# zhongyuanzhao/multihop-offload

Measured on AMD Instinct MI355X. Metric: episodes/sec, higher is better.
Workload: dtype fp32; 1 GPU; model=ChebConv-K2-5L-h32, graph=ba100-m2, global_batch=256, T=1000, parallelism=dp1, congest_jobs=2124

## Files before the change

### multihop_offload_amd/engine.py

```python

from __future__ import annotations

import dataclasses
from typing import Optional, Sequence

import numpy as np
import torch

from .graphs import CaseGraph
from .models.chebconv import ChebConvStack
from .queueing import ConflictCSR, delay_with_fallback, fixed_point_mu
from .ops import dispatch as ops


@dataclasses.dataclass
class JobBatch:
    sources: torch.Tensor
    mask: torch.Tensor
    rates: torch.Tensor
    ul: torch.Tensor
    dl: torch.Tensor

    @property
    def num_real(self):
        return self.mask.sum()


@dataclasses.dataclass
class EpisodeResult:
    tau: torch.Tensor
    congest: torch.Tensor
    num_jobs: torch.Tensor
    delay_emp: torch.Tensor
    loss_fn: Optional[torch.Tensor] = None
    loss_mse: Optional[torch.Tensor] = None
    dst: Optional[torch.Tensor] = None
    route_links: Optional[torch.Tensor] = None
    nhop: Optional[torch.Tensor] = None


def hist_percentile(hist: torch.Tensor, dmax: torch.Tensor,
                    q: float) -> torch.Tensor:
    from .sim.timeslot import delay_bin_upper
    hist = hist.to(torch.int64)
    total = hist.sum(-1)
    need = torch.ceil(q * total.to(torch.float64)).to(torch.int64) \
        .clamp(min=1)
    k = (hist.cumsum(-1) >= need[..., None]).to(torch.int8).argmax(-1)
    edges = torch.tensor([delay_bin_upper(i) for i in range(hist.shape[-1])],
                         dtype=torch.int64, device=hist.device)
    got = torch.minimum(edges[k], dmax.to(torch.int64)).to(torch.float64)
    return torch.where(total > 0, got, torch.full_like(got, float("nan")))


@dataclasses.dataclass
class SimStats:
    delay_max: torch.Tensor
    late: torch.Tensor
    delay_hist: torch.Tensor
    stuck: torch.Tensor
    stuck_age: torch.Tensor
    qlen_sum: torch.Tensor
    qlen_max: torch.Tensor
    busy_slots: torch.Tensor
    nb_sum: torch.Tensor
    delay_sum: torch.Tensor
    count: torch.Tensor
    late_after: torch.Tensor
    num_links: int
    T_sim: int
    warmup: int

    def _scope(self, x: torch.Tensor, per: str, how: str = "sum"):
        if per == "job":
            return x
        if per not in ("graph", "all"):
            raise ValueError("per: 'graph', 'job' or 'all'")
        dims = (1,) if per == "graph" else (0, 1)
        return x.amax(dims) if how == "max" else x.sum(dims)

    @staticmethod
    def _ratio(num, den):
        num, den = num.to(torch.float64), den.to(torch.float64)
        return torch.where(den > 0, num / den.clamp(min=1),
                           torch.full_like(den, float("nan")))

    def percentile(self, q: float, per: str = "graph") -> torch.Tensor:
        return hist_percentile(
            self._scope(self.delay_hist.to(torch.int64), per),
            self._scope(self.delay_max, per, "max"), q)

    def late_ratio(self, per: str = "graph") -> torch.Tensor:
        return self._ratio(self._scope(self.late.to(torch.int64), per),
                           self._scope(self.count.to(torch.int64), per))

    def censored_mean_delay(self, per: str = "graph") -> torch.Tensor:
        return self._ratio(
            self._scope(self.delay_sum + self.stuck_age, per),
            self._scope((self.count + self.stuck).to(torch.int64), per))

    def utilization(self) -> torch.Tensor:
        return self.busy_slots.to(torch.float64) \
            / max(self.T_sim - self.warmup, 1)

    def mean_qlen(self) -> torch.Tensor:
        return self.qlen_sum.to(torch.float64) \
            / max(self.T_sim - self.warmup, 1)

    def mean_contention(self) -> torch.Tensor:
        E = self.num_links
        return self._ratio(self.nb_sum[:, :E], self.busy_slots[:, :E])


@dataclasses.dataclass
class SimResult:
    delay_sum: torch.Tensor
    count: torch.Tensor
    mean_delay: torch.Tensor
    backlog: torch.Tensor
    trace: Optional[torch.Tensor] = None
    stats: Optional[SimStats] = None
    sched_slots: Optional[torch.Tensor] = None

    def sched_share(self) -> torch.Tensor:
        if self.sched_slots is None or self.stats is None:
            raise ValueError("sched_share: needs simulate(stats=True, "
                             "mac='mwis')")
        E = self.sched_slots.shape[1]
        return SimStats._ratio(self.sched_slots,
                               self.stats.busy_slots[:, :E])


class EpisodeEngine:

    def __init__(self, cases: Sequence[CaseGraph], model: ChebConvStack,
                 device: str = "cpu", dtype: torch.dtype = torch.float32,
                 fp_iters: int = 10, walk_cap: Optional[int] = None,
                 delay_clamp: float = 0.0, lam_margin: float = 0.0,
                 native_glue: bool = True):
        assert len(cases) > 0
        N = cases[0].num_nodes
        T = cases[0].T
        assert all(c.num_nodes == N for c in cases), "batch shares N"
        E = max(c.num_links for c in cases)
        self.cases = list(cases)
        self.B, self.N, self.E, self.T = len(cases), N, E, T
        self.E_list = [c.num_links for c in cases]
        self.device = torch.device(device)
        self.dtype = dtype
        self.fp_iters = fp_iters
        self.delay_clamp = float(delay_clamp)
        self.lam_margin = float(lam_margin)
        self.model = model.to(self.device)
        self.walk_cap = walk_cap or N

        Cmax = max(len(c.ext.comp_nodes) for c in cases)
        Ee = E + Cmax
        self.Ee = Ee
        B = self.B

        def t(a, dt=None):
            return torch.as_tensor(np.asarray(a), dtype=dt or dtype,
                                   device=self.device)

        def ti(a):
            return torch.as_tensor(np.asarray(a), dtype=torch.int64,
                                   device=self.device)

        def pad_rows(arrs, width, fill, dt=np.float64):
            out = np.full((B, width), fill, dtype=dt)
            for b, a in enumerate(arrs):
                out[b, :len(a)] = a
            return out

        edges_np = np.zeros((B, E, 2), dtype=np.int64)
        for b, c in enumerate(cases):
            edges_np[b, :c.num_links] = c.edges
        self.edges = ti(edges_np)
        self.link_rates = t(pad_rows([c.link_rates for c in cases], E, 1.0))
        self.cf_degs = t(pad_rows([c.cf_degs for c in cases], E, 0.0))
        self.proc_bws = t([c.proc_bws for c in cases])
        self.roles = ti([c.roles for c in cases])
        self.adj = torch.as_tensor(
            np.stack([c.adj for c in cases]) != 0, device=self.device)
        self.link_matrix = ti([c.link_matrix for c in cases])
        nv = -np.ones((B, N), dtype=np.int64)
        for b, c in enumerate(cases):
            v = c.ext.node_vedge
            nv[b] = np.where(v >= 0, v - c.num_links + E, -1)
        self.node_vedge = ti(nv)
        self.comp_mask = self.roles < 2
        self.sp_hop = t([c.sp_hop for c in cases])
        lm = np.zeros((B, E), dtype=bool)
        for b, c in enumerate(cases):
            lm[b, :c.num_links] = True
        self.link_mask = torch.as_tensor(lm, device=self.device)
        sel_b, sel_e = np.nonzero(lm)
        self._lk_sel = ti(sel_b * E + sel_e)
        e0v = edges_np[sel_b, sel_e, 0]
        e1v = edges_np[sel_b, sel_e, 1]
        self._lk_lin01 = ti(sel_b * (N * N) + e0v * N + e1v)
        self._lk_lin10 = ti(sel_b * (N * N) + e1v * N + e0v)

        S = max(len(c.servers) for c in cases)
        srv = -np.ones((B, S), dtype=np.int64)
        for b, c in enumerate(cases):
            srv[b, :len(c.servers)] = c.servers
        self.S = S
        self.servers = ti(srv)
        self.server_mask = self.servers >= 0
        self.servers_safe = self.servers.clamp(min=0)

        mob_counts = [len(c.mobile_nodes) for c in cases]
        assert min(mob_counts) >= 1, \
            "every case needs at least one mobile node (job sources)"
        self.Jmax = max(mob_counts) - 1 if max(mob_counts) > 1 else 1
        self.mobile_mask = self.roles == 0

        rows, cols = [], []
        for b, c in enumerate(cases):
            r = np.repeat(np.arange(c.num_links),
                          np.diff(c.conf_indptr)) + b * E
            rows.append(r)
            cols.append(c.conf_indices + b * E)
        self.conf = ConflictCSR.__new__(ConflictCSR)
        self.conf.row = ti(np.concatenate(rows))
        self.conf.col = ti(np.concatenate(cols))
        self.conf.n = B * E

        def remap(ids, Eb):
            ids = np.asarray(ids)
            return np.where(ids < Eb, ids, ids - Eb + E)

        rows, cols = [], []
        for b, c in enumerate(cases):
            ext = c.ext
            Eb = c.num_links
            ne = ext.num_edges_ext
            r = remap(np.repeat(np.arange(ne), np.diff(ext.ext_indptr)),
                      Eb) + b * Ee
            rows.append(r)
            cols.append(remap(ext.ext_indices, Eb) + b * Ee)
        self.support = ConflictCSR.__new__(ConflictCSR)
        self.support.row = ti(np.concatenate(rows))
        self.support.col = ti(np.concatenate(cols))
        self.support.n = B * Ee

        def feat(attr, link_fill, tail_fill):
            out = np.full((B, Ee), tail_fill, dtype=np.float64)
            for b, c in enumerate(cases):
                v = getattr(c.ext, attr)
                Eb = c.num_links
                out[b, :Eb] = v[:Eb]
                out[b, Eb:E] = link_fill
                out[b, E:E + len(v) - Eb] = v[Eb:]
            return t(out)

        for c in cases:
            c.ext.refresh_rates()
        self.f_self_loop = feat("edge_self_loop", 0.0, 1.0)
        self.f_as_server = feat("edge_as_server", 0.0, 0.0)
        self.f_rate = feat("edge_rate_ext", 1.0, 1.0)
        self.Cmax = Cmax
        bw = np.ones((B, self.Cmax), dtype=np.float64)
        for b, c in enumerate(cases):
            bw[b, :len(c.ext.comp_nodes)] = c.proc_bws[c.ext.comp_nodes]
        self.bw_comp = t(bw)

        cb, cn, cr = [], [], []
        for b, c in enumerate(cases):
            for rank, n in enumerate(c.ext.comp_nodes):
                cb.append(b)
                cn.append(int(n))
                cr.append(rank)
        self._comp_b = ti(cb)
        self._comp_n = ti(cn)
        self._comp_r = ti(cr)

        self._bidx = torch.arange(B, device=self.device)
        self._eye = torch.eye(N, dtype=torch.bool,
                              device=self.device)[None, :, :]
        self._explore_buf = torch.zeros((), dtype=torch.float32,
                                        device=self.device)
        self._rng_state = torch.tensor([12345, 0], dtype=torch.int64,
                                       device=self.device)
        self.overflow_total = torch.zeros((), dtype=torch.int64,
                                          device=self.device)
        self.T_arr = t([float(c.T) for c in cases])
        self.T_link = self.T_arr.repeat_interleave(E)

        def t32(a):
            return torch.as_tensor(np.asarray(a, dtype=np.int32),
                                   device=self.device)

        self.k_adj_indptr = t32([c.adj_indptr for c in cases])

        def pad_i32(arrs, width):
            out = np.zeros((B, width), dtype=np.int32)
            for b, a in enumerate(arrs):
                out[b, :len(a)] = a
            return t32(out)

        self.k_adj_idx = pad_i32([c.adj_indices for c in cases], 2 * E)
        self.k_adj_link = pad_i32([c.adj_link_ids for c in cases], 2 * E)
        cip = np.zeros((B, E + 1), dtype=np.int32)
        for b, c in enumerate(cases):
            Eb = c.num_links
            cip[b, :Eb + 1] = c.conf_indptr
            cip[b, Eb + 1:] = c.conf_indptr[-1]
        self.k_conf_indptr = t32(cip)
        self.k_E_arr = t32([c.num_links for c in cases])
        self.k_N_arr = t32([getattr(c, "real_n", c.num_nodes)
                            for c in cases])
        self._padded = any(getattr(c, "real_n", c.num_nodes) != N
                           for c in cases)
        cc, base = [], [0]
        for c in cases:
            cc.append(np.asarray(c.conf_indices, dtype=np.int32))
            base.append(base[-1] + len(c.conf_indices))
        self.k_conf_cols = t32(np.concatenate(cc))
        self.k_conf_base = torch.as_tensor(np.asarray(base[:-1]),
                                           dtype=torch.int64,
                                           device=self.device)
        self.k_edges = t32(edges_np)
        self.k_servers = t32(srv)
        ipt = np.zeros((B, Ee + 1), dtype=np.int32)
        cc, base = [], [0]
        for b, c in enumerate(cases):
            ext = c.ext
            Eb = c.num_links
            src_ipt = ext.ext_indptr
            counts = np.zeros(Ee, dtype=np.int64)
            counts[:Eb] = np.diff(src_ipt)[:Eb]
            nv = ext.num_edges_ext - Eb
            counts[E:E + nv] = np.diff(src_ipt)[Eb:]
            ipt[b, 1:] = np.cumsum(counts)
            colsrc = np.asarray(ext.ext_indices)
            link_cols = colsrc[:src_ipt[Eb]]
            virt_cols = colsrc[src_ipt[Eb]:]
            allc = np.concatenate([link_cols, virt_cols])
            allc = np.where(allc < Eb, allc, allc - Eb + E)
            cc.append(allc.astype(np.int32))
            base.append(base[-1] + len(allc))
        self.k_ext_indptr = t32(ipt)
        self.k_ext_max_nnz = int(max(int(c.ext.ext_indptr[-1])
                                     for c in cases))
        self.k_ext_cols = t32(np.concatenate(cc))
        self.k_ext_base = torch.as_tensor(np.asarray(base[:-1]),
                                          dtype=torch.int64,
                                          device=self.device)
        import os
        self.use_hip = (self.device.type == "cuda"
                        and os.environ.get("MHO_FORCE_TORCH") != "1")
        self.hip_walk_ok = self.hip_critic_ok = self.hip_actor_ok = False
        if self.use_hip:
            assert dtype == torch.float32, "HIP kernels are fp32"
            from .ops import dispatch
            plan = dispatch.require_hip().queue_lds_plan(N, E, Ee, fp_iters)
            self.hip_walk_ok = plan["walk_eval"]["fits"]
            self.hip_critic_ok = plan["critic"]["fits"]
            self.hip_actor_ok = (plan["actor_head_fwd"]["fits"]
                                 and plan["actor_head_bwd"]["fits"])
        self.native_glue = bool(native_glue) and self.use_hip

    def set_rng_seed(self, seed: int):
        self._rng_state[0] = int(seed)
        self._rng_state[1] = 0

    def sample_jobs(self, arrival_scale: float,
                    gen: Optional[torch.Generator] = None) -> JobBatch:
        B, N, J = self.B, self.N, self.Jmax
        dev = self.device
        scores_raw = torch.rand(B, N, device=dev, generator=gen)
        r_nj = torch.rand(B, device=dev, generator=gen)
        r_rates = torch.rand(B, J, device=dev, generator=gen)
        return self._jobs_from_draws(scores_raw, r_nj, r_rates,
                                     arrival_scale)

    def _jobs_from_draws(self, scores_raw: torch.Tensor, r_nj: torch.Tensor,
                         r_rates: torch.Tensor,
                         arrival_scale: float) -> JobBatch:
        J = self.Jmax
        dev = self.device
        if self.native_glue:
            sources, mask, rates, ul, dl = ops.require_hip().jobs_from_draws(
                scores_raw, r_nj, r_rates, self.mobile_mask,
                float(arrival_scale))
            return JobBatch(sources=sources, mask=mask, rates=rates, ul=ul,
                            dl=dl)
        scores = torch.where(self.mobile_mask, scores_raw,
                             torch.full_like(scores_raw, 2.0))
        order = torch.argsort(scores, dim=1)
        sources = order[:, :J]
        M = self.mobile_mask.sum(1)
        lo = (0.3 * M).to(torch.int64)
        span = (M - lo).clamp(min=1)
        nj = lo + (r_nj * span.to(self.dtype)).to(torch.int64)
        nj = nj.clamp(min=1)
        mask = torch.arange(J, device=dev)[None, :] < nj[:, None]
        sources = torch.where(mask, sources, sources[:, :1])
        rates = (r_rates * 0.4 + 0.1) * arrival_scale
        z = torch.zeros(self.B, J, device=dev, dtype=self.dtype)
        return JobBatch(
            sources=sources,
            mask=mask,
            rates=torch.where(mask, rates.to(self.dtype), z),
            ul=torch.where(mask, torch.full_like(z, 100.0), z),
            dl=torch.where(mask, torch.full_like(z, 1.0), z),
        )

    def pack_jobs(self, instances) -> JobBatch:
        B, J = self.B, self.Jmax
        assert len(instances) == B
        src = np.zeros((B, J), dtype=np.int64)
        mask = np.zeros((B, J), dtype=bool)
        rates = np.zeros((B, J))
        ul = np.zeros((B, J))
        dl = np.zeros((B, J))
        for b, jobs in enumerate(instances):
            k = jobs.num_jobs
            assert k <= J, (k, J)
            src[b, :k] = jobs.sources
            src[b, k:] = (jobs.sources[0] if k
                          else self.cases[b].ext.comp_nodes[0])
            mask[b, :k] = True
            rates[b, :k] = jobs.rates
            ul[b, :k] = jobs.ul
            dl[b, :k] = jobs.dl
        dev, dt = self.device, self.dtype
        return JobBatch(
            sources=torch.as_tensor(src, device=dev),
            mask=torch.as_tensor(mask, device=dev),
            rates=torch.as_tensor(rates, dtype=dt, device=dev),
            ul=torch.as_tensor(ul, dtype=dt, device=dev),
            dl=torch.as_tensor(dl, dtype=dt, device=dev),
        )

    def _features(self, jobs: JobBatch) -> torch.Tensor:
        if self.native_glue:
            return ops.require_hip().cheb_features(
                jobs.sources, jobs.rates.contiguous(), jobs.ul.contiguous(),
                jobs.mask, self.node_vedge, self.comp_mask, self.f_self_loop,
                self.f_rate, self.f_as_server)
        B, Ee, N = self.B, self.Ee, self.N
        arr = torch.zeros(B, N, dtype=self.dtype, device=self.device)
        arr = arr.scatter_add(1, jobs.sources, jobs.rates * jobs.ul)
        f_job = torch.zeros(B, Ee, dtype=self.dtype, device=self.device)
        vidx = torch.where(self.comp_mask, self.node_vedge,
                           torch.zeros_like(self.node_vedge))
        f_job = f_job.scatter_add(
            1, vidx, torch.where(self.comp_mask, arr, torch.zeros_like(arr)))
        return torch.stack([self.f_self_loop, self.f_rate, f_job,
                            self.f_as_server], dim=-1)

    def _actor_head_tables(self):
        return (self.k_conf_indptr, self.k_conf_base, self.k_conf_cols,
                self.link_rates.contiguous(), self.bw_comp.contiguous(),
                self.k_edges, self.node_vedge, self.T_arr.contiguous(),
                self.k_E_arr)

    def _lam_hip(self, jobs: JobBatch) -> torch.Tensor:
        B, Ee = self.B, self.Ee
        x = self._features(jobs)
        from .ops.functions import ChebStackFn, cheb_compat
        if cheb_compat(self.model):
            params = []
            for layer in self.model.layers:
                params += [layer.weight, layer.bias]
            lam = ChebStackFn.apply(x.contiguous(), self, *params)
        else:
            import os as _os
            if _os.environ.get("MHO_ALLOW_TORCH_GPU") != "1":
                raise RuntimeError(
                    "model shape unsupported by the fused ChebConv "
                    "kernels (feature width > 32 or dropout > 0); "
                    "refusing eager torch on GPU — set "
                    "MHO_ALLOW_TORCH_GPU=1 to override")
            return self.model(x.reshape(B * Ee, 4),
                              self.support).reshape(B, Ee)
        if self.lam_margin:
            lam = lam * (1.0 + self.lam_margin)
        return lam

    def _actor_forward_native(self, jobs: JobBatch):
        lam = self._lam_hip(jobs)
        lam_c = lam.detach().contiguous()
        dm, mu_hist = ops.require_hip().actor_head_fwd(
            lam_c, *self._actor_head_tables(), self.N, self.fp_iters,
            self.delay_clamp)
        return dm, (lam, lam_c, mu_hist)

    def _actor_backward_native(self, saved, grad_edge, dm, unit_mtx,
                               written):
        lam, lam_c, mu_hist = saved
        dlam, loss_mse = ops.require_hip().actor_head_bwd_fused(
            grad_edge.contiguous(), dm, unit_mtx, written, lam_c, mu_hist,
            *self._actor_head_tables(), self.fp_iters, self.delay_clamp)
        lam.backward(dlam)
        return loss_mse

    def actor_forward(self, jobs: JobBatch):
        B, E, Ee, N = self.B, self.E, self.Ee, self.N
        if self.use_hip and self.hip_actor_ok:
            from .ops.functions import ActorHeadFn
            dm = ActorHeadFn.apply(self._lam_hip(jobs), self)
            return dm, None, None

        x = self._features(jobs)
        lam = self.model(x.reshape(B * Ee, 4), self.support).reshape(B, Ee)
        if self.lam_margin:
            lam = lam * (1.0 + self.lam_margin)

        lam_link = lam[:, :E].reshape(-1)
        mu = fixed_point_mu(lam_link, self.link_rates.reshape(-1),
                            self.cf_degs.reshape(-1), self.conf,
                            self.fp_iters)
        link_delay = delay_with_fallback(lam_link, mu, self.T_link, 101.0,
                                         self.delay_clamp).reshape(B, E)
        node_delay = delay_with_fallback(lam[:, E:], self.bw_comp,
                                         self.T_arr[:, None], 100.0,
                                         self.delay_clamp)

        dm = self._delay_matrix(link_delay, node_delay)
        return dm, link_delay, node_delay

    def _delay_matrix(self, link_delay, node_delay):
        B, N, E = self.B, self.N, self.E
        flat = torch.zeros(B * N * N, dtype=self.dtype, device=self.device)
        ld_valid = link_delay.reshape(-1)[self._lk_sel]
        flat = flat.index_put((self._lk_lin01,), ld_valid)
        flat = flat.index_put((self._lk_lin10,), ld_valid)
        diag_idx = (self._bidx[:, None] * (N * N)
                    + torch.arange(N, device=self.device)[None, :] * (N + 1))
        inf = torch.full((B, N), float("inf"), dtype=self.dtype,
                         device=self.device)
        flat = flat.index_put((diag_idx.reshape(-1),), inf.reshape(-1))
        lin = (self._comp_b * (N * N) + self._comp_n * (N + 1))
        flat = flat.index_put((lin,), node_delay[self._comp_b, self._comp_r])
        return flat.reshape(B, N, N)

    def apsp(self, dm: torch.Tensor) -> torch.Tensor:
        B, N = self.B, self.N
        with torch.no_grad():
            if self.native_glue:
                return ops.require_hip().floyd_warshall_dm(
                    dm.detach(), self.adj,
                    self.k_N_arr if self._padded else None)
            w = torch.where(self.adj, dm.detach(),
                            torch.full_like(dm, float("inf")))
            w = torch.where(self._eye, torch.zeros_like(w), w)
            return ops.floyd_warshall(
                w, self.k_N_arr if self._padded else None)

    def offload_decide(self, jobs: JobBatch, sp: torch.Tensor,
                       uds: torch.Tensor, explore: float = 0.0,
                       gen: Optional[torch.Generator] = None,
                       prob: bool = False):
        B, J, S = self.B, self.Jmax, self.S
        if S == 0:
            local = uds.gather(1, jobs.sources) * jobs.ul
            return jobs.sources.clone(), local
        if self.use_hip:
            from .ops import dispatch
            ext = dispatch.require_hip()
            expl_t = None
            if torch.is_tensor(explore):
                expl_t = explore.to(self.device, torch.float32)
            elif explore > 0:
                self._explore_buf.fill_(float(explore))
                expl_t = self._explore_buf
            rng_t = None
            if expl_t is not None or prob:
                self._rng_state[1] += 1
                rng_t = self._rng_state
            dst, islocal = ext.decide(
                sp.contiguous(), self.sp_hop.contiguous(), uds.contiguous(),
                self.k_servers, jobs.sources, jobs.mask,
                jobs.ul.contiguous(), jobs.dl.contiguous(),
                expl_t, rng_t, 1 if prob else 0)
            return dst, None

        bJ = self._bidx[:, None]
        src = jobs.sources
        local = uds.gather(1, src) * jobs.ul

        sp_src = sp[bJ, src]
        hop_src = self.sp_hop[bJ, src]
        srv = self.servers_safe[:, None, :].expand(B, J, S)
        ul_d = torch.maximum(sp_src.gather(2, srv) * jobs.ul[..., None],
                             hop_src.gather(2, srv))
        dl_d = torch.maximum(sp_src.gather(2, srv) * jobs.dl[..., None],
                             hop_src.gather(2, srv))
        uds_srv = uds.gather(1, srv.reshape(B, -1)).reshape(B, J, S)
        pr_d = torch.maximum(uds_srv * jobs.ul[..., None],
                             torch.ones_like(uds_srv))
        server_costs = ul_d + dl_d + pr_d
        server_costs = torch.where(
            self.server_mask[:, None, :], server_costs,
            torch.full_like(server_costs, float("inf")))
        costs = torch.cat([server_costs, local[..., None]], dim=2)

        if prob:
            logits = costs.clamp(max=1e30)
            logits = logits - logits.amax(dim=2, keepdim=True)
            p = torch.exp(logits)
            p = torch.where(torch.isfinite(costs), p, torch.zeros_like(p))
            choice = torch.multinomial(
                p.reshape(B * J, S + 1), 1, generator=gen).reshape(B, J)
        else:
            choice = costs.argmin(dim=2)
        if explore > 0:
            nS = self.server_mask.sum(1, keepdim=True)
            r = torch.rand(B, J, device=self.device, generator=gen)
            rc = (torch.rand(B, J, device=self.device, generator=gen)
                  * (nS + 1).to(self.dtype)).to(torch.int64)
            rc = torch.where(rc >= nS, torch.full_like(rc, S), rc)
            choice = torch.where(r < explore, rc, choice)

        is_local = choice >= torch.minimum(
            self.server_mask.sum(1, keepdim=True),
            torch.full_like(choice, S))
        dst = torch.where(
            is_local, src,
            self.servers_safe.gather(1, choice.clamp(max=S - 1)))
        dst = torch.where(jobs.mask, dst, src)
        est = torch.where(
            is_local, local,
            server_costs.gather(2, choice.clamp(max=S - 1)[..., None])[..., 0])
        return dst, est

    def route_walk(self, jobs: JobBatch, dst: torch.Tensor, sp: torch.Tensor):
        B, J, N = self.B, self.Jmax, self.N
        bJ = self._bidx[:, None]
        node = jobs.sources.clone()
        links, hops = [], torch.zeros(B, J, dtype=torch.int64,
                                      device=self.device)
        sp_to_dst = sp.gather(
            2, dst[:, None, :].expand(B, N, J))
        for _ in range(self.walk_cap):
            active = (node != dst) & jobs.mask
            if not bool(active.any()):
                break
            adj_row = self.adj[bJ, node]
            cand = torch.where(adj_row, sp_to_dst.transpose(1, 2),
                               torch.full_like(sp_to_dst.transpose(1, 2),
                                               float("inf")))
            nxt = cand.argmin(dim=2)
            link = self.link_matrix[bJ, node, nxt]
            links.append(torch.where(active, link,
                                     torch.full_like(link, -1)))
            node = torch.where(active, nxt, node)
            hops += active.to(torch.int64)
        if links:
            route_links = torch.stack(links, dim=2)
        else:
            route_links = torch.full((B, J, 0), -1, dtype=torch.int64,
                                     device=self.device)
        self.overflow_total += ((node != dst) & jobs.mask).sum()
        return route_links, hops

    def _episode_eval(self, jobs: JobBatch, dst: torch.Tensor,
                      sp: torch.Tensor):
        if self.use_hip and self.hip_walk_ok:
            from .ops import dispatch
            ext = dispatch.require_hip()
            H = min(self.walk_cap, 64)
            rl, nhop, delay_emp, unit_mtx, written, overflow = ext.walk_eval(
                sp.contiguous(), jobs.sources, dst.contiguous(), jobs.mask,
                jobs.rates.contiguous(), jobs.ul.contiguous(),
                jobs.dl.contiguous(), self.k_adj_indptr, self.k_adj_idx,
                self.k_adj_link, self.k_conf_indptr, self.k_conf_base,
                self.k_conf_cols, self.link_rates.contiguous(),
                self.proc_bws.contiguous(), self.k_edges,
                self.T_arr.contiguous(), self.k_E_arr, self.k_N_arr, H,
                self.fp_iters)
            self._last_overflow = overflow
            self.overflow_total += overflow.sum().to(torch.int64)
            return rl, nhop, delay_emp, unit_mtx, written
        rl, nhop = self.route_walk(jobs, dst, sp)
        delay_emp, unit_mtx, written, *_ = self.evaluate(jobs, dst, rl, nhop)
        return rl, nhop, delay_emp, unit_mtx, written

    def check_overflow(self, strict: bool = True) -> int:
        n = int(self.overflow_total)
        if n:
            self.overflow_total.zero_()
            if strict:
                raise RuntimeError(
                    f"{n} greedy routing walk(s) failed to reach their "
                    f"destination within walk_cap={self.walk_cap} hops — "
                    "loads/delays for those jobs are truncated "
                    "(pathological delay matrix or walk_cap too small "
                    "for this topology)")
        return n

    def evaluate(self, jobs: JobBatch, dst: torch.Tensor,
                 route_links: torch.Tensor, nhop: torch.Tensor):
        B, E, N, J = self.B, self.E, self.N, self.Jmax
        H = route_links.shape[2]
        valid = route_links >= 0
        safe = route_links.clamp(min=0)

        ulr = jobs.ul * jobs.rates
        dlr = jobs.dl * jobs.rates
        load = (ulr + dlr)[..., None].expand(B, J, H)
        flat_idx = (self._bidx[:, None, None] * E + safe).reshape(-1)
        link_lambda = torch.zeros(B * E, dtype=self.dtype, device=self.device)
        link_lambda = link_lambda.scatter_add(
            0, flat_idx, torch.where(valid, load,
                                     torch.zeros_like(load)).reshape(-1))
        server_load = torch.zeros(B, N, dtype=self.dtype, device=self.device)
        server_load = server_load.scatter_add(
            1, dst, torch.where(jobs.mask, ulr, torch.zeros_like(ulr)))

        with torch.no_grad():
            mu = fixed_point_mu(link_lambda, self.link_rates.reshape(-1),
                                self.cf_degs.reshape(-1), self.conf,
                                self.fp_iters)
        lam_r = link_lambda.reshape(B, E)
        mu_r = mu.reshape(B, E)

        lam_h = lam_r.gather(1, safe.reshape(B, -1)).reshape(B, J, H)
        mu_h = mu_r.gather(1, safe.reshape(B, -1)).reshape(B, J, H)
        tot = (jobs.ul + jobs.dl)[..., None]
        gap = mu_h - lam_h
        unit = torch.where(gap > 0, 1.0 / torch.where(gap > 0, gap,
                                                      torch.ones_like(gap)),
                           self.T_arr[:, None, None] * lam_h / (tot * mu_h))
        nh = nhop.to(self.dtype)[..., None]
        hop_delay = (torch.maximum(jobs.ul[..., None] * unit, nh)
                     + torch.maximum(jobs.dl[..., None] * unit, nh))
        link_part = torch.where(valid, hop_delay,
                                torch.zeros_like(hop_delay)).sum(dim=2)

        bw_dst = self.proc_bws.gather(1, dst)
        sl_dst = server_load.gather(1, dst)
        sgap = bw_dst - sl_dst
        sunit = torch.where(
            sgap > 0, 1.0 / torch.where(sgap > 0, sgap, torch.ones_like(sgap)),
            self.T_arr[:, None] * sl_dst / (jobs.ul * bw_dst))
        server_part = torch.maximum(jobs.ul * sunit, torch.ones_like(sunit))
        delay_emp = torch.where(jobs.mask, link_part + server_part,
                                torch.full_like(link_part, float("nan")))

        unit_mtx = torch.zeros(B * N * N, dtype=self.dtype, device=self.device)
        written = torch.zeros(B * N * N, dtype=torch.bool, device=self.device)
        e0 = self.edges[..., 0].gather(1, safe.reshape(B, -1)).reshape(B, J, H)
        e1 = self.edges[..., 1].gather(1, safe.reshape(B, -1)).reshape(B, J, H)
        base = (self._bidx[:, None, None] * (N * N))
        lin01 = (base + e0 * N + e1).reshape(-1)
        lin10 = (base + e1 * N + e0).reshape(-1)
        vmask = valid.reshape(-1)
        unit_mtx = unit_mtx.index_put((lin01[vmask],),
                                      unit.reshape(-1)[vmask])
        unit_mtx = unit_mtx.index_put((lin10[vmask],),
                                      unit.reshape(-1)[vmask])
        written = written.index_put((lin01[vmask],),
                                    torch.ones_like(lin01[vmask],
                                                    dtype=torch.bool))
        written = written.index_put((lin10[vmask],),
                                    torch.ones_like(lin10[vmask],
                                                    dtype=torch.bool))
        lin_d = (self._bidx[:, None] * (N * N) + dst * (N + 1)).reshape(-1)
        jm = jobs.mask.reshape(-1)
        unit_mtx = unit_mtx.index_put((lin_d[jm],), sunit.reshape(-1)[jm])
        written = written.index_put((lin_d[jm],),
                                    torch.ones_like(lin_d[jm],
                                                    dtype=torch.bool))
        return (delay_emp, unit_mtx.reshape(B, N, N),
                written.reshape(B, N, N), lam_r, mu_r, server_load)

    def critic_backward(self, jobs: JobBatch, dst: torch.Tensor,
                        route_links: torch.Tensor,
                        nhop: Optional[torch.Tensor] = None):
        B, E, Ee, J = self.B, self.E, self.Ee, self.Jmax
        vedge_dst = self.node_vedge.gather(1, dst)
        if self.use_hip and self.hip_critic_ok:
            from .ops import dispatch
            ext = dispatch.require_hip()
            grad_edge, loss = ext.critic(
                route_links.contiguous(), nhop.contiguous(),
                vedge_dst.contiguous(), jobs.mask,
                jobs.rates.contiguous(), jobs.ul.contiguous(),
                jobs.dl.contiguous(), self.k_conf_indptr, self.k_conf_base,
                self.k_conf_cols, self.link_rates.contiguous(),
                self.bw_comp.contiguous(), self.k_E_arr,
                self.T_arr.contiguous(), Ee,
                self.fp_iters, self.delay_clamp)
            return grad_edge, loss.sum()
        H = route_links.shape[2]
        valid = route_links >= 0
        safe = route_links.clamp(min=0)

        routes = torch.zeros(B, Ee, J, dtype=self.dtype, device=self.device)
        jidx = torch.arange(J, device=self.device)[None, :, None] \
            .expand(B, J, H)
        routes = routes.index_put(
            (self._bidx[:, None, None].expand(B, J, H)[valid],
             safe[valid], jidx[valid]), torch.ones(1, dtype=self.dtype,
                                                   device=self.device)[0]
            .expand(int(valid.sum())))
        jm = jobs.mask
        routes = routes.index_put(
            (self._bidx[:, None].expand(B, J)[jm], vedge_dst[jm],
             torch.arange(J, device=self.device)[None, :].expand(B, J)[jm]),
            torch.ones(int(jm.sum()), dtype=self.dtype, device=self.device))
        routes.requires_grad_(True)

        jobs_load = (jobs.rates * jobs.ul)[..., None]
        jobs_data = (jobs.ul + jobs.dl)[:, None, :]
        link_load = torch.bmm(routes, jobs_load)[..., 0]
        lam_link = link_load[:, :E].reshape(-1)
        mu = fixed_point_mu(lam_link, self.link_rates.reshape(-1),
                            self.cf_degs.reshape(-1), self.conf,
                            self.fp_iters)
        link_d = delay_with_fallback(lam_link, mu, self.T_link, 101.0,
                                     self.delay_clamp).reshape(B, E)
        node_d = delay_with_fallback(link_load[:, E:], self.bw_comp,
                                     self.T_arr[:, None], 100.0,
                                     self.delay_clamp)
        unit_edge = torch.cat([link_d, node_d], dim=1)
        delay_job_edge = torch.maximum(
            jobs_data * unit_edge[..., None] * routes, routes)
        loss_fn = delay_job_edge.sum()
        (grad_routes,) = torch.autograd.grad(loss_fn, routes,
                                             retain_graph=False)

        seq = torch.cat([safe, vedge_dst[..., None]], dim=2)
        seq_valid = torch.cat([valid, jm[..., None]], dim=2)
        g_seq = grad_routes.gather(
            1, seq.transpose(1, 2)).transpose(1, 2)
        g_seq = grad_routes.gather(1, seq.permute(0, 2, 1))
        g_seq = g_seq.permute(0, 2, 1)
        g_seq = torch.where(seq_valid, g_seq, torch.zeros_like(g_seq))
        pref = -torch.cumsum(g_seq, dim=2)
        grad_edge = torch.zeros(B * Ee, dtype=self.dtype, device=self.device)
        flat_seq = (self._bidx[:, None, None] * Ee + seq).reshape(-1)
        grad_edge = grad_edge.scatter_add(
            0, flat_seq, torch.where(seq_valid, pref,
                                     torch.zeros_like(pref)).reshape(-1))
        return grad_edge.reshape(B, Ee), loss_fn.detach()

    def grad_dist_matrix(self, grad_edge: torch.Tensor, dm: torch.Tensor,
                         unit_mtx: torch.Tensor, written: torch.Tensor):
        B, N, E = self.B, self.N, self.E
        flat = torch.zeros(B * N * N, dtype=self.dtype, device=self.device)
        ge_valid = grad_edge[:, :E].reshape(-1)[self._lk_sel]
        flat = flat.index_put((self._lk_lin01,), ge_valid)
        flat = flat.index_put((self._lk_lin10,), ge_valid)
        lin = (self._comp_b * (N * N) + self._comp_n * (N + 1))
        flat = flat.index_put(
            (lin,), grad_edge[self._comp_b, E + self._comp_r])
        grad_dist = flat.reshape(B, N, N)

        diff = dm.detach() - unit_mtx
        anchor_mask = written & torch.isfinite(dm.detach())
        anchor = torch.where(anchor_mask, 0.001 * diff,
                             torch.zeros_like(diff))
        n_valid = anchor_mask.sum().clamp(min=1)
        loss_mse = ((torch.where(anchor_mask, diff, torch.zeros_like(diff))
                     ** 2).sum() / n_valid.to(diff.dtype))
        return grad_dist + anchor, loss_mse

    def gnn_episode(self, jobs: JobBatch, explore: float = 0.0,
                    gen: Optional[torch.Generator] = None,
                    train: bool = True, prob: bool = False,
                    per_sample: bool = False,
                    refine: int = 0) -> EpisodeResult:
        ctx = torch.enable_grad() if train else torch.no_grad()
        native_bwd = self.native_glue and self.hip_actor_ok
        with ctx:
            if native_bwd:
                dm, actor_saved = self._actor_forward_native(jobs)
            else:
                dm, link_delay, node_delay = self.actor_forward(jobs)
        sp = self.apsp(dm)
        uds = torch.diagonal(dm.detach(), dim1=1, dim2=2)
        dst, est = self.offload_decide(jobs, sp, uds, explore, gen, prob)
        route_links, nhop, delay_emp, unit_mtx, written = \
            self._episode_eval(jobs, dst, sp)
        for _ in range(int(refine) if not train else 0):
            over = jobs.mask & (delay_emp > self.T_arr[:, None])
            if not bool(over.any()):
                break
            dst = torch.where(over, jobs.sources, dst)
            route_links, nhop, delay_emp, unit_mtx, written = \
                self._episode_eval(jobs, dst, sp)

        loss_fn = loss_mse = None
        self.last_per_sample_grads = None
        if train:
            grad_edge, loss_fn = self.critic_backward(jobs, dst, route_links,
                                                      nhop)
            self.per_sample_request = per_sample
            if native_bwd:
                loss_mse = self._actor_backward_native(
                    actor_saved, grad_edge, dm, unit_mtx, written)
            else:
                grad_dist, loss_mse = self.grad_dist_matrix(
                    grad_edge, dm, unit_mtx, written)
            if per_sample and not self.use_hip:
                params = list(self.model.parameters())
                out = []
                for b in range(self.B):
                    gd = torch.zeros_like(grad_dist)
                    gd[b] = grad_dist[b]
                    gs = torch.autograd.grad(dm, params, grad_outputs=gd,
                                             retain_graph=True,
                                             allow_unused=True)
                    out.append([torch.zeros_like(p) if g is None
                                else g.detach()
                                for p, g in zip(params, gs)])
                self.last_per_sample_grads = out
                dm.backward(grad_dist)
            else:
                if not native_bwd:
                    dm.backward(grad_dist)
                if per_sample:
                    self.last_per_sample_grads = \
                        self._collect_per_sample_grads()
            self.per_sample_request = False

        return self._result(jobs, delay_emp, loss_fn, loss_mse,
                            routes=(dst, route_links, nhop))

    def _result(self, jobs: JobBatch, delay_emp: torch.Tensor,
                loss_fn=None, loss_mse=None, routes=None) -> EpisodeResult:
        if self.native_glue:
            tau, congest, nj = ops.require_hip().episode_summary(
                delay_emp.contiguous(), jobs.mask, self.T_arr)
        else:
            nj = jobs.mask.sum(1)
            de = torch.where(jobs.mask, delay_emp,
                             torch.zeros_like(delay_emp))
            tau = de.sum(1) / nj.to(self.dtype)
            congest = ((delay_emp > self.T_arr[:, None]) & jobs.mask).sum(1)
        dst, route_links, nhop = routes or (None, None, None)
        return EpisodeResult(tau=tau, congest=congest, num_jobs=nj,
                             delay_emp=delay_emp, loss_fn=loss_fn,
                             loss_mse=loss_mse, dst=dst,
                             route_links=route_links, nhop=nhop)

    def draw_arrivals(self, jobs: JobBatch, T_sim: int,
                      gen: Optional[torch.Generator] = None) -> torch.Tensor:
        lam = torch.where(jobs.mask, jobs.rates,
                          torch.zeros_like(jobs.rates))
        lam = lam[:, None, :].expand(self.B, int(T_sim), lam.shape[1])
        arr = torch.poisson(lam.contiguous(), generator=gen)
        if arr.numel() and float(arr.max()) > 255:
            raise ValueError("draw_arrivals: a slot count exceeds 255 "
                             "(uint8) — job rates too high for the "
                             "simulator's arrival format")
        return arr.to(torch.uint8)

    def simulate(self, jobs: JobBatch, result: EpisodeResult,
                 arrivals: torch.Tensor, warmup: int = 0,
                 trace: bool = False, stats: bool = False,
                 late_after=None, mac: str = "share") -> SimResult:
        if mac not in ops.MAC_MODES:
            raise ValueError(f"simulate: mac must be one of {ops.MAC_MODES}, "
                             f"not {mac!r}")
        mwis = mac == "mwis"
        sched = None
        if result.dst is None or result.route_links is None \
                or result.nhop is None:
            raise ValueError("simulate: the EpisodeResult carries no routes")
        B, J = self.B, self.Jmax
        arrivals = torch.as_tensor(arrivals, device=self.device)
        assert arrivals.shape[0] == B and arrivals.shape[2] == J, \
            (tuple(arrivals.shape), (B, J))
        T_sim = arrivals.shape[1]
        warmup = int(warmup)
        st = None
        if stats:
            if late_after is None:
                late_after = torch.floor(self.T_arr)
            if not torch.is_tensor(late_after):
                late_after = torch.full((B,), int(late_after))
            late_after = late_after.to(device=self.device,
                                       dtype=torch.int32).reshape(B)
        if self.use_hip:
            out = ops.timeslot_sim(
                arrivals, result.route_links, result.nhop, result.dst,
                jobs.mask, jobs.ul, jobs.dl, self.link_rates, self.proc_bws,
                self.k_conf_indptr, self.k_conf_base, self.k_conf_cols,
                self.k_E_arr, self.k_N_arr, self.T_arr, warmup=warmup,
                trace=trace, stats=stats, late_after=late_after, mac=mac)
            delay_sum, count, tr = out[:3]
            st = out[3] if stats else None
            sched = out[-1] if mwis else None
        else:
            from .sim.timeslot import num_delay_bins, simulate_routes
            if arrivals.numel() and (int(arrivals.max()) > 255
                                     or int(arrivals.min()) < 0):
                raise ValueError("simulate: arrival counts must lie in "
                                 "[0, 255]")
            delay_sum = torch.zeros(B, J, dtype=torch.int64)
            count = torch.zeros(B, J, dtype=torch.int32)
            tr = torch.zeros(B, T_sim, 3, dtype=torch.int32) if trace \
                else None
            arr_np = arrivals.cpu().numpy()
            if stats:
                st = ops.empty_stats(B, J, self.E + self.N,
                                     num_delay_bins(T_sim))
            if mwis:
                sched = torch.zeros(B, self.E, dtype=torch.int32)
            for b, g in enumerate(self.cases):
                k = int(jobs.mask[b].sum())
                assert bool(jobs.mask[b, :k].all()), "mask is a prefix"
                out = simulate_routes(
                    g, jobs.ul[b, :k].cpu().numpy().astype(np.float64),
                    jobs.dl[b, :k].cpu().numpy().astype(np.float64),
                    result.dst[b, :k].cpu().numpy(),
                    result.route_links[b, :k].cpu().numpy(),
                    result.nhop[b, :k].cpu().numpy(), arr_np[b][:, :k],
                    warmup=warmup, trace=trace, stats=stats,
                    late_after=int(late_after[b]) if stats else None,
                    mac=mac)
                if mwis:
                    sched[b, :g.num_links] = torch.as_tensor(
                        out[-1]["sched_slots"])
                    out = out[:-1]
                if stats:
                    ops.fill_stats(st, b, out[-1], slice(0, k),
                                   g.num_links, self.E)
                delay_sum[b, :k] = torch.as_tensor(out[0])
                count[b, :k] = torch.as_tensor(out[1]).to(torch.int32)
                if trace:
                    for c, name in enumerate(("arrivals", "departures",
                                              "pkts_in_network")):
                        tr[b, :, c] = torch.as_tensor(
                            out[2][name]).to(torch.int32)
            delay_sum = delay_sum.to(self.device)
            count = count.to(self.device)
            tr = tr.to(self.device) if trace else None
            if stats:
                st = {k: v.to(self.device) for k, v in st.items()}
            if mwis:
                sched = sched.to(self.device)
        cnt = count.to(torch.float64)
        mean = torch.where(count > 0,
                           delay_sum.to(torch.float64) / cnt.clamp(min=1),
                           torch.full_like(cnt, float("nan")))
        arrived = torch.where(jobs.mask[:, None, :], arrivals,
                              torch.zeros_like(arrivals))[:, warmup:] \
            .sum(1, dtype=torch.int64)
        if stats:
            st = SimStats(**st, delay_sum=delay_sum, count=count,
                          late_after=late_after, num_links=self.E,
                          T_sim=int(T_sim), warmup=warmup)
        return SimResult(delay_sum=delay_sum, count=count, mean_delay=mean,
                         backlog=arrived - count.to(torch.int64), trace=tr,
                         stats=st, sched_slots=sched)

    def _collect_per_sample_grads(self):
        raw = getattr(self, "_per_sample_raw", None)
        if raw is None:
            raise RuntimeError(
                "per-sample gradients need the fused ChebConv GPU path")
        dW, db = raw
        self._per_sample_raw = None
        params = list(self.model.parameters())
        L = len(params) // 2
        out = []
        for b in range(self.B):
            gset = []
            for l in range(L):
                kw, fi, fo = params[2 * l].shape
                gset.append(dW[b, l, :kw, :fi, :fo])
                gset.append(db[b, l, :params[2 * l + 1].shape[0]])
            out.append(gset)
        return out

    def baseline_episode(self, jobs: JobBatch) -> EpisodeResult:
        B, N = self.B, self.N
        with torch.no_grad():
            dlist = 1.0 / self.link_rates
            dm = self._delay_matrix(
                dlist, torch.zeros_like(self.bw_comp))
            sp = self.apsp(dm)
            dproc = 1.0 / self.proc_bws
            uds = torch.where((self.proc_bws > 0),
                              dproc, torch.full_like(dproc, float("inf")))
            dst, est = self.offload_decide(jobs, sp, uds)
            rl, nhop, delay_emp, _, _ = self._episode_eval(jobs, dst, sp)
            return self._result(jobs, delay_emp, routes=(dst, rl, nhop))

    def local_episode(self, jobs: JobBatch) -> EpisodeResult:
        B, J = self.B, self.Jmax
        with torch.no_grad():
            dst = jobs.sources
            if self.use_hip:
                sp0 = torch.zeros(B, self.N, self.N, dtype=self.dtype,
                                  device=self.device)
                route_links, nhop, delay_emp, _, _ = self._episode_eval(
                    jobs, dst, sp0)
            else:
                route_links = torch.full((B, J, 0), -1, dtype=torch.int64,
                                         device=self.device)
                nhop = torch.zeros(B, J, dtype=torch.int64,
                                   device=self.device)
                delay_emp, *_ = self.evaluate(jobs, dst, route_links, nhop)
            return self._result(jobs, delay_emp,
                                routes=(dst, route_links, nhop))
```

### multihop_offload_amd/ops/dispatch.py

```python

from __future__ import annotations

import os

import torch

from . import torch_ref

_HIP_EXT = None
_HIP_TRIED = False


def _load_hip():
    global _HIP_EXT, _HIP_TRIED
    if _HIP_TRIED:
        return _HIP_EXT
    _HIP_TRIED = True
    try:
        from . import hip_loader
        _HIP_EXT = hip_loader.load()
    except Exception:
        _HIP_EXT = None
    return _HIP_EXT


def hip_available() -> bool:
    return _load_hip() is not None


def require_hip():
    ext = _load_hip()
    if ext is None:
        raise RuntimeError(
            "multihop_offload_amd HIP extension not built — run "
            "`python setup.py build_ext --inplace` (gfx950). GPU execution "
            "without the native kernels is disabled by design.")
    return ext


_require_hip = require_hip


def floyd_warshall(w: torch.Tensor, n_arr=None) -> torch.Tensor:
    if w.is_cuda and os.environ.get("MHO_FORCE_TORCH") != "1":
        ext = _require_hip()
        return ext.floyd_warshall(w.contiguous(), n_arr)
    return torch_ref.floyd_warshall(w)


def fw_force_inplace(on: bool) -> None:
    _require_hip().fw_force_inplace(bool(on))


def queue_csr_force_global(on: bool) -> None:
    _require_hip().queue_csr_force_global(bool(on))


def cheb_force_full_width(on: bool) -> None:
    _require_hip().cheb_force_full_width(bool(on))


def cheb_lds_plan(Ee: int, K: int, max_nnz: int) -> dict:
    plan = _require_hip().cheb_lds_plan(int(Ee), int(K), int(max_nnz))
    return {k: dict(v) for k, v in plan.items()}


STAT_KEYS = ("delay_max", "late", "delay_hist", "stuck", "stuck_age",
             "qlen_sum", "qlen_max", "busy_slots", "nb_sum")
_STAT_I64 = ("stuck_age", "qlen_sum", "nb_sum")
_STAT_PER_JOB = STAT_KEYS[:5]


def empty_stats(B: int, J: int, R: int, NB: int) -> dict:
    out = {}
    for k in STAT_KEYS:
        shape = (B, J, NB) if k == "delay_hist" else \
            (B, J) if k in _STAT_PER_JOB else (B, R)
        out[k] = torch.zeros(shape, dtype=torch.int64 if k in _STAT_I64
                             else torch.int32)
    return out


def fill_stats(st: dict, b: int, one: dict, idx, Eb: int, E: int) -> None:
    for k in STAT_KEYS:
        v = torch.as_tensor(one[k])
        if k in _STAT_PER_JOB:
            st[k][b, idx] = v
        else:
            st[k][b, :Eb] = v[:Eb]
            st[k][b, E:E + len(v) - Eb] = v[Eb:]


def timeslot_lds_plan(N: int, E: int, J: int) -> dict:
    return dict(_require_hip().timeslot_lds_plan(int(N), int(E), int(J)))


def timeslot_stats_lds_plan(N: int, E: int, J: int) -> dict:
    return dict(_require_hip().timeslot_stats_lds_plan(int(N), int(E),
                                                       int(J)))


def timeslot_mwis_lds_plan(N: int, E: int, J: int,
                           stats: bool = False) -> dict:
    return dict(_require_hip().timeslot_mwis_lds_plan(int(N), int(E), int(J),
                                                      bool(stats)))


MAC_MODES = ("share", "mwis")


def timeslot_sim(arrivals, route_links, nhop, dst, mask, ul, dl, link_rates,
                 proc_bws, conf_indptr, conf_base, conf_cols, E_arr, n_arr,
                 T_arr=None, warmup: int = 0, trace: bool = False,
                 stats: bool = False, late_after=None, mac: str = "share"):
    if mac not in MAC_MODES:
        raise ValueError(f"timeslot_sim: mac must be one of {MAC_MODES}, "
                         f"not {mac!r}")
    mwis = mac == "mwis"
    B, T, J = arrivals.shape
    if arrivals.numel() and (int(arrivals.max()) > 255
                             or int(arrivals.min()) < 0):
        raise ValueError("timeslot_sim: arrival counts must lie in [0, 255]")
    mask = mask.to(torch.bool)
    arr = torch.where(mask[:, None, :], arrivals,
                      torch.zeros_like(arrivals)).to(torch.uint8).contiguous()
    if route_links.shape[2] == 0:
        route_links = route_links.new_full((B, J, 1), -1)
    warmup = int(warmup)
    if warmup < 0:
        raise ValueError("timeslot_sim: warmup must be non-negative")

    if stats:
        if late_after is None:
            late_after = T
        if not torch.is_tensor(late_after):
            late_after = torch.full((B,), int(late_after), dtype=torch.int32)
        late_after = late_after.to(device=arr.device, dtype=torch.int32) \
            .reshape(B).contiguous()

    if arr.is_cuda:
        ext = _require_hip()
        slot_off = torch.zeros(B, T + 1, dtype=torch.int32, device=arr.device)
        slot_off[:, 1:] = arr.sum(2, dtype=torch.int64).cumsum(1)
        pool = int(slot_off[:, -1].max()) if B else 0
        if T_arr is None:
            T_arr = torch.zeros(B, dtype=torch.float32, device=arr.device)
        args = (
            arr, slot_off, route_links.to(torch.int32).contiguous(),
            nhop.to(torch.int32).contiguous(),
            dst.to(torch.int64).contiguous(), mask.contiguous(),
            ul.to(torch.float32).contiguous(),
            dl.to(torch.float32).contiguous(), conf_indptr, conf_base,
            conf_cols, link_rates.to(torch.float32).contiguous(),
            proc_bws.to(torch.float32).contiguous(),
            T_arr.to(torch.float32).contiguous(), E_arr, n_arr, warmup,
            pool, bool(trace))
        if stats:
            from ..sim.timeslot import num_delay_bins
            fn = ext.timeslot_sim_mwis_stats if mwis \
                else ext.timeslot_sim_stats
            out = fn(*args, late_after, num_delay_bins(T))
        else:
            out = (ext.timeslot_sim_mwis if mwis else ext.timeslot_sim)(*args)
        delay_sum, count, error, tr = out[:4]
        if bool(error.any()):
            bad = torch.nonzero(error).flatten().tolist()
            raise RuntimeError(
                "timeslot_sim: guard rail tripped (input out of range, pool "
                f"or loop bound) in graphs {bad[:8]}, bits "
                f"{error[bad[:8]].tolist()}")
        ret = (delay_sum, count, (tr if trace else None))
        if stats:
            ret += (dict(zip(STAT_KEYS, out[4:4 + len(STAT_KEYS)])),)
        if mwis:
            ret += (out[-1],)
        return ret

    from types import SimpleNamespace

    import numpy as np

    from ..sim.timeslot import num_delay_bins, simulate_routes
    delay_sum = torch.zeros(B, J, dtype=torch.int64)
    count = torch.zeros(B, J, dtype=torch.int32)
    tr = torch.zeros(B, T, 3, dtype=torch.int32) if trace else None
    cip = conf_indptr.numpy()
    cols = conf_cols.numpy()
    N = proc_bws.shape[1]
    E = link_rates.shape[1]
    st = empty_stats(B, J, E + N, num_delay_bins(T)) if stats else None
    sched = torch.zeros(B, E, dtype=torch.int32) if mwis else None
    for b in range(B):
        Eb = int(E_arr[b])
        lo = int(conf_base[b])
        g = SimpleNamespace(
            num_links=Eb, num_nodes=N, conf_indptr=cip[b, :Eb + 1],
            conf_indices=cols[lo:lo + int(cip[b, Eb])],
            link_rates=link_rates[b, :Eb].numpy().astype(np.float64),
            proc_bws=proc_bws[b].numpy().astype(np.float64))
        idx = torch.nonzero(mask[b]).flatten()
        out = simulate_routes(
            g, ul[b, idx].numpy().astype(np.float64),
            dl[b, idx].numpy().astype(np.float64), dst[b, idx].numpy(),
            route_links[b, idx].numpy(), nhop[b, idx].numpy(),
            arr[b][:, idx].numpy(), warmup=warmup, trace=trace,
            stats=stats, late_after=int(late_after[b]) if stats else None,
            mac=mac)
        if mwis:
            sched[b, :Eb] = torch.as_tensor(out[-1]["sched_slots"])
            out = out[:-1]
        if stats:
            fill_stats(st, b, out[-1], idx, Eb, E)
        delay_sum[b, idx] = torch.as_tensor(out[0])
        count[b, idx] = torch.as_tensor(out[1]).to(torch.int32)
        if trace:
            for k, name in enumerate(("arrivals", "departures",
                                      "pkts_in_network")):
                tr[b, :, k] = torch.as_tensor(out[2][name]).to(torch.int32)
    ret = (delay_sum, count, tr)
    if stats:
        ret += (st,)
    if mwis:
        ret += (sched,)
    return ret
```

### multihop_offload_amd/ops/functions.py

```python

from __future__ import annotations

import torch

from . import dispatch


def cheb_compat(model) -> bool:
    if getattr(model, "dropout", 0.0) > 0:
        return False
    for layer in model.layers:
        K, fi, fo = layer.weight.shape
        if fi > 32 or fo > 32:
            return False
    return True


def cheb_lds_fits(Ee: int, K: int = 2) -> bool:
    return dispatch.require_hip().cheb_fits_lds(Ee, K)


def pack_cheb_params(params):
    L = len(params) // 2
    K = params[0].shape[0]
    Wp = params[0].new_zeros(L, K, 32, 32)
    bp = params[0].new_zeros(L, 32)
    for l in range(L):
        w, b = params[2 * l], params[2 * l + 1]
        Wp[l, :w.shape[0], :w.shape[1], :w.shape[2]] = w
        bp[l, :b.shape[0]] = b
    return Wp, bp


class ChebStackFn(torch.autograd.Function):

    @staticmethod
    def forward(ctx, x: torch.Tensor, eng, *params):
        ext = dispatch.require_hip()
        K = params[0].shape[0]
        ctx.native = bool(getattr(eng, "native_glue", False))
        if ctx.native:
            Wp, bp = ext.cheb_pack_params(list(params))
        else:
            Wp, bp = pack_cheb_params(params)
        ctx.K = K
        ctx.large = not cheb_lds_fits(eng.Ee, K)
        extra = ()
        if K > 2:
            if ctx.large:
                raise RuntimeError(
                    f"fused ChebConv with K={K} does not fit LDS at "
                    f"Ee={eng.Ee}; no GPU path for this configuration "
                    "(set MHO_ALLOW_TORCH_GPU=1 to accept eager torch)")
            lam, acts, t1s = ext.cheb_kn_fwd(x, Wp, bp, eng.k_ext_indptr,
                                             eng.k_ext_base, eng.k_ext_cols,
                                             eng.k_ext_max_nnz)
            ctx.t1s = t1s
        elif ctx.large:
            lam, acts = ext.cheb_large_fwd(x, Wp, bp, eng.k_ext_indptr,
                                           eng.k_ext_base, eng.k_ext_cols)
        else:
            lam, acts, t1s, ctx.edge = ext.cheb_fwd_edge(
                x, Wp, bp, eng.k_ext_indptr, eng.k_ext_base, eng.k_ext_cols,
                eng.k_ext_max_nnz, params[-2].shape[2])
            ctx.t1s = t1s
            extra = (x, lam)
        ctx.save_for_backward(acts, Wp, *extra)
        ctx.eng = eng
        ctx.shapes = [tuple(p.shape) for p in params]
        ctx.params = params
        return lam

    @staticmethod
    def backward(ctx, dlam: torch.Tensor):
        acts, Wp, *x_lam = ctx.saved_tensors
        eng = ctx.eng
        ext = dispatch.require_hip()
        if ctx.K > 2:
            dW, db = ext.cheb_kn_bwd(dlam.contiguous(), acts, ctx.t1s, Wp,
                                     eng.k_ext_indptr, eng.k_ext_base,
                                     eng.k_ext_cols, eng.k_ext_max_nnz)
        elif ctx.large:
            dW, db = ext.cheb_large_bwd(dlam.contiguous(), acts, Wp,
                                        eng.k_ext_indptr, eng.k_ext_base,
                                        eng.k_ext_cols)
        else:
            dW, db = ext.cheb_bwd_edge(dlam.contiguous(), *x_lam, acts,
                                       ctx.t1s, Wp, eng.k_ext_indptr,
                                       eng.k_ext_base, eng.k_ext_cols,
                                       eng.k_ext_max_nnz, ctx.edge)
        if getattr(eng, "per_sample_request", False):
            eng._per_sample_raw = (dW, db)
        if ctx.native:
            return (None, None, *_reduce_grads_native(ext, ctx, dW, db))
        dW = dW.sum(dim=0)
        db = db.sum(dim=0)
        grads = []
        for l in range(len(ctx.shapes) // 2):
            kw, fi, fo = ctx.shapes[2 * l]
            grads.append(dW[l, :kw, :fi, :fo].contiguous())
            grads.append(db[l, :ctx.shapes[2 * l + 1][0]].contiguous())
        return (None, None, *grads)


def _reduce_grads_native(ext, ctx, dW, db):
    shapes = [list(s) for s in ctx.shapes]
    numels = [p.numel() for p in ctx.params]
    owner = getattr(ctx.eng.model, "_fused_grad_owner", None)
    if owner is not None:
        flat_g, offsets = owner
        if len(offsets) == len(ctx.params) and all(
                p.grad is not None and p.grad.is_contiguous()
                and p.grad.shape == p.shape
                and p.grad.data_ptr() == flat_g.data_ptr() + 4 * off
                for p, off in zip(ctx.params, offsets)):
            ext.cheb_reduce_grads(dW, db, shapes, flat_g, list(offsets),
                                  True)
            return [None] * len(ctx.params)
    offsets = [sum(numels[:i]) for i in range(len(numels))]
    flat = dW.new_empty(sum(numels))
    ext.cheb_reduce_grads(dW, db, shapes, flat, offsets, False)
    return [flat[o:o + k].view(s)
            for o, k, s in zip(offsets, numels, ctx.shapes)]


class ActorHeadFn(torch.autograd.Function):

    @staticmethod
    def forward(ctx, lam_ext: torch.Tensor, eng):
        ext = dispatch.require_hip()
        dm, mu_hist = ext.actor_head_fwd(
            lam_ext.contiguous(), *eng._actor_head_tables(), eng.N,
            eng.fp_iters, eng.delay_clamp)
        ctx.save_for_backward(lam_ext, mu_hist)
        ctx.eng = eng
        return dm

    @staticmethod
    def backward(ctx, grad_dist: torch.Tensor):
        lam_ext, mu_hist = ctx.saved_tensors
        eng = ctx.eng
        ext = dispatch.require_hip()
        dlam = ext.actor_head_bwd(
            grad_dist.contiguous(), lam_ext.contiguous(), mu_hist,
            *eng._actor_head_tables(), eng.fp_iters, eng.delay_clamp)
        return dlam, None


class FusedAdam:

    def __init__(self, model, lr=1e-4, betas=(0.9, 0.999), eps=1e-7,
                 constraints=True):
        import torch as _t
        params = list(model.parameters())
        n = sum(p.numel() for p in params)
        dev = params[0].device
        assert params[0].dtype == _t.float32, "FusedAdam is fp32"
        self.flat_p = _t.zeros(n, dtype=_t.float32, device=dev)
        self.flat_g = _t.zeros(n, dtype=_t.float32, device=dev)
        self.m = _t.zeros_like(self.flat_p)
        self.v = _t.zeros_like(self.flat_p)
        self.step_dev = _t.zeros(1, dtype=_t.int32, device=dev)
        segs = []
        off = 0
        with _t.no_grad():
            for p in params:
                k = p.numel()
                self.flat_p[off:off + k] = p.detach().reshape(-1)
                p.data = self.flat_p[off:off + k].view(p.shape)
                p.grad = self.flat_g[off:off + k].view(p.shape)
                if p.dim() == 3:
                    K, fi, fo = p.shape
                    segs.append([off, k, K, fi, fo])
                else:
                    segs.append([off, k, 0, 0, 0])
                off += k
        self.seg = _t.tensor(segs, dtype=_t.int32, device=dev)
        model._fused_grad_owner = (self.flat_g, [s[0] for s in segs])
        self.lr, self.betas, self.eps = lr, betas, eps
        self.constraints = constraints

    def zero_grad(self):
        self.flat_g.zero_()

    def step(self, scale: float = 1.0):
        ext = dispatch.require_hip()
        ext.fused_adam(self.flat_p, self.flat_g, self.m, self.v, self.seg,
                       self.step_dev, scale, self.lr, self.betas[0],
                       self.betas[1], self.eps, self.constraints)

    def state_dict(self):
        return {"m": self.m.detach().clone(),
                "v": self.v.detach().clone(),
                "step_dev": self.step_dev.detach().clone(),
                "lr": self.lr}

    def load_state_dict(self, state):
        with torch.no_grad():
            self.m.copy_(state["m"])
            self.v.copy_(state["v"])
            self.step_dev.copy_(state["step_dev"])
        self.lr = state["lr"]

    @property
    def param_groups(self):
        return [_FusedAdamGroup(self)]


class _FusedAdamGroup(dict):
    def __init__(self, opt):
        super().__init__(lr=opt.lr)
        self._opt = opt

    def __setitem__(self, key, value):
        super().__setitem__(key, value)
        if key == "lr":
            self._opt.lr = value


def timeslot_sim(*args, **kwargs):
    return dispatch.timeslot_sim(*args, **kwargs)


def timeslot_lds_fits(N: int, E: int, J: int) -> bool:
    return bool(dispatch.timeslot_lds_plan(N, E, J)["fits"])
```

### multihop_offload_amd/ops/hip/bindings.cpp

```cpp
#include <torch/extension.h>

torch::Tensor floyd_warshall_hip(torch::Tensor w,
                                 c10::optional<torch::Tensor> n_arr);
std::vector<torch::Tensor> decide_hip(
    torch::Tensor sp, torch::Tensor hop, torch::Tensor uds,
    torch::Tensor servers, torch::Tensor src, torch::Tensor mask,
    torch::Tensor ul, torch::Tensor dl,
    c10::optional<torch::Tensor> explore, c10::optional<torch::Tensor> rng,
    long prob);
std::vector<torch::Tensor> walk_eval_hip(
    torch::Tensor sp, torch::Tensor src, torch::Tensor dst,
    torch::Tensor mask, torch::Tensor rate, torch::Tensor ul,
    torch::Tensor dl, torch::Tensor adj_indptr, torch::Tensor adj_idx,
    torch::Tensor adj_link, torch::Tensor conf_indptr,
    torch::Tensor conf_base, torch::Tensor conf_cols, torch::Tensor rates,
    torch::Tensor bw, torch::Tensor edges, torch::Tensor T_arr,
    torch::Tensor E_arr, torch::Tensor n_arr, long H,
    long fp_iters);
std::vector<torch::Tensor> critic_hip(
    torch::Tensor route_links, torch::Tensor nhop, torch::Tensor vedge_dst,
    torch::Tensor mask, torch::Tensor rate, torch::Tensor ul,
    torch::Tensor dl, torch::Tensor conf_indptr, torch::Tensor conf_base,
    torch::Tensor conf_cols, torch::Tensor rates, torch::Tensor bw_comp,
    torch::Tensor E_arr, torch::Tensor T_arr, long Ee, long iters,
    double cap);
std::vector<torch::Tensor> actor_head_fwd_hip(
    torch::Tensor lam_ext, torch::Tensor conf_indptr,
    torch::Tensor conf_base, torch::Tensor conf_cols, torch::Tensor rates,
    torch::Tensor bw_comp, torch::Tensor edges, torch::Tensor node_vedge,
    torch::Tensor T_arr, torch::Tensor E_arr, long N, long iters,
    double cap);
torch::Tensor actor_head_bwd_hip(
    torch::Tensor grad_dist, torch::Tensor lam_ext, torch::Tensor mu_hist,
    torch::Tensor conf_indptr, torch::Tensor conf_base,
    torch::Tensor conf_cols, torch::Tensor rates, torch::Tensor bw_comp,
    torch::Tensor edges, torch::Tensor node_vedge, torch::Tensor T_arr,
    torch::Tensor E_arr, long iters, double cap);
std::vector<torch::Tensor> actor_head_bwd_fused_hip(
    torch::Tensor grad_edge, torch::Tensor dm, torch::Tensor unit_mtx,
    torch::Tensor written, torch::Tensor lam_ext, torch::Tensor mu_hist,
    torch::Tensor conf_indptr, torch::Tensor conf_base,
    torch::Tensor conf_cols, torch::Tensor rates, torch::Tensor bw_comp,
    torch::Tensor edges, torch::Tensor node_vedge, torch::Tensor T_arr,
    torch::Tensor E_arr, long iters, double cap);
torch::Tensor floyd_warshall_dm_hip(torch::Tensor dm, torch::Tensor adj,
                                    c10::optional<torch::Tensor> n_arr);
void fw_force_inplace(bool on);
long fw_register_rows(long N);
py::dict queue_lds_plan(long N, long E, long Ee, long iters);
py::dict queue_csr_stage(long N, long E, long Ee, long iters);
long queue_csr_bytes(long Eb, long nnz);
void queue_csr_force_global(bool on);
long queue_csr_set_budget(long bytes);

std::vector<torch::Tensor> timeslot_sim_hip(
    torch::Tensor arrivals, torch::Tensor slot_off, torch::Tensor route_links,
    torch::Tensor nhop, torch::Tensor dst, torch::Tensor mask,
    torch::Tensor ul, torch::Tensor dl, torch::Tensor conf_indptr,
    torch::Tensor conf_base, torch::Tensor conf_cols, torch::Tensor rates,
    torch::Tensor bw, torch::Tensor T_arr, torch::Tensor E_arr,
    torch::Tensor n_arr, long warmup, long pool, bool want_trace);
py::dict timeslot_lds_plan(long N, long E, long J);
std::vector<torch::Tensor> timeslot_sim_stats_hip(
    torch::Tensor arrivals, torch::Tensor slot_off, torch::Tensor route_links,
    torch::Tensor nhop, torch::Tensor dst, torch::Tensor mask,
    torch::Tensor ul, torch::Tensor dl, torch::Tensor conf_indptr,
    torch::Tensor conf_base, torch::Tensor conf_cols, torch::Tensor rates,
    torch::Tensor bw, torch::Tensor T_arr, torch::Tensor E_arr,
    torch::Tensor n_arr, long warmup, long pool, bool want_trace,
    torch::Tensor late_after, long nbins);
py::dict timeslot_stats_lds_plan(long N, long E, long J);
std::vector<torch::Tensor> timeslot_sim_mwis_hip(
    torch::Tensor arrivals, torch::Tensor slot_off, torch::Tensor route_links,
    torch::Tensor nhop, torch::Tensor dst, torch::Tensor mask,
    torch::Tensor ul, torch::Tensor dl, torch::Tensor conf_indptr,
    torch::Tensor conf_base, torch::Tensor conf_cols, torch::Tensor rates,
    torch::Tensor bw, torch::Tensor T_arr, torch::Tensor E_arr,
    torch::Tensor n_arr, long warmup, long pool, bool want_trace);
std::vector<torch::Tensor> timeslot_sim_mwis_stats_hip(
    torch::Tensor arrivals, torch::Tensor slot_off, torch::Tensor route_links,
    torch::Tensor nhop, torch::Tensor dst, torch::Tensor mask,
    torch::Tensor ul, torch::Tensor dl, torch::Tensor conf_indptr,
    torch::Tensor conf_base, torch::Tensor conf_cols, torch::Tensor rates,
    torch::Tensor bw, torch::Tensor T_arr, torch::Tensor E_arr,
    torch::Tensor n_arr, long warmup, long pool, bool want_trace,
    torch::Tensor late_after, long nbins);
py::dict timeslot_mwis_lds_plan(long N, long E, long J, bool stats);

std::vector<torch::Tensor> cheb_pack_params_hip(
    std::vector<torch::Tensor> params);
void cheb_reduce_grads_hip(torch::Tensor dW, torch::Tensor db,
                           std::vector<std::vector<int64_t>> shapes,
                           torch::Tensor flat_out,
                           std::vector<int64_t> offsets, bool accumulate);
torch::Tensor cheb_features_hip(
    torch::Tensor sources, torch::Tensor rates, torch::Tensor ul,
    torch::Tensor mask, torch::Tensor node_vedge, torch::Tensor comp_mask,
    torch::Tensor f_self_loop, torch::Tensor f_rate,
    torch::Tensor f_as_server);
std::vector<torch::Tensor> episode_summary_hip(torch::Tensor delay_emp,
                                               torch::Tensor mask,
                                               torch::Tensor T_arr);
std::vector<torch::Tensor> jobs_from_draws_hip(
    torch::Tensor scores_raw, torch::Tensor r_nj, torch::Tensor r_rates,
    torch::Tensor mobile_mask, double arrival_scale);

std::vector<torch::Tensor> cheb_fwd_hip(
    torch::Tensor x, torch::Tensor W, torch::Tensor bias,
    torch::Tensor ext_indptr, torch::Tensor ext_base, torch::Tensor ext_cols,
    long max_nnz);
std::vector<torch::Tensor> cheb_bwd_hip(
    torch::Tensor dlam, torch::Tensor acts, torch::Tensor t1s,
    torch::Tensor W, torch::Tensor ext_indptr, torch::Tensor ext_base,
    torch::Tensor ext_cols, long max_nnz);

std::vector<torch::Tensor> cheb_bwd_hip_mask(
    torch::Tensor dlam, torch::Tensor acts, torch::Tensor t1s,
    torch::Tensor W, torch::Tensor ext_indptr, torch::Tensor ext_base,
    torch::Tensor ext_cols, long max_nnz, long stage_mask);
std::vector<torch::Tensor> cheb_kn_fwd_hip(
    torch::Tensor x, torch::Tensor W, torch::Tensor bias,
    torch::Tensor ext_indptr, torch::Tensor ext_base, torch::Tensor ext_cols,
    long max_nnz);
std::vector<torch::Tensor> cheb_kn_bwd_hip(
    torch::Tensor dlam, torch::Tensor acts, torch::Tensor tks,
    torch::Tensor W, torch::Tensor ext_indptr, torch::Tensor ext_base,
    torch::Tensor ext_cols, long max_nnz);
bool cheb_fits_lds(long Ee, long K);
py::dict cheb_lds_plan_py(long Ee, long K, long max_nnz);
void cheb_force_full_width(bool on);
std::tuple<torch::Tensor, torch::Tensor, torch::Tensor, bool>
cheb_fwd_edge_hip(torch::Tensor x, torch::Tensor W, torch::Tensor bias,
                  torch::Tensor ext_indptr, torch::Tensor ext_base,
                  torch::Tensor ext_cols, long max_nnz, long out_width);
std::vector<torch::Tensor> cheb_bwd_edge_hip(
    torch::Tensor dlam, torch::Tensor x, torch::Tensor lam,
    torch::Tensor acts, torch::Tensor t1s, torch::Tensor W,
    torch::Tensor ext_indptr, torch::Tensor ext_base,
    torch::Tensor ext_cols, long max_nnz, bool edge);
std::vector<torch::Tensor> cheb_bwd_edge_hip_mask(
    torch::Tensor dlam, torch::Tensor x, torch::Tensor lam,
    torch::Tensor acts, torch::Tensor t1s, torch::Tensor W,
    torch::Tensor ext_indptr, torch::Tensor ext_base,
    torch::Tensor ext_cols, long max_nnz, bool edge, long stage_mask);

std::vector<torch::Tensor> cheb_large_fwd_hip(
    torch::Tensor x, torch::Tensor W, torch::Tensor bias,
    torch::Tensor ext_indptr, torch::Tensor ext_base,
    torch::Tensor ext_cols);
std::vector<torch::Tensor> cheb_large_bwd_hip(
    torch::Tensor dlam, torch::Tensor acts, torch::Tensor W,
    torch::Tensor ext_indptr, torch::Tensor ext_base,
    torch::Tensor ext_cols);
void fused_adam_hip(torch::Tensor p, torch::Tensor g, torch::Tensor m,
                    torch::Tensor v, torch::Tensor seg, torch::Tensor step,
                    double scale, double lr, double beta1, double beta2,
                    double eps, bool constraints);

PYBIND11_MODULE(TORCH_EXTENSION_NAME, m) {
    m.def("floyd_warshall", &floyd_warshall_hip);
    m.def("decide", &decide_hip);
    m.def("walk_eval", &walk_eval_hip);
    m.def("critic", &critic_hip);
    m.def("actor_head_fwd", &actor_head_fwd_hip);
    m.def("actor_head_bwd", &actor_head_bwd_hip);
    m.def("actor_head_bwd_fused", &actor_head_bwd_fused_hip);
    m.def("floyd_warshall_dm", &floyd_warshall_dm_hip);
    m.def("fw_force_inplace", &fw_force_inplace);
    m.def("fw_register_rows", &fw_register_rows);
    m.def("cheb_pack_params", &cheb_pack_params_hip);
    m.def("cheb_reduce_grads", &cheb_reduce_grads_hip);
    m.def("cheb_features", &cheb_features_hip);
    m.def("episode_summary", &episode_summary_hip);
    m.def("jobs_from_draws", &jobs_from_draws_hip);
    m.def("queue_lds_plan", &queue_lds_plan);
    m.def("queue_csr_stage", &queue_csr_stage);
    m.def("queue_csr_bytes", &queue_csr_bytes);
    m.def("queue_csr_force_global", &queue_csr_force_global);
    m.def("queue_csr_set_budget", &queue_csr_set_budget);
    m.def("timeslot_sim", &timeslot_sim_hip);
    m.def("timeslot_lds_plan", &timeslot_lds_plan);
    m.def("timeslot_sim_stats", &timeslot_sim_stats_hip);
    m.def("timeslot_stats_lds_plan", &timeslot_stats_lds_plan);
    m.def("timeslot_sim_mwis", &timeslot_sim_mwis_hip);
    m.def("timeslot_sim_mwis_stats", &timeslot_sim_mwis_stats_hip);
    m.def("timeslot_mwis_lds_plan", &timeslot_mwis_lds_plan);
    m.def("cheb_fwd", &cheb_fwd_hip);
    m.def("cheb_bwd", &cheb_bwd_hip);
    m.def("cheb_bwd_ablate", &cheb_bwd_hip_mask);
    m.def("cheb_force_full_width", &cheb_force_full_width);
    m.def("cheb_fwd_edge", &cheb_fwd_edge_hip);
    m.def("cheb_bwd_edge", &cheb_bwd_edge_hip);
    m.def("cheb_bwd_edge_ablate", &cheb_bwd_edge_hip_mask);
    m.def("cheb_kn_fwd", &cheb_kn_fwd_hip);
    m.def("cheb_kn_bwd", &cheb_kn_bwd_hip);
    m.def("cheb_fits_lds", &cheb_fits_lds);
    m.def("cheb_lds_plan", &cheb_lds_plan_py);
    m.def("fused_adam", &fused_adam_hip);
    m.def("cheb_large_fwd", &cheb_large_fwd_hip);
    m.def("cheb_large_bwd", &cheb_large_bwd_hip);
}
```

### multihop_offload_amd/ops/hip/chebconv.hip

```cpp

#include <hip/hip_runtime.h>
#include <torch/extension.h>
#include <ATen/cuda/CUDAContext.h>

#include "cheb_tiles.h"

namespace {

using namespace cheb;

constexpr int FWD_NBUF = 2;
constexpr int BWD_NBUF = 3;
constexpr int KN_NBUF = 3;

constexpr int WGRAD_SPLIT = 2;

DEV_INLINE void gemm_layer_fused(float* __restrict__ Xb,
                                 const float* __restrict__ Tb,
                                 const float* __restrict__ Wl,
                                 const float* __restrict__ bl,
                                 int K, bool last, int rows_pad, int tid) {
    const int lane = tid & 63;
    const int wid = tid >> 6;
    const int nw = blockDim.x >> 6;
    const int r_in = lane & 15;
    const int k_in = lane >> 4;
    for (int mt = wid; mt < rows_pad / 16; mt += nw) {
        f32x4 acc[2] = {{0.f, 0.f, 0.f, 0.f}, {0.f, 0.f, 0.f, 0.f}};
#pragma unroll
        for (int kk = 0; kk < F / 4; ++kk) {
            const int k = kk * 4 + k_in;
            const float a = Xb[(mt * 16 + r_in) * STRIDE + k];
#pragma unroll
            for (int h = 0; h < 2; ++h)
                acc[h] = __builtin_amdgcn_mfma_f32_16x16x4f32(
                    a, Wl[k * F + h * 16 + r_in], acc[h], 0, 0, 0);
        }
        if (K > 1) {
#pragma unroll
            for (int kk = 0; kk < F / 4; ++kk) {
                const int k = kk * 4 + k_in;
                const float a = Tb[(mt * 16 + r_in) * STRIDE + k];
#pragma unroll
                for (int h = 0; h < 2; ++h)
                    acc[h] = __builtin_amdgcn_mfma_f32_16x16x4f32(
                        a, Wl[F * F + k * F + h * 16 + r_in], acc[h], 0, 0,
                        0);
            }
        }
#pragma unroll
        for (int h = 0; h < 2; ++h) {
            const int col = h * 16 + (lane & 15);
            const float bv = bl[col];
#pragma unroll
            for (int r = 0; r < 4; ++r) {
                const int row = mt * 16 + (lane >> 4) * 4 + r;
                Xb[row * STRIDE + col] = act(acc[h][r] + bv, last);
            }
        }
    }
}

DEV_INLINE void gemm_dx_fused(const float* __restrict__ Db,
                              float* __restrict__ Ab,
                              float* __restrict__ Tb,
                              const float* __restrict__ Wl, int K,
                              int rows_pad, int tid) {
    const int lane = tid & 63;
    const int wid = tid >> 6;
    const int nw = blockDim.x >> 6;
    const int mtiles = rows_pad / 16;
    const int r_in = lane & 15;
    const int k_in = lane >> 4;
    for (int t = wid; t < mtiles * 2; t += nw) {
        const int mt = t >> 1;
        const int c0 = (t & 1) * 16;
        f32x4 acc0 = {0.f, 0.f, 0.f, 0.f};
        f32x4 acc1 = {0.f, 0.f, 0.f, 0.f};
#pragma unroll
        for (int kk = 0; kk < F / 4; ++kk) {
            const int k = kk * 4 + k_in;
            const float d = Db[(mt * 16 + r_in) * STRIDE + k];
            acc0 = __builtin_amdgcn_mfma_f32_16x16x4f32(
                d, Wl[(c0 + r_in) * F + k], acc0, 0, 0, 0);
            if (K > 1)
                acc1 = __builtin_amdgcn_mfma_f32_16x16x4f32(
                    d, Wl[F * F + (c0 + r_in) * F + k], acc1, 0, 0, 0);
        }
        const int col = c0 + (lane & 15);
#pragma unroll
        for (int r = 0; r < 4; ++r) {
            const int row = mt * 16 + (lane >> 4) * 4 + r;
            Ab[row * STRIDE + col] = acc0[r];
            if (K > 1) Tb[row * STRIDE + col] = acc1[r];
        }
    }
}

DEV_INLINE void spmv(const float* __restrict__ src, float* __restrict__ dst,
                     const int* __restrict__ indptr,
                     const int* __restrict__ cols, int Ee, int rows_pad,
                     int tid, int nt, int mode) {
    for (int task = tid; task < rows_pad * (F / 8); task += nt) {
        const int r = task / (F / 8);
        const int c0 = (task % (F / 8)) * 8;
        float acc[8] = {0, 0, 0, 0, 0, 0, 0, 0};
        if (r < Ee) {
            int a = indptr[r];
            const int end = indptr[r + 1];
            float acc1[8] = {0, 0, 0, 0, 0, 0, 0, 0};
            for (; a + 3 < end; a += 4) {
                const float* s0 = src + cols[a] * STRIDE + c0;
                const float* s1 = src + cols[a + 1] * STRIDE + c0;
                const float* s2 = src + cols[a + 2] * STRIDE + c0;
                const float* s3 = src + cols[a + 3] * STRIDE + c0;
#pragma unroll
                for (int c = 0; c < 8; ++c) {
                    acc[c] += s0[c] + s1[c];
                    acc1[c] += s2[c] + s3[c];
                }
            }
            for (; a < end; ++a) {
                const float* s = src + cols[a] * STRIDE + c0;
#pragma unroll
                for (int c = 0; c < 8; ++c) acc[c] += s[c];
            }
#pragma unroll
            for (int c = 0; c < 8; ++c) acc[c] += acc1[c];
        }
        float* d = dst + r * STRIDE + c0;
        if (mode == 0) {
#pragma unroll
            for (int c = 0; c < 8; ++c) d[c] = acc[c];
        } else if (mode == 1) {
#pragma unroll
            for (int c = 0; c < 8; ++c) d[c] += acc[c];
        } else if (mode == 2) {
#pragma unroll
            for (int c = 0; c < 8; ++c) d[c] = 2.f * acc[c] - d[c];
        } else {
#pragma unroll
            for (int c = 0; c < 8; ++c) d[c] += 2.f * acc[c];
        }
    }
}

DEV_INLINE void zero_rows(float* __restrict__ buf, int rows_pad, int tid,
                          int nt) {
    for (int t = tid; t < rows_pad * F; t += nt)
        buf[(t / F) * STRIDE + (t % F)] = 0.f;
}

DEV_INLINE void negate_rows(float* __restrict__ buf, int rows_pad, int tid,
                            int nt) {
    for (int t = tid; t < rows_pad * F; t += nt) {
        float* p = buf + (t / F) * STRIDE + (t % F);
        *p = -*p;
    }
}

DEV_INLINE void add_rows(float* __restrict__ dst,
                         const float* __restrict__ src, int rows_pad,
                         int tid, int nt) {
    for (int t = tid; t < rows_pad * F; t += nt)
        dst[(t / F) * STRIDE + (t % F)] += src[(t / F) * STRIDE + (t % F)];
}

DEV_INLINE void bias_act_rows(const float* __restrict__ src,
                              float* __restrict__ dst,
                              const float* __restrict__ bl, bool last,
                              int rows_pad, int tid, int nt) {
    for (int t = tid; t < rows_pad * F; t += nt) {
        const int r = t / F, c = t % F;
        dst[r * STRIDE + c] = act(src[r * STRIDE + c] + bl[c], last);
    }
}

DEV_INLINE void graph_csr(const int* __restrict__ ext_indptr,
                          const long* __restrict__ ext_base,
                          const int* __restrict__ ext_cols, int b, int Ee,
                          int stage_csr, int* __restrict__ lds, int tid,
                          int nt, const int*& ipt, const int*& cls) {
    ipt = ext_indptr + (size_t)b * (Ee + 1);
    cls = ext_cols + ext_base[b];
    if (stage_csr) {
        int* l_ipt = lds;
        int* l_cols = l_ipt + (Ee + 1);
        for (int i = tid; i < Ee + 1; i += nt) l_ipt[i] = ipt[i];
        const int nnz = ipt[Ee];
        for (int i = tid; i < nnz; i += nt) l_cols[i] = cls[i];
        ipt = l_ipt;
        cls = l_cols;
    }
}

DEV_INLINE void load_features(float* __restrict__ Xb,
                              const float* __restrict__ xb, int Ee,
                              int rows_pad, int tid, int nt) {
    for (int r = tid; r < rows_pad; r += nt) {
        float* row = Xb + r * STRIDE;
        for (int c = 0; c < F; ++c) row[c] = 0.f;
        if (r < Ee) {
            const float4 v =
                *reinterpret_cast<const float4*>(xb + (size_t)r * 4);
            row[0] = v.x; row[1] = v.y; row[2] = v.z; row[3] = v.w;
        }
    }
}

DEV_INLINE void load_top_delta(float* __restrict__ Db,
                               const float* __restrict__ dlamb, int Ee,
                               int rows_pad, int tid, int nt) {
    for (int r = tid; r < rows_pad; r += nt) {
        float* row = Db + r * STRIDE;
        for (int c = 0; c < F; ++c) row[c] = 0.f;
        if (r < Ee) row[0] = dlamb[r];
    }
}

constexpr int FIN = 4;

DEV_INLINE void load_rows4(float* __restrict__ buf,
                           const float* __restrict__ g4, int cols, int Ee,
                           int rows_pad, int tid, int nt) {
    for (int r = tid; r < rows_pad; r += nt) {
        float* row = buf + r * STRIDE;
        float4 v = {0.f, 0.f, 0.f, 0.f};
        if (r < Ee) v = *reinterpret_cast<const float4*>(g4 + (size_t)r * 4);
        row[0] = v.x; row[1] = v.y; row[2] = v.z; row[3] = v.w;
        for (int c = FIN; c < cols; ++c) row[c] = 0.f;
    }
}

DEV_INLINE void spmv4(const float* __restrict__ src, float* __restrict__ dst,
                      const int* __restrict__ indptr,
                      const int* __restrict__ cols, int Ee, int rows_pad,
                      int tid, int nt) {
    for (int r = tid; r < rows_pad; r += nt) {
        float acc[FIN] = {0, 0, 0, 0};
        if (r < Ee) {
            int a = indptr[r];
            const int end = indptr[r + 1];
            float acc1[FIN] = {0, 0, 0, 0};
            for (; a + 3 < end; a += 4) {
                const float* s0 = src + cols[a] * STRIDE;
                const float* s1 = src + cols[a + 1] * STRIDE;
                const float* s2 = src + cols[a + 2] * STRIDE;
                const float* s3 = src + cols[a + 3] * STRIDE;
#pragma unroll
                for (int c = 0; c < FIN; ++c) {
                    acc[c] += s0[c] + s1[c];
                    acc1[c] += s2[c] + s3[c];
                }
            }
            for (; a < end; ++a) {
                const float* s = src + cols[a] * STRIDE;
#pragma unroll
                for (int c = 0; c < FIN; ++c) acc[c] += s[c];
            }
#pragma unroll
            for (int c = 0; c < FIN; ++c) acc[c] += acc1[c];
        }
#pragma unroll
        for (int c = 0; c < FIN; ++c) dst[r * STRIDE + c] = acc[c];
    }
}

DEV_INLINE void gemm_layer_first(float* __restrict__ Xb,
                                 const float* __restrict__ Tb,
                                 const float* __restrict__ Wl,
                                 const float* __restrict__ bl, int K,
                                 int rows_pad, int tid) {
    const int lane = tid & 63;
    const int wid = tid >> 6;
    const int nw = blockDim.x >> 6;
    const int r_in = lane & 15;
    const int k_in = lane >> 4;
    for (int mt = wid; mt < rows_pad / 16; mt += nw) {
        const float ax = Xb[(mt * 16 + r_in) * STRIDE + k_in];
        const float at = K > 1 ? Tb[(mt * 16 + r_in) * STRIDE + k_in] : 0.f;
        f32x4 acc[2];
#pragma unroll
        for (int h = 0; h < 2; ++h) {
            const f32x4 zero = {0.f, 0.f, 0.f, 0.f};
            acc[h] = __builtin_amdgcn_mfma_f32_16x16x4f32(
                ax, Wl[k_in * F + h * 16 + r_in], zero, 0, 0, 0);
            if (K > 1)
                acc[h] = __builtin_amdgcn_mfma_f32_16x16x4f32(
                    at, Wl[F * F + k_in * F + h * 16 + r_in], acc[h], 0, 0,
                    0);
        }
#pragma unroll
        for (int h = 0; h < 2; ++h) {
            const int col = h * 16 + (lane & 15);
            const float bv = bl[col];
#pragma unroll
            for (int r = 0; r < 4; ++r) {
                const int row = mt * 16 + (lane >> 4) * 4 + r;
                Xb[row * STRIDE + col] = act(acc[h][r] + bv, false);
            }
        }
    }
}

DEV_INLINE void gemm_layer_last(const float* __restrict__ Xb,
                                const float* __restrict__ Tb,
                                const float* __restrict__ Wl,
                                const float* __restrict__ bl,
                                float* __restrict__ lam, int K, int Ee,
                                int rows_pad, int tid) {
    const int lane = tid & 63;
    const int wid = tid >> 6;
    const int nw = blockDim.x >> 6;
    const int r_in = lane & 15;
    const int k_in = lane >> 4;
    for (int mt = wid; mt < rows_pad / 16; mt += nw) {
        f32x4 acc = {0.f, 0.f, 0.f, 0.f};
#pragma unroll
        for (int kk = 0; kk < F / 4; ++kk) {
            const int k = kk * 4 + k_in;
            acc = __builtin_amdgcn_mfma_f32_16x16x4f32(
                Xb[(mt * 16 + r_in) * STRIDE + k], Wl[k * F + r_in], acc, 0,
                0, 0);
        }
        if (K > 1) {
#pragma unroll
            for (int kk = 0; kk < F / 4; ++kk) {
                const int k = kk * 4 + k_in;
                acc = __builtin_amdgcn_mfma_f32_16x16x4f32(
                    Tb[(mt * 16 + r_in) * STRIDE + k],
                    Wl[F * F + k * F + r_in], acc, 0, 0, 0);
            }
        }
        if ((lane & 15) == 0) {
            const float bv = bl[0];
#pragma unroll
            for (int r = 0; r < 4; ++r) {
                const int row = mt * 16 + (lane >> 4) * 4 + r;
                if (row < Ee) lam[row] = act(acc[r] + bv, true);
            }
        }
    }
}

DEV_INLINE void load_top_delta_edge(float* __restrict__ Db,
                                    const float* __restrict__ dlamb,
                                    const float* __restrict__ lamb, int Ee,
                                    int rows_pad, int tid, int nt) {
    for (int r = tid; r < rows_pad; r += nt) {
        float* row = Db + r * STRIDE;
        float d = 0.f;
        if (r < Ee) d = dlamb[r] * (lamb ? dact(lamb[r], 0.f) : 1.f);
        row[0] = d;
        for (int c = 1; c < 16; ++c) row[c] = 0.f;
    }
}

DEV_INLINE void db_col0(const float* __restrict__ D, int rows,
                        float* __restrict__ db_out, int tid) {
    if (tid >= 64) return;
    float acc = 0.f;
    for (int r = tid; r < rows; r += 64) acc += D[r * STRIDE];
#pragma unroll
    for (int o = 32; o > 0; o >>= 1) acc += __shfl_xor(acc, o);
    if (tid == 0) db_out[0] = acc;
}

DEV_INLINE void wgrad_edge(const float* __restrict__ Xs,
                           const float* __restrict__ Ts,
                           const float* __restrict__ delta,
                           float* __restrict__ dw_out,
                           int K, bool first, int rows, int tid) {
    const int lane = tid & 63;
    const int wid = tid >> 6;
    const int nw = blockDim.x >> 6;
    const int n = rows / (4 * WGRAD_SPLIT);
    for (int t = wid; t < 2 * WGRAD_SPLIT * K; t += nw) {
        const int k = t / (2 * WGRAD_SPLIT);
        const int o = ((t / WGRAD_SPLIT) & 1) * 16;
        const int part = t % WGRAD_SPLIT;
        const int i0 = first ? 0 : o, j0 = first ? o : 0;
        const f32x4 acc = wgrad_tile(k ? Ts : Xs, delta, i0, j0, part * n,
                                     part * n + n, lane);
        if (first ? (lane >> 4) == 0 : (lane & 15) == 0) {
#pragma unroll
            for (int r = 0; r < 4; ++r)
                atomicAdd(&dw_out[(size_t)k * F * F +
                                  (i0 + (lane >> 4) * 4 + r) * F + j0 +
                                  (lane & 15)], acc[r]);
        }
    }
}

DEV_INLINE void dx_rank1(const float* __restrict__ Db, float* __restrict__ Ab,
                         const float* __restrict__ wv,
                         const int* __restrict__ indptr,
                         const int* __restrict__ cols, int Ee, int rows_pad,
                         int K, int parts, int tid, int nt) {
    for (int r = tid; r < rows_pad; r += nt) {
        const float dv = (parts & 1) ? Db[r * STRIDE] : 0.f;
        float ad = 0.f;
        if ((parts & 2) && K > 1 && r < Ee) {
            int a = indptr[r];
            const int end = indptr[r + 1];
            float ad1 = 0.f;
            for (; a + 3 < end; a += 4) {
                ad += Db[cols[a] * STRIDE] + Db[cols[a + 1] * STRIDE];
                ad1 += Db[cols[a + 2] * STRIDE] + Db[cols[a + 3] * STRIDE];
            }
            for (; a < end; ++a) ad += Db[cols[a] * STRIDE];
            ad += ad1;
        }
        float* o = Ab + r * STRIDE;
#pragma unroll
        for (int c = 0; c < F; ++c)
            o[c] = dv * wv[c] + (K > 1 ? ad * wv[F + c] : 0.f);
    }
}

template <bool EDGE>
__global__ void cheb_fwd_kernel(
    const float* __restrict__ x_in,
    const float* __restrict__ W,
    const float* __restrict__ bias,
    const int* __restrict__ ext_indptr,
    const long* __restrict__ ext_base,
    const int* __restrict__ ext_cols,
    float* __restrict__ acts,
    float* __restrict__ t1s,
    float* __restrict__ lam,
    int Ee, int L, int K, int rows_pad, int stage_csr) {
    extern __shared__ __attribute__((aligned(16))) char smem_raw[];
    float* Xb = reinterpret_cast<float*>(smem_raw);
    float* Tb = Xb + (size_t)rows_pad * STRIDE;
    float* Wl = Tb + (size_t)rows_pad * STRIDE;
    float* bl = Wl + (size_t)K * F * F;

    const int b = blockIdx.x;
    const int tid = threadIdx.x, nt = blockDim.x;
    const int *ipt, *cls;
    graph_csr(ext_indptr, ext_base, ext_cols, b, Ee, stage_csr,
              reinterpret_cast<int*>(bl + F), tid, nt, ipt, cls);
    float* actsb = acts + (size_t)b * (L + 1) * Ee * F;

    if (EDGE) {
        load_rows4(Xb, x_in + (size_t)b * Ee * 4, FIN, Ee, rows_pad, tid,
                   nt);
        for (int i = tid; i < K * FIN * F; i += nt)
            Wl[(i / (FIN * F)) * F * F + i % (FIN * F)] =
                W[(size_t)(i / (FIN * F)) * F * F + i % (FIN * F)];
        for (int i = tid; i < F; i += nt) bl[i] = bias[i];
        __syncthreads();
        if (K > 1) {
            spmv4(Xb, Tb, ipt, cls, Ee, rows_pad, tid, nt);
            __syncthreads();
            float4* t1b =
                reinterpret_cast<float4*>(t1s + (size_t)b * L * Ee * F);
            for (int r = tid; r < Ee; r += nt) {
                const float* s = Tb + r * STRIDE;
                t1b[r] = make_float4(s[0], s[1], s[2], s[3]);
            }
        }
        gemm_layer_first(Xb, Tb, Wl, bl, K, rows_pad, tid);
        __syncthreads();
        store_rows(Xb, actsb + (size_t)Ee * F, 0, Ee, Ee, tid, nt);
        __syncthreads();
    } else {
        load_features(Xb, x_in + (size_t)b * Ee * 4, Ee, rows_pad, tid, nt);
        __syncthreads();
        store_rows(Xb, actsb, 0, Ee, Ee, tid, nt);
    }

    for (int l = EDGE ? 1 : 0; l < (EDGE ? L - 1 : L); ++l) {
        for (int i = tid; i < K * F * F; i += nt)
            Wl[i] = W[((size_t)l * K) * F * F + i];
        for (int i = tid; i < F; i += nt) bl[i] = bias[l * F + i];
        __syncthreads();
        if (K > 1) {
            spmv(Xb, Tb, ipt, cls, Ee, rows_pad, tid, nt, 0);
            __syncthreads();
            store_rows(Tb, t1s + ((size_t)b * L + l) * Ee * F, 0, Ee,
                       Ee, tid, nt);
        }
        gemm_layer_fused(Xb, Tb, Wl, bl, K, l == L - 1, rows_pad, tid);
        __syncthreads();
        store_rows(Xb, actsb + (size_t)(l + 1) * Ee * F, 0, Ee, Ee,
                   tid, nt);
        __syncthreads();
    }

    if (EDGE) {
        const int l = L - 1;
        for (int i = tid; i < K * F * F; i += nt)
            Wl[i] = W[((size_t)l * K) * F * F + i];
        if (tid == 0) bl[0] = bias[l * F];
        __syncthreads();
        if (K > 1) {
            spmv(Xb, Tb, ipt, cls, Ee, rows_pad, tid, nt, 0);
            __syncthreads();
            store_rows(Tb, t1s + ((size_t)b * L + l) * Ee * F, 0, Ee, Ee,
                       tid, nt);
        }
        gemm_layer_last(Xb, Tb, Wl, bl, lam + (size_t)b * Ee, K, Ee,
                        rows_pad, tid);
    } else {
        for (int r = tid; r < Ee; r += nt) lam[(size_t)b * Ee + r] =
            Xb[r * STRIDE];
    }
}

template <bool EDGE>
__global__ void cheb_bwd_kernel(
    const float* __restrict__ dlam,
    const float* __restrict__ x_in,
    const float* __restrict__ lam,
    const float* __restrict__ acts,
    const float* __restrict__ t1s,
    const float* __restrict__ W,
    const int* __restrict__ ext_indptr,
    const long* __restrict__ ext_base,
    const int* __restrict__ ext_cols,
    float* __restrict__ dW,
    float* __restrict__ db,
    int Ee, int L, int K, int rows_pad, int stage_csr, int stage_mask) {
    extern __shared__ __attribute__((aligned(16))) char smem_raw[];
    float* Ab = reinterpret_cast<float*>(smem_raw);
    float* Db = Ab + (size_t)rows_pad * STRIDE;
    float* Tb = Db + (size_t)rows_pad * STRIDE;
    float* Wl = Tb + (size_t)rows_pad * STRIDE;

    const int b = blockIdx.x;
    const int tid = threadIdx.x, nt = blockDim.x;
    const int *ipt, *cls;
    graph_csr(ext_indptr, ext_base, ext_cols, b, Ee, stage_csr,
              reinterpret_cast<int*>(Wl + (size_t)K * F * F), tid, nt, ipt,
              cls);
    const float* actsb = acts + (size_t)b * (L + 1) * Ee * F;
    float* dWb = dW + (size_t)b * L * K * F * F;
    float* dbb = db + (size_t)b * L * F;

    if (EDGE) {
        const int l = L - 1;
        load_top_delta_edge(Db, dlam + (size_t)b * Ee,
                            (stage_mask & 1) ? lam + (size_t)b * Ee : nullptr,
                            Ee, rows_pad, tid, nt);
        if (stage_mask & 2) {
            load_rows(Ab, actsb + (size_t)l * Ee * F, 0, rows_pad, Ee, tid,
                      nt);
            if (K > 1)
                load_rows(Tb, t1s + ((size_t)b * L + l) * Ee * F, 0,
                          rows_pad, Ee, tid, nt);
        }
        for (int i = tid; i < K * F; i += nt)
            Wl[i] = W[(((size_t)l * K + i / F) * F + i % F) * F];
        __syncthreads();
        if (stage_mask & 1) db_col0(Db, Ee, dbb + l * F, tid);
        if (stage_mask & 2)
            wgrad_edge(Ab, Tb, Db, dWb + ((size_t)l * K) * F * F, K, false,
                       rows_pad, tid);
        __syncthreads();
        if (stage_mask & 12)
            dx_rank1(Db, Ab, Wl, ipt, cls, Ee, rows_pad, K,
                     (stage_mask >> 2) & 3, tid, nt);
        __syncthreads();
        float* tmp = Ab;
        Ab = Db;
        Db = tmp;
    } else {
        load_top_delta(Db, dlam + (size_t)b * Ee, Ee, rows_pad, tid, nt);
        __syncthreads();
    }

    for (int l = EDGE ? L - 2 : L - 1; l >= (EDGE ? 1 : 0); --l) {
        const bool last = (l == L - 1);
        if (stage_mask & 1)
            mask_rows(Db, actsb + (size_t)(l + 1) * Ee * F, Ee,
                      last ? 0.f : 0.2f, tid, nt);
        if (stage_mask & 2) {
            if (EDGE)
                load_rows(Ab, actsb + (size_t)l * Ee * F, 0, rows_pad, Ee, tid,
                      nt);
            else
                load_rows(Ab, actsb + (size_t)l * Ee * F, 0, rows_pad, Ee,
                          tid, nt);
        }
        for (int i = tid; i < K * F * F; i += nt)
            Wl[i] = W[((size_t)l * K) * F * F + i];
        __syncthreads();

        if (stage_mask & 1) db_colsum(Db, Ee, dbb + l * F, tid, nt);
        if (stage_mask & 2) {
            if (K > 1)
                load_rows(Tb, t1s + ((size_t)b * L + l) * Ee * F, 0,
                          rows_pad, Ee, tid, nt);
            wgrad_rows<WGRAD_SPLIT>(Ab, Db, dWb + ((size_t)l * K) * F * F,
                                    rows_pad, tid);
            if (K > 1) {
                __syncthreads();
                wgrad_rows<WGRAD_SPLIT>(Tb, Db,
                                        dWb + ((size_t)l * K + 1) * F * F,
                                        rows_pad, tid);
            }
        }
        if (l == 0) break;
        __syncthreads();
        if (stage_mask & 4)
            gemm_dx_fused(Db, Ab, Tb, Wl, K, rows_pad, tid);
        __syncthreads();
        if ((stage_mask & 8) && K > 1) {
            spmv(Tb, Ab, ipt, cls, Ee, rows_pad, tid, nt, 1);
            __syncthreads();
        }
        float* tmp = Ab;
        Ab = Db;
        Db = tmp;
        if (!EDGE) __syncthreads();
    }

    if (EDGE) {
        if (stage_mask & 1)
            mask_rows(Db, actsb + (size_t)Ee * F, Ee, 0.2f, tid, nt);
        if (stage_mask & 2) {
            load_rows4(Ab, x_in + (size_t)b * Ee * 4, 16, Ee, rows_pad, tid,
                       nt);
            if (K > 1)
                load_rows4(Tb, t1s + (size_t)b * L * Ee * F, 16, Ee,
                           rows_pad, tid, nt);
        }
        __syncthreads();
        if (stage_mask & 1) db_colsum(Db, Ee, dbb, tid, nt);
        if (stage_mask & 2)
            wgrad_edge(Ab, Tb, Db, dWb, K, true, rows_pad, tid);
    }
}

__global__ void cheb_kn_fwd_kernel(
    const float* __restrict__ x_in,
    const float* __restrict__ W,
    const float* __restrict__ bias,
    const int* __restrict__ ext_indptr,
    const long* __restrict__ ext_base,
    const int* __restrict__ ext_cols,
    float* __restrict__ acts,
    float* __restrict__ tks,
    float* __restrict__ lam,
    int B, int Ee, int L, int K, int rows_pad, int stage_csr) {
    extern __shared__ __attribute__((aligned(16))) char smem_raw[];
    float* Xb = reinterpret_cast<float*>(smem_raw);
    float* Tb = Xb + (size_t)rows_pad * STRIDE;
    float* Yb = Tb + (size_t)rows_pad * STRIDE;
    float* Wl = Yb + (size_t)rows_pad * STRIDE;
    float* bl = Wl + (size_t)K * F * F;

    const int b = blockIdx.x;
    const int tid = threadIdx.x, nt = blockDim.x;
    const int *ipt, *cls;
    graph_csr(ext_indptr, ext_base, ext_cols, b, Ee, stage_csr,
              reinterpret_cast<int*>(bl + F), tid, nt, ipt, cls);
    float* actsb = acts + (size_t)b * (L + 1) * Ee * F;
    float* tksb = tks + (size_t)b * L * (K - 1) * Ee * F;

    load_features(Xb, x_in + (size_t)b * Ee * 4, Ee, rows_pad, tid, nt);
    __syncthreads();
    store_rows(Xb, actsb, 0, Ee, Ee, tid, nt);

    for (int l = 0; l < L; ++l) {
        for (int i = tid; i < K * F * F; i += nt)
            Wl[i] = W[((size_t)l * K) * F * F + i];
        for (int i = tid; i < F; i += nt) bl[i] = bias[l * F + i];
        zero_rows(Yb, rows_pad, tid, nt);
        __syncthreads();
        gemm_rows(Xb, Yb, Wl, false, rows_pad, tid);
        spmv(Xb, Tb, ipt, cls, Ee, rows_pad, tid, nt, 0);
        __syncthreads();
        store_rows(Tb, tksb + (size_t)l * (K - 1) * Ee * F, 0, Ee, Ee,
                   tid, nt);
        gemm_rows(Tb, Yb, Wl + F * F, false, rows_pad, tid);
        float* prev = Xb;
        float* cur = Tb;
        for (int k = 2; k < K; ++k) {
            __syncthreads();
            spmv(cur, prev, ipt, cls, Ee, rows_pad, tid, nt, 2);
            __syncthreads();
            float* t = prev; prev = cur; cur = t;
            store_rows(cur, tksb + ((size_t)l * (K - 1) + k - 1) * Ee * F,
                       0, Ee, Ee, tid, nt);
            gemm_rows(cur, Yb, Wl + (size_t)k * F * F, false, rows_pad,
                      tid);
        }
        __syncthreads();
        bias_act_rows(Yb, Xb, bl, l == L - 1, rows_pad, tid, nt);
        __syncthreads();
        store_rows(Xb, actsb + (size_t)(l + 1) * Ee * F, 0, Ee, Ee,
                   tid, nt);
        __syncthreads();
    }
    for (int r = tid; r < Ee; r += nt) lam[(size_t)b * Ee + r] =
        Xb[r * STRIDE];
}

__global__ void cheb_kn_bwd_kernel(
    const float* __restrict__ dlam,
    const float* __restrict__ acts,
    const float* __restrict__ tks,
    const float* __restrict__ W,
    const int* __restrict__ ext_indptr,
    const long* __restrict__ ext_base,
    const int* __restrict__ ext_cols,
    float* __restrict__ dW,
    float* __restrict__ db,
    int B, int Ee, int L, int K, int rows_pad, int stage_csr) {
    extern __shared__ __attribute__((aligned(16))) char smem_raw[];
    float* Db = reinterpret_cast<float*>(smem_raw);
    float* Pb = Db + (size_t)rows_pad * STRIDE;
    float* Qb = Pb + (size_t)rows_pad * STRIDE;
    float* Wl = Qb + (size_t)rows_pad * STRIDE;

    const int b = blockIdx.x;
    const int tid = threadIdx.x, nt = blockDim.x;
    const int *ipt, *cls;
    graph_csr(ext_indptr, ext_base, ext_cols, b, Ee, stage_csr,
              reinterpret_cast<int*>(Wl + (size_t)K * F * F), tid, nt, ipt,
              cls);
    const float* actsb = acts + (size_t)b * (L + 1) * Ee * F;
    const float* tksb = tks + (size_t)b * L * (K - 1) * Ee * F;
    float* dWb = dW + (size_t)b * L * K * F * F;
    float* dbb = db + (size_t)b * L * F;

    load_top_delta(Db, dlam + (size_t)b * Ee, Ee, rows_pad, tid, nt);
    __syncthreads();

    for (int l = L - 1; l >= 0; --l) {
        const bool last = (l == L - 1);
        mask_rows(Db, actsb + (size_t)(l + 1) * Ee * F, Ee,
                  last ? 0.f : 0.2f, tid, nt);
        for (int i = tid; i < K * F * F; i += nt)
            Wl[i] = W[((size_t)l * K) * F * F + i];
        __syncthreads();
        db_colsum(Db, Ee, dbb + l * F, tid, nt);
        load_rows(Pb, actsb + (size_t)l * Ee * F, 0, rows_pad, Ee, tid, nt);
        __syncthreads();
        wgrad_rows<WGRAD_SPLIT>(Pb, Db, dWb + ((size_t)l * K) * F * F,
                                rows_pad, tid);
        for (int k = 1; k < K; ++k) {
            __syncthreads();
            load_rows(Pb, tksb + ((size_t)l * (K - 1) + k - 1) * Ee * F, 0,
                      rows_pad, Ee, tid, nt);
            __syncthreads();
            wgrad_rows<WGRAD_SPLIT>(Pb, Db,
                                    dWb + ((size_t)l * K + k) * F * F,
                                    rows_pad, tid);
        }
        if (l == 0) break;
        __syncthreads();
        zero_rows(Pb, rows_pad, tid, nt);
        zero_rows(Qb, rows_pad, tid, nt);
        __syncthreads();
        if (K == 1) {
            gemm_rows(Db, Pb, Wl, true, rows_pad, tid);
            __syncthreads();
            for (int t = tid; t < rows_pad * F; t += nt)
                Db[(t / F) * STRIDE + (t % F)] =
                    Pb[(t / F) * STRIDE + (t % F)];
        } else {
            gemm_rows(Db, Pb, Wl + (size_t)(K - 1) * F * F, true, rows_pad,
                     tid);
            gemm_rows(Db, Qb, Wl + (size_t)(K - 2) * F * F, true, rows_pad,
                     tid);
            float* cur = Pb;
            float* prv = Qb;
            for (int k = K - 1; k >= 2; --k) {
                __syncthreads();
                spmv(cur, prv, ipt, cls, Ee, rows_pad, tid, nt, 3);
                __syncthreads();
                negate_rows(cur, rows_pad, tid, nt);
                __syncthreads();
                gemm_rows(Db, cur, Wl + (size_t)(k - 2) * F * F, true,
                         rows_pad, tid);
                float* t = cur; cur = prv; prv = t;
            }
            __syncthreads();
            spmv(cur, Db, ipt, cls, Ee, rows_pad, tid, nt, 0);
            __syncthreads();
            add_rows(Db, prv, rows_pad, tid, nt);
        }
        __syncthreads();
    }
}

}

bool cheb_fits_lds(long Ee, long K) {
    const bool kn = K > 2;
    return cheb_lds_plan(Ee, K, kn ? KN_NBUF : FWD_NBUF, true, 0).fits &&
           cheb_lds_plan(Ee, K, kn ? KN_NBUF : BWD_NBUF, false, 0).fits;
}

py::dict cheb_lds_plan_py(long Ee, long K, long max_nnz) {
    using namespace pybind11::literals;
    auto row = [&](int nbuf, bool with_bias) {
        const LdsPlan p = cheb_lds_plan((int)Ee, (int)K, nbuf, with_bias,
                                        max_nnz);
        return py::dict("rows_pad"_a = p.rows_pad,
                        "lds_bytes"_a = (long)p.lds_bytes,
                        "stage_csr"_a = p.stage_csr, "fits"_a = p.fits);
    };
    return py::dict("fwd"_a = row(FWD_NBUF, true),
                    "bwd"_a = row(BWD_NBUF, false),
                    "kn_fwd"_a = row(KN_NBUF, true),
                    "kn_bwd"_a = row(KN_NBUF, false));
}

static bool cheb_full_forced = false;
void cheb_force_full_width(bool on) { cheb_full_forced = on; }

static std::vector<torch::Tensor> cheb_fwd_launch(
    torch::Tensor x, torch::Tensor W, torch::Tensor bias,
    torch::Tensor ext_indptr, torch::Tensor ext_base,
    torch::Tensor ext_cols, long max_nnz, bool edge) {
    const int B = x.size(0), Ee = x.size(1);
    const int L = W.size(0), K = W.size(1);
    TORCH_CHECK(K <= 2, "fused ChebConv kernel supports K<=2");
    TORCH_CHECK(x.dim() == 3 && x.size(2) == FIN && x.is_contiguous(),
                "x must be a contiguous (B,Ee,4)");
    const LdsPlan plan = cheb_lds_plan(Ee, K, FWD_NBUF, true, max_nnz);
    TORCH_CHECK(plan.fits, "graph too large for fused ChebConv");
    auto acts = torch::empty({B, L + 1, Ee, F}, x.options());
    auto t1s = torch::empty({B, L, Ee, F}, x.options());
    auto lam = torch::empty({B, Ee}, x.options());
    auto stream = at::cuda::getCurrentCUDAStream();
    hipLaunchKernelGGL(edge ? cheb_fwd_kernel<true> : cheb_fwd_kernel<false>,
                       dim3(B), dim3(512), plan.lds_bytes, stream.stream(),
                       x.data_ptr<float>(), W.data_ptr<float>(),
                       bias.data_ptr<float>(), ext_indptr.data_ptr<int>(),
                       ext_base.data_ptr<long>(), ext_cols.data_ptr<int>(),
                       acts.data_ptr<float>(), t1s.data_ptr<float>(),
                       lam.data_ptr<float>(),
                       Ee, L, K, plan.rows_pad, plan.stage_csr);
    return {lam, acts, t1s};
}

std::vector<torch::Tensor> cheb_fwd_hip(
    torch::Tensor x, torch::Tensor W, torch::Tensor bias,
    torch::Tensor ext_indptr, torch::Tensor ext_base,
    torch::Tensor ext_cols, long max_nnz) {
    return cheb_fwd_launch(x, W, bias, ext_indptr, ext_base, ext_cols,
                           max_nnz, false);
}

std::tuple<torch::Tensor, torch::Tensor, torch::Tensor, bool>
cheb_fwd_edge_hip(torch::Tensor x, torch::Tensor W, torch::Tensor bias,
                  torch::Tensor ext_indptr, torch::Tensor ext_base,
                  torch::Tensor ext_cols, long max_nnz, long out_width) {
    const bool edge = !cheb_full_forced && out_width == 1 && W.size(0) >= 2;
    auto out = cheb_fwd_launch(x, W, bias, ext_indptr, ext_base, ext_cols,
                               max_nnz, edge);
    return {out[0], out[1], out[2], edge};
}

std::vector<torch::Tensor> cheb_kn_fwd_hip(
    torch::Tensor x, torch::Tensor W, torch::Tensor bias,
    torch::Tensor ext_indptr, torch::Tensor ext_base,
    torch::Tensor ext_cols, long max_nnz) {
    const int B = x.size(0), Ee = x.size(1);
    const int L = W.size(0), K = W.size(1);
    TORCH_CHECK(K >= 2, "generic-K ChebConv kernel expects K>=2");
    const LdsPlan plan = cheb_lds_plan(Ee, K, KN_NBUF, true, max_nnz);
    TORCH_CHECK(plan.fits,
                "graph too large for generic-K fused ChebConv (LDS)");
    auto acts = torch::empty({B, L + 1, Ee, F}, x.options());
    auto tks = torch::empty({B, L, K - 1, Ee, F}, x.options());
    auto lam = torch::empty({B, Ee}, x.options());
    auto stream = at::cuda::getCurrentCUDAStream();
    hipLaunchKernelGGL(cheb_kn_fwd_kernel, dim3(B), dim3(512),
                       plan.lds_bytes, stream.stream(),
                       x.data_ptr<float>(), W.data_ptr<float>(),
                       bias.data_ptr<float>(), ext_indptr.data_ptr<int>(),
                       ext_base.data_ptr<long>(), ext_cols.data_ptr<int>(),
                       acts.data_ptr<float>(), tks.data_ptr<float>(),
                       lam.data_ptr<float>(),
                       B, Ee, L, K, plan.rows_pad, plan.stage_csr);
    return {lam, acts, tks};
}

std::vector<torch::Tensor> cheb_kn_bwd_hip(
    torch::Tensor dlam, torch::Tensor acts, torch::Tensor tks,
    torch::Tensor W, torch::Tensor ext_indptr, torch::Tensor ext_base,
    torch::Tensor ext_cols, long max_nnz) {
    const int B = dlam.size(0), Ee = dlam.size(1);
    const int L = W.size(0), K = W.size(1);
    const LdsPlan plan = cheb_lds_plan(Ee, K, KN_NBUF, false, max_nnz);
    TORCH_CHECK(plan.fits,
                "graph too large for generic-K fused ChebConv bwd (LDS)");
    auto dW = torch::zeros({B, L, K, F, F}, dlam.options());
    auto db = torch::zeros({B, L, F}, dlam.options());
    auto stream = at::cuda::getCurrentCUDAStream();
    hipLaunchKernelGGL(cheb_kn_bwd_kernel, dim3(B), dim3(512),
                       plan.lds_bytes, stream.stream(),
                       dlam.data_ptr<float>(), acts.data_ptr<float>(),
                       tks.data_ptr<float>(), W.data_ptr<float>(),
                       ext_indptr.data_ptr<int>(), ext_base.data_ptr<long>(),
                       ext_cols.data_ptr<int>(),
                       dW.data_ptr<float>(), db.data_ptr<float>(),
                       B, Ee, L, K, plan.rows_pad, plan.stage_csr);
    return {dW, db};
}

std::vector<torch::Tensor> cheb_bwd_edge_hip_mask(
    torch::Tensor dlam, torch::Tensor x, torch::Tensor lam,
    torch::Tensor acts, torch::Tensor t1s, torch::Tensor W,
    torch::Tensor ext_indptr, torch::Tensor ext_base,
    torch::Tensor ext_cols, long max_nnz, bool edge, long stage_mask) {
    const int B = dlam.size(0), Ee = dlam.size(1);
    const int L = W.size(0), K = W.size(1);
    TORCH_CHECK(K <= 2, "fused ChebConv kernel supports K<=2");
    TORCH_CHECK(dlam.is_contiguous() && acts.size(0) == B &&
                acts.size(1) == L + 1 && acts.size(2) == Ee &&
                t1s.size(0) == B && t1s.size(1) == L && t1s.size(2) == Ee,
                "cheb_bwd: dlam / acts / t1s shapes disagree");
    if (edge)
        TORCH_CHECK(L >= 2 && x.dim() == 3 && x.size(0) == B &&
                    x.size(1) == Ee && x.size(2) == FIN &&
                    x.is_contiguous() && lam.dim() == 2 &&
                    lam.size(0) == B && lam.size(1) == Ee &&
                    lam.is_contiguous(),
                    "cheb_bwd_edge: x (B,Ee,4) and lam (B,Ee) of the "
                    "forward expected");
    const LdsPlan plan = cheb_lds_plan(Ee, K, BWD_NBUF, false, max_nnz);
    TORCH_CHECK(plan.fits, "graph too large for fused ChebConv bwd");
    auto dW = torch::zeros({B, L, K, F, F}, dlam.options());
    auto db = torch::zeros({B, L, F}, dlam.options());
    auto stream = at::cuda::getCurrentCUDAStream();
    hipLaunchKernelGGL(edge ? cheb_bwd_kernel<true> : cheb_bwd_kernel<false>,
                       dim3(B), dim3(512), plan.lds_bytes, stream.stream(),
                       dlam.data_ptr<float>(),
                       edge ? x.data_ptr<float>() : nullptr,
                       edge ? lam.data_ptr<float>() : nullptr,
                       acts.data_ptr<float>(), t1s.data_ptr<float>(),
                       W.data_ptr<float>(), ext_indptr.data_ptr<int>(),
                       ext_base.data_ptr<long>(), ext_cols.data_ptr<int>(),
                       dW.data_ptr<float>(), db.data_ptr<float>(),
                       Ee, L, K, plan.rows_pad, plan.stage_csr,
                       (int)stage_mask);
    return {dW, db};
}

std::vector<torch::Tensor> cheb_bwd_edge_hip(
    torch::Tensor dlam, torch::Tensor x, torch::Tensor lam,
    torch::Tensor acts, torch::Tensor t1s, torch::Tensor W,
    torch::Tensor ext_indptr, torch::Tensor ext_base,
    torch::Tensor ext_cols, long max_nnz, bool edge) {
    return cheb_bwd_edge_hip_mask(dlam, x, lam, acts, t1s, W, ext_indptr,
                                  ext_base, ext_cols, max_nnz, edge, 0xF);
}

std::vector<torch::Tensor> cheb_bwd_hip_mask(
    torch::Tensor dlam, torch::Tensor acts, torch::Tensor t1s,
    torch::Tensor W, torch::Tensor ext_indptr, torch::Tensor ext_base,
    torch::Tensor ext_cols, long max_nnz, long stage_mask) {
    return cheb_bwd_edge_hip_mask(dlam, torch::Tensor(), torch::Tensor(),
                                  acts, t1s, W, ext_indptr, ext_base,
                                  ext_cols, max_nnz, false, stage_mask);
}

std::vector<torch::Tensor> cheb_bwd_hip(
    torch::Tensor dlam, torch::Tensor acts, torch::Tensor t1s,
    torch::Tensor W, torch::Tensor ext_indptr, torch::Tensor ext_base,
    torch::Tensor ext_cols, long max_nnz) {
    return cheb_bwd_hip_mask(dlam, acts, t1s, W, ext_indptr, ext_base,
                             ext_cols, max_nnz, 0xF);
}
```

### multihop_offload_amd/ops/hip/episode.hip

```cpp

#include <hip/hip_runtime.h>
#include <torch/extension.h>
#include <ATen/cuda/CUDAContext.h>

#include "queue_model.h"

namespace {

DEV_INLINE float fmax1(float a, float b) { return a > b ? a : b; }

DEV_INLINE unsigned long long mix64(unsigned long long z) {
    z += 0x9E3779B97F4A7C15ull;
    z = (z ^ (z >> 30)) * 0xBF58476D1CE4E5B9ull;
    z = (z ^ (z >> 27)) * 0x94D049BB133111EBull;
    return z ^ (z >> 31);
}

DEV_INLINE float u01(unsigned long long h) {
    return (float)(h >> 40) * (1.0f / 16777216.0f);
}

DEV_INLINE float server_cost(const float* sp_row, const float* hop_row,
                             const float* uds, int sv, float ulj,
                             float dlj) {
    const float spv = sp_row[sv];
    const float hpv = hop_row[sv];
    return fmax1(spv * ulj, hpv) + fmax1(spv * dlj, hpv)
           + fmax1(uds[sv] * ulj, 1.0f);
}

DEV_INLINE float softmax_w(float c, float cmax) {
    return isfinite(c) ? __expf((c < 1e30f ? c : 1e30f) - cmax) : 0.f;
}

__global__ void decide_kernel(
    const float* __restrict__ sp,
    const float* __restrict__ hop,
    const float* __restrict__ uds,
    const int* __restrict__ servers,
    const long* __restrict__ src,
    const bool* __restrict__ mask,
    const float* __restrict__ ul,
    const float* __restrict__ dl,
    const float* __restrict__ explore,
    const long* __restrict__ rng,
    long* __restrict__ dst_out,
    bool* __restrict__ islocal_out,
    int prob, int N, int J, int S) {
    const int b = blockIdx.x;
    const float* spb = sp + (size_t)b * N * N;
    const float* hpb = hop + (size_t)b * N * N;
    const float* udsb = uds + (size_t)b * N;
    const int* srvb = servers + (size_t)b * S;
    const float eps = explore ? *explore : 0.0f;
    const unsigned long long key =
        rng ? mix64((unsigned long long)rng[0]
                    ^ mix64((unsigned long long)rng[1])) : 0ull;
    int nS = 0;
    for (int s = 0; s < S; ++s) nS += (srvb[s] >= 0);
    for (int j = threadIdx.x; j < J; j += blockDim.x) {
        const size_t bj = (size_t)b * J + j;
        const int s0 = (int)src[bj];
        if (!mask[bj]) { dst_out[bj] = s0; islocal_out[bj] = true; continue; }
        const float ulj = ul[bj], dlj = dl[bj];
        const float local = udsb[s0] * ulj;
        const float* sp_row = spb + (size_t)s0 * N;
        const float* hop_row = hpb + (size_t)s0 * N;
        int best_s;
        if (prob) {
            float cmax = local < 1e30f ? local : 1e30f;
            for (int s = 0; s < S; ++s) {
                const int sv = srvb[s];
                if (sv < 0) continue;
                float c = server_cost(sp_row, hop_row, udsb, sv, ulj, dlj);
                if (isfinite(c)) { c = c < 1e30f ? c : 1e30f;
                                   cmax = c > cmax ? c : cmax; }
            }
            float psum = 0.f;
            for (int s = 0; s < S; ++s) {
                const int sv = srvb[s];
                if (sv < 0) continue;
                psum += softmax_w(
                    server_cost(sp_row, hop_row, udsb, sv, ulj, dlj), cmax);
            }
            psum += softmax_w(local, cmax);
            const float r = u01(mix64(key ^ (unsigned long long)bj)) * psum;
            float acc = 0.f;
            best_s = -1;
            for (int s = 0; s < S; ++s) {
                const int sv = srvb[s];
                if (sv < 0) continue;
                acc += softmax_w(
                    server_cost(sp_row, hop_row, udsb, sv, ulj, dlj), cmax);
                if (r < acc) { best_s = s; break; }
            }
        } else {
            float best = INFINITY;
            best_s = -1;
            for (int s = 0; s < S; ++s) {
                const int sv = srvb[s];
                if (sv < 0) continue;
                const float c =
                    server_cost(sp_row, hop_row, udsb, sv, ulj, dlj);
                if (c < best) { best = c; best_s = s; }
            }
            if (local < best) best_s = -1;
        }
        if (eps > 0.f) {
            const unsigned long long h1 =
                mix64(key ^ (0x517CC1B727220A95ull + bj));
            if (u01(h1) < eps) {
                const int rc = (int)(u01(mix64(h1)) * (float)(nS + 1));
                best_s = rc >= nS ? -1 : rc;
            }
        }
        dst_out[bj] = best_s < 0 ? s0 : srvb[best_s];
        islocal_out[bj] = best_s < 0;
    }
}

__global__ void walk_eval_kernel(
    const float* __restrict__ sp,
    const long* __restrict__ src,
    const long* __restrict__ dstv,
    const bool* __restrict__ mask,
    const float* __restrict__ rate,
    const float* __restrict__ ul,
    const float* __restrict__ dl,
    const int* __restrict__ adj_indptr,
    const int* __restrict__ adj_idx,
    const int* __restrict__ adj_link,
    const qm::Tables t,
    const int* __restrict__ edges,
    int* __restrict__ route_links,
    int* __restrict__ nhop,
    float* __restrict__ delay_emp,
    float* __restrict__ unit_mtx,
    bool* __restrict__ written,
    unsigned long long* __restrict__ upack,
    int* __restrict__ overflow,
    const int* __restrict__ n_arr,
    const qm::WalkPlan p, int stage_budget, int N, int E, int J, int H,
    int fp_iters) {
    extern __shared__ __attribute__((aligned(16))) char smem_raw[];
    float* lds = reinterpret_cast<float*>(smem_raw);
    float* lam = lds + p.lam;
    float* mu = lds + p.mu;
    float* busy = lds + p.busy;
    float* sload = lds + p.sload;

    const int b = blockIdx.x;
    const int tid = threadIdx.x;
    const int nt = blockDim.x;
    const float* spb = sp + (size_t)b * N * N;
    const int* aip = adj_indptr + (size_t)b * (N + 1);
    const int* aix = adj_idx + (size_t)b * 2 * E;
    const int* alk = adj_link + (size_t)b * 2 * E;
    const qm::Graph g = qm::graph_view(t, b);
    unsigned long long* upk = upack + (size_t)b * N * N;
    const int Eb = g.Eb;
    const int nb_ = n_arr[b];
    const qm::Csr csr = qm::stage_csr(
        g.cip, g.rates, g.ccols, Eb, smem_raw + qm::stage_align(p.lds_bytes),
        stage_budget, tid, nt);

    for (int e = tid; e < Eb; e += nt) lam[e] = 0.0f;
    for (int n = tid; n < nb_; n += nt) sload[n] = 0.0f;
    for (int i = tid; i < nb_ * nb_; i += nt)
        upk[(i / nb_) * N + (i % nb_)] = 0ull;
    __syncthreads();

    for (int j = tid; j < J; j += nt) {
        const size_t bj = (size_t)b * J + j;
        if (!mask[bj]) {
            nhop[bj] = 0;
            for (int h = 0; h < H; ++h)
                route_links[bj * H + h] = -1;
            continue;
        }
        const int d = (int)dstv[bj];
        int node = (int)src[bj];
        const float add = (ul[bj] + dl[bj]) * rate[bj];
        int h = 0;
        while (node != d && h < H) {
            const int lo = aip[node], hi = aip[node + 1];
            float bestv = INFINITY;
            int bestn = -1, bestl = -1;
            for (int a = lo; a < hi; ++a) {
                const int nb2 = aix[a];
                const float v = spb[(size_t)nb2 * N + d];
                if (v < bestv) { bestv = v; bestn = nb2; bestl = alk[a]; }
            }
            if (bestl < 0) break;
            route_links[((size_t)b * J + j) * H + h] = bestl;
            atomicAdd(&lam[bestl], add);
            node = bestn;
            ++h;
        }
        if (node != d) atomicAdd(&overflow[b], 1);
        nhop[bj] = h;
        for (int h2 = h; h2 < H; ++h2)
            route_links[bj * H + h2] = -1;
        atomicAdd(&sload[d], ul[bj] * rate[bj]);
    }
    __syncthreads();

    qm::fixed_point_fwd(csr, lam, mu, busy, Eb, 0, fp_iters, tid, nt);

    const int* edg = edges + (size_t)b * E * 2;
    for (int j = tid; j < J; j += nt) {
        const size_t bj = (size_t)b * J + j;
        if (!mask[bj]) { delay_emp[bj] = NAN; continue; }
        const float ulj = ul[bj], dlj = dl[bj];
        const float tot = ulj + dlj;
        const float nh = (float)nhop[bj];
        const unsigned long long jtag = ((unsigned long long)(j + 1)) << 32;
        float acc = 0.0f;
        for (int h = 0; h < nhop[bj]; ++h) {
            const int l = route_links[((size_t)b * J + j) * H + h];
            if (l < 0) break;
            const float unit = qm::emp_unit(lam[l], mu[l], g.T, tot);
            const int u = edg[l * 2], v = edg[l * 2 + 1];
            const unsigned long long pk = jtag | (unsigned long long)
                __float_as_uint(unit);
            atomicMax(&upk[(size_t)u * N + v], pk);
            atomicMax(&upk[(size_t)v * N + u], pk);
            acc += fmax1(ulj * unit, nh) + fmax1(dlj * unit, nh);
        }
        const int d = (int)dstv[bj];
        const float sunit = qm::emp_unit(sload[d], g.bw[d], g.T, ulj);
        atomicMax(&upk[(size_t)d * N + d],
                  jtag | (unsigned long long)__float_as_uint(sunit));
        acc += fmax1(ulj * sunit, 1.0f);
        delay_emp[bj] = acc;
    }
    __syncthreads();
    float* um = unit_mtx + (size_t)b * N * N;
    bool* wm = written + (size_t)b * N * N;
    for (int i = tid; i < N * N; i += nt) {
        const int r = i / N, c = i % N;
        const unsigned long long pk =
            (r < nb_ && c < nb_) ? upk[i] : 0ull;
        um[i] = pk ? __uint_as_float((unsigned int)(pk & 0xffffffffull))
                   : 0.f;
        wm[i] = pk != 0ull;
    }
}

}

std::vector<torch::Tensor> decide_hip(
    torch::Tensor sp, torch::Tensor hop, torch::Tensor uds,
    torch::Tensor servers, torch::Tensor src, torch::Tensor mask,
    torch::Tensor ul, torch::Tensor dl,
    c10::optional<torch::Tensor> explore, c10::optional<torch::Tensor> rng,
    long prob) {
    const int B = sp.size(0), N = sp.size(1);
    const int J = src.size(1), S = servers.size(1);
    auto dst = torch::empty({B, J}, src.options());
    auto islocal = torch::empty({B, J}, mask.options());
    const float* ep = explore.has_value()
        ? explore->data_ptr<float>() : nullptr;
    const long* rp = rng.has_value() ? rng->data_ptr<long>() : nullptr;
    auto stream = at::cuda::getCurrentCUDAStream();
    hipLaunchKernelGGL(decide_kernel, dim3(B), dim3(256), 0, stream.stream(),
                       sp.data_ptr<float>(), hop.data_ptr<float>(),
                       uds.data_ptr<float>(),
                       servers.data_ptr<int>(), src.data_ptr<long>(),
                       mask.data_ptr<bool>(), ul.data_ptr<float>(),
                       dl.data_ptr<float>(), ep, rp,
                       dst.data_ptr<long>(),
                       islocal.data_ptr<bool>(), (int)prob, N, J, S);
    return {dst, islocal};
}

std::vector<torch::Tensor> walk_eval_hip(
    torch::Tensor sp, torch::Tensor src, torch::Tensor dst,
    torch::Tensor mask, torch::Tensor rate, torch::Tensor ul,
    torch::Tensor dl, torch::Tensor adj_indptr, torch::Tensor adj_idx,
    torch::Tensor adj_link, torch::Tensor conf_indptr,
    torch::Tensor conf_base, torch::Tensor conf_cols, torch::Tensor rates,
    torch::Tensor bw, torch::Tensor edges, torch::Tensor T_arr,
    torch::Tensor E_arr, torch::Tensor n_arr, long H,
    long fp_iters) {
    const int B = sp.size(0), N = sp.size(1);
    const int J = src.size(1), E = rates.size(1);
    auto opts_i = adj_indptr.options();
    auto opts_f = sp.options();
    auto route_links = torch::empty({B, J, H}, opts_i.dtype(torch::kInt32));
    auto nhop = torch::empty({B, J}, opts_i.dtype(torch::kInt32));
    auto delay_emp = torch::empty({B, J}, opts_f);
    auto unit_mtx = torch::empty({B, N, N}, opts_f);
    auto written = torch::empty({B, N, N}, opts_f.dtype(torch::kBool));
    auto upack = torch::empty({B, N, N}, opts_f.dtype(torch::kInt64));
    auto overflow = torch::zeros({B}, opts_i.dtype(torch::kInt32));
    const qm::WalkPlan p = qm::walk_plan(N, E);
    TORCH_CHECK(p.fits, "graph too large for LDS walk_eval");
    auto stream = at::cuda::getCurrentCUDAStream();
    const int budget = qm::stage_budget(p);
    hipLaunchKernelGGL(walk_eval_kernel, dim3(B), dim3(p.threads),
                       qm::launch_lds_bytes(p, budget), stream.stream(),
                       sp.data_ptr<float>(), src.data_ptr<long>(),
                       dst.data_ptr<long>(), mask.data_ptr<bool>(),
                       rate.data_ptr<float>(), ul.data_ptr<float>(),
                       dl.data_ptr<float>(),
                       adj_indptr.data_ptr<int>(), adj_idx.data_ptr<int>(),
                       adj_link.data_ptr<int>(),
                       qm::tables(conf_indptr, conf_base, conf_cols, rates,
                                  bw, T_arr, E_arr),
                       edges.data_ptr<int>(),
                       route_links.data_ptr<int>(), nhop.data_ptr<int>(),
                       delay_emp.data_ptr<float>(),
                       unit_mtx.data_ptr<float>(), written.data_ptr<bool>(),
                       reinterpret_cast<unsigned long long*>(
                           upack.data_ptr<long>()),
                       overflow.data_ptr<int>(), n_arr.data_ptr<int>(), p,
                       budget, N, E, J, (int)H, (int)fp_iters);
    return {route_links, nhop, delay_emp, unit_mtx, written, overflow};
}
```

### multihop_offload_amd/ops/hip/optimizer.hip

```cpp

#include <hip/hip_runtime.h>
#include <torch/extension.h>
#include <ATen/cuda/CUDAContext.h>

namespace {

constexpr int NT = 256;
constexpr int SEG_GROUP = 16;

__device__ __forceinline__ void tree_rows(float (*red)[NT], int rows,
                                          int tid, int nt) {
    __syncthreads();
    for (int w = nt >> 1; w > 0; w >>= 1) {
        if (tid < w)
            for (int r = 0; r < rows; ++r) red[r][tid] += red[r][tid + w];
        __syncthreads();
    }
}

__device__ __forceinline__ float adam_element(
    float* __restrict__ p, const float* __restrict__ g,
    float* __restrict__ m, float* __restrict__ v, int j, float f, float lr,
    float beta1, float beta2, float eps, float bc1, float bc2) {
    if (f < 0.f) return p[j];
    float gv = g[j] * f;
    gv = isfinite(gv) ? gv : 0.f;
    const float mn = beta1 * m[j] + (1.f - beta1) * gv;
    const float vn = beta2 * v[j] + (1.f - beta2) * gv * gv;
    m[j] = mn;
    v[j] = vn;
    float pj = p[j];
    pj -= lr * (mn * bc1) / (sqrtf(vn * bc2) + eps);
    p[j] = pj;
    return pj;
}

__global__ void fused_adam_kernel(
    float* __restrict__ p, float* __restrict__ g,
    float* __restrict__ m, float* __restrict__ v,
    const int* __restrict__ seg, int n_seg,
    float scale, float lr, float beta1, float beta2, float eps,
    int* __restrict__ step_dev, int do_constraints) {
    __shared__ float red[SEG_GROUP][NT];
    __shared__ float factor[SEG_GROUP];
    __shared__ float bc_s[2];
    const int tid = threadIdx.x;
    const int nt = blockDim.x;
    if (tid == 0) {
        const float t = (float)(atomicAdd(step_dev, 1) + 1);
        bc_s[0] = 1.0f / (1.0f - powf(beta1, t));
        bc_s[1] = 1.0f / (1.0f - powf(beta2, t));
    }

    for (int s0 = 0; s0 < n_seg; s0 += SEG_GROUP) {
        const int ns = n_seg - s0 < SEG_GROUP ? n_seg - s0 : SEG_GROUP;
        const int* sg = seg + s0 * 5;

        for (int r = 0; r < ns; ++r) {
            const int off = sg[r * 5], size = sg[r * 5 + 1];
            float acc = 0.f;
            for (int i = tid; i < size; i += nt) {
                const float gv = g[off + i] * scale;
                g[off + i] = gv;
                acc += gv * gv;
            }
            red[r][tid] = acc;
        }
        tree_rows(red, ns, tid, nt);
        if (tid < ns) {
            const float nrm = sqrtf(red[tid][0]);
            factor[tid] = isfinite(nrm) ? (nrm > 1.0f ? 1.0f / nrm : 1.0f)
                                        : -1.0f;
        }
        __syncthreads();
        const float bc1 = bc_s[0], bc2 = bc_s[1];

        for (int r = 0; r < ns; ++r) {
            const int off = sg[r * 5], size = sg[r * 5 + 1];
            const int K = sg[r * 5 + 2];
            const float f = factor[r];
            if (K > 0 && do_constraints) {
                const int pairs = sg[r * 5 + 3] * sg[r * 5 + 4];
                for (int i = tid; i < pairs; i += nt) {
                    float sq = 0.f;
                    for (int k = 0; k < K; ++k) {
                        const float w = adam_element(
                            p, g, m, v, off + k * pairs + i, f, lr, beta1,
                            beta2, eps, bc1, bc2);
                        sq += w * w;
                    }
                    const float nrm = sqrtf(sq);
                    if (nrm > 1.0f) {
                        const float c = 1.0f / nrm;
                        for (int k = 0; k < K; ++k) p[off + k * pairs + i] *= c;
                    }
                }
                red[r][tid] = 0.f;
            } else {
                float acc = 0.f;
                for (int i = tid; i < size; i += nt) {
                    const float w = adam_element(p, g, m, v, off + i, f, lr,
                                                 beta1, beta2, eps, bc1, bc2);
                    acc += w * w;
                }
                red[r][tid] = acc;
            }
        }
        if (!do_constraints) {
            __syncthreads();
            continue;
        }
        tree_rows(red, ns, tid, nt);
        for (int r = 0; r < ns; ++r) {
            if (sg[r * 5 + 2] > 0) continue;
            const int off = sg[r * 5], size = sg[r * 5 + 1];
            const float nrm = sqrtf(red[r][0]);
            if (nrm > 1.0f) {
                const float c = 1.0f / nrm;
                for (int i = tid; i < size; i += nt) p[off + i] *= c;
            }
        }
        __syncthreads();
    }
}

}

void fused_adam_hip(torch::Tensor p, torch::Tensor g, torch::Tensor m,
                    torch::Tensor v, torch::Tensor seg, torch::Tensor step,
                    double scale, double lr, double beta1, double beta2,
                    double eps, bool constraints) {
    const int n_seg = seg.size(0);
    auto stream = at::cuda::getCurrentCUDAStream();
    hipLaunchKernelGGL(fused_adam_kernel, dim3(1), dim3(NT), 0,
                       stream.stream(),
                       p.data_ptr<float>(), g.data_ptr<float>(),
                       m.data_ptr<float>(), v.data_ptr<float>(),
                       seg.data_ptr<int>(), n_seg,
                       (float)scale, (float)lr, (float)beta1, (float)beta2,
                       (float)eps, step.data_ptr<int>(),
                       constraints ? 1 : 0);
}
```

### multihop_offload_amd/ops/hip/queueing.hip

```cpp

#include <hip/hip_runtime.h>
#include <torch/extension.h>
#include <ATen/cuda/CUDAContext.h>

#include "queue_model.h"

namespace {

using namespace qm;

__global__ void critic_kernel(
    const int* __restrict__ route_links,
    const int* __restrict__ nhop,
    const long* __restrict__ vedge_dst,
    const bool* __restrict__ mask,
    const float* __restrict__ rate,
    const float* __restrict__ ul,
    const float* __restrict__ dl,
    const Tables t,
    float* __restrict__ grad_edge,
    float* __restrict__ loss_out,
    float* __restrict__ g_hist,
    float* __restrict__ g_dunit,
    float* __restrict__ g_dlam,
    const CriticPlan p,
    float cap,
    int stage_budget,
    int E, int C, int Ee, int J, int H, int iters) {
    extern __shared__ __attribute__((aligned(16))) char smem_raw[];
    float* lds = reinterpret_cast<float*>(smem_raw);
    const int b = blockIdx.x;
    const int tid = threadIdx.x, nt = blockDim.x;
    float* lam_e = lds + p.lam_e;
    float* unit = lds + p.unit;
    float* dunit = region(lds, p.dunit, g_dunit + (size_t)b * Ee);
    float* dlam = region(lds, p.dlam, g_dlam + (size_t)b * Ee);
    float* dgre = region(lds, p.dgre, grad_edge + (size_t)b * Ee);
    float* hist = region(lds, p.hist, g_hist + (size_t)b * (iters + 1) * E);
    float* s1 = lds + p.s1;
    float* s2 = lds + p.s2;
    float* s3 = lds + p.s3;
    __shared__ float loss_acc;
    const Graph g = graph_view(t, b);
    const Csr csr = stage_csr(g.cip, g.rates, g.ccols, g.Eb,
                              smem_raw + stage_align(p.lds_bytes),
                              stage_budget, tid, nt);

    for (int e = tid; e < Ee; e += nt) {
        lam_e[e] = 0.f;
        if (!p.large) { dunit[e] = 0.f; dlam[e] = 0.f; dgre[e] = 0.f; }
    }
    if (tid == 0) loss_acc = 0.f;
    __syncthreads();

    for (int j = tid; j < J; j += nt) {
        const size_t bj = (size_t)b * J + j;
        if (!mask[bj]) continue;
        const float load = rate[bj] * ul[bj];
        const int nh = nhop[bj];
        for (int h = 0; h < nh; ++h) {
            const int l = route_links[bj * H + h];
            if (l < 0) break;
            atomicAdd(&lam_e[l], load);
        }
        atomicAdd(&lam_e[(int)vedge_dst[bj]], load);
    }
    __syncthreads();

    fixed_point_fwd(csr, lam_e, hist, s1, g.Eb, E, iters, tid, nt);
    const float* mu_last = hist + (size_t)iters * E;
    for (int e = tid; e < g.Eb; e += nt)
        unit[e] = unit_fwd(lam_e[e], mu_last[e], g.T, 101.0f, cap);
    for (int k = tid; k < C; k += nt)
        unit[E + k] = unit_fwd(lam_e[E + k], g.bw[k], g.T, 100.0f, cap);
    __syncthreads();

    float lloc = 0.f;
    for (int j = tid; j < J; j += nt) {
        const size_t bj = (size_t)b * J + j;
        if (!mask[bj]) continue;
        const float data = ul[bj] + dl[bj];
        const int nh = nhop[bj];
        for (int h = 0; h <= nh; ++h) {
            const int e = (h < nh) ? route_links[bj * H + h]
                                   : (int)vedge_dst[bj];
            if (e < 0) break;
            const float x = data * unit[e];
            lloc += x > 1.f ? x : 1.f;
            const float wx = x > 1.f ? 1.f : (x < 1.f ? 0.f : 0.5f);
            atomicAdd(&dunit[e], data * wx);
        }
    }
    atomicAdd(&loss_acc, lloc);
    __syncthreads();

    for (int e = tid; e < g.Eb; e += nt) {
        float dl_, dm_;
        unit_bwd(lam_e[e], mu_last[e], g.T, 101.0f, cap, dunit[e], &dl_,
                 &dm_);
        dlam[e] += dl_;
        s2[e] = dm_;
    }
    for (int k = tid; k < C; k += nt) {
        float dl_, dm_;
        unit_bwd(lam_e[E + k], g.bw[k], g.T, 100.0f, cap, dunit[E + k], &dl_,
                 &dm_);
        dlam[E + k] += dl_;
    }
    __syncthreads();
    fixed_point_bwd(csr, lam_e, hist, s2 , s1 , s3 ,
                    dlam, g.Eb, E, iters, tid, nt);
    __syncthreads();

    for (int j = tid; j < J; j += nt) {
        const size_t bj = (size_t)b * J + j;
        if (!mask[bj]) continue;
        const float data = ul[bj] + dl[bj];
        const float load = rate[bj] * ul[bj];
        const int nh = nhop[bj];
        float run = 0.f;
        for (int h = 0; h <= nh; ++h) {
            const int e = (h < nh) ? route_links[bj * H + h]
                                   : (int)vedge_dst[bj];
            if (e < 0) break;
            const float x = data * unit[e];
            const float wx = x > 1.f ? 1.f : (x < 1.f ? 0.f : 0.5f);
            const float direct = data * unit[e] * wx + (1.f - wx);
            const float gr = direct + dlam[e] * load;
            run += gr;
            atomicAdd(&dgre[e], -run);
        }
    }
    __syncthreads();
    if (!p.large) {
        float* geb = grad_edge + (size_t)b * Ee;
        for (int e = tid; e < Ee; e += nt) geb[e] = dgre[e];
    }
    if (tid == 0) loss_out[b] = loss_acc;
}

__global__ void actor_head_fwd_kernel(
    const float* __restrict__ lam_ext,
    const Tables t,
    const int* __restrict__ edges,
    const long* __restrict__ node_vedge,
    float* __restrict__ dm,
    float* __restrict__ mu_hist_out,
    const ActorFwdPlan p, float cap, int stage_budget, int N, int E, int C,
    int Ee, int iters) {
    extern __shared__ __attribute__((aligned(16))) char smem_raw[];
    float* lds = reinterpret_cast<float*>(smem_raw);
    const int b = blockIdx.x;
    const int tid = threadIdx.x, nt = blockDim.x;
    float* ho = mu_hist_out + (size_t)b * (iters + 1) * E;
    float* lam = lds + p.lam;
    float* hist = region(lds, p.hist, ho);
    float* busy = lds + p.busy;
    const Graph g = graph_view(t, b);
    const float* le = lam_ext + (size_t)b * Ee;
    const int* edg = edges + (size_t)b * E * 2;
    const long* nv = node_vedge + (size_t)b * N;
    float* dmb = dm + (size_t)b * N * N;

    for (int e = tid; e < g.Eb; e += nt) lam[e] = le[e];
    const Csr csr = stage_csr(g.cip, g.rates, g.ccols, g.Eb,
                              smem_raw + stage_align(p.lds_bytes),
                              stage_budget, tid, nt);
    __syncthreads();
    fixed_point_fwd(csr, lam, hist, busy, g.Eb, E, iters, tid, nt);
    const float* mu_last = hist + (size_t)iters * E;
    for (int e = tid; e < g.Eb; e += nt) {
        const float d = unit_fwd(lam[e], mu_last[e], g.T, 101.0f, cap);
        const int u = edg[e * 2], v = edg[e * 2 + 1];
        dmb[(size_t)u * N + v] = d;
        dmb[(size_t)v * N + u] = d;
    }
    for (int n = tid; n < N; n += nt) {
        const long ve = nv[n];
        dmb[(size_t)n * N + n] =
            ve >= 0 ? unit_fwd(le[ve], g.bw[ve - E], g.T, 100.0f, cap)
                    : INFINITY;
    }
    if (!p.large) {
        for (size_t i = tid; i < (size_t)(iters + 1) * E; i += nt)
            ho[i] = hist[i];
    }
}

struct DenseCot {
    const float* grad_dist;
    DEV_INLINE float cell(int b, int N, int r, int c, int ,
                          float& , int& ) const {
        return grad_dist[((size_t)b * N + r) * N + c];
    }
    DEV_INLINE void finish(int, float, int, float*, float*) const {}
};

struct FusedCot {
    const float* grad_edge;
    const float* dm;
    const float* unit_mtx;
    const bool* written;
    float* mse_sq;
    int* mse_cnt;
    int Ee;
    DEV_INLINE float cell(int b, int N, int r, int c, int edge, float& sq,
                          int& cnt) const {
#pragma clang fp contract(off)
        const size_t i = ((size_t)b * N + r) * N + c;
        float a = 0.f;
        if (written[i]) {
            const float d = dm[i];
            if (isfinite(d)) {
                const float diff = d - unit_mtx[i];
                a = 0.001f * diff;
                sq += diff * diff;
                cnt += 1;
            }
        }
        const float ge = edge >= 0 ? grad_edge[(size_t)b * Ee + edge] : 0.f;
        return ge + a;
    }
    DEV_INLINE void finish(int b, float sq, int cnt, float* free1,
                           float* free2) const {
        float* s_sq = free1;
        int* s_cnt = reinterpret_cast<int*>(free2);
        if (threadIdx.x == 0) { *s_sq = 0.f; *s_cnt = 0; }
        __syncthreads();
        if (cnt) { atomicAdd(s_sq, sq); atomicAdd(s_cnt, cnt); }
        __syncthreads();
        if (threadIdx.x == 0) {
            mse_sq[b] = *s_sq;
            mse_cnt[b] = *s_cnt;
        }
    }
};

__global__ void mse_finish_kernel(const float* __restrict__ mse_sq,
                                  const int* __restrict__ mse_cnt, int B,
                                  float* __restrict__ out) {
    __shared__ float s_sq[256];
    __shared__ long long s_cnt[256];
    float sq = 0.f;
    long long cnt = 0;
    for (int b = threadIdx.x; b < B; b += 256) {
        sq += mse_sq[b];
        cnt += mse_cnt[b];
    }
    s_sq[threadIdx.x] = sq;
    s_cnt[threadIdx.x] = cnt;
    __syncthreads();
    for (int w = 128; w > 0; w >>= 1) {
        if (threadIdx.x < w) {
            s_sq[threadIdx.x] += s_sq[threadIdx.x + w];
            s_cnt[threadIdx.x] += s_cnt[threadIdx.x + w];
        }
        __syncthreads();
    }
    if (threadIdx.x == 0)
        out[0] = s_sq[0] / (float)(s_cnt[0] > 1 ? s_cnt[0] : 1);
}

template <class Cot>
__global__ void actor_head_bwd_kernel(
    const Cot cot,
    const float* __restrict__ lam_ext,
    const float* __restrict__ mu_hist,
    const Tables t,
    const int* __restrict__ edges,
    const long* __restrict__ node_vedge,
    float* __restrict__ dlam_ext,
    const ActorBwdPlan p, float cap, int stage_budget, int N, int E, int C,
    int Ee, int iters) {
    extern __shared__ __attribute__((aligned(16))) char smem_raw[];
    float* lds = reinterpret_cast<float*>(smem_raw);
    const int b = blockIdx.x;
    const int tid = threadIdx.x, nt = blockDim.x;
    const float* hg = mu_hist + (size_t)b * (iters + 1) * E;
    float* lam = lds + p.lam;
    const float* hist = region(lds, p.hist, hg);
    float* dmu = lds + p.dmu;
    float* dlam = lds + p.dlam;
    float* s1 = lds + p.s1;
    float* s2 = lds + p.s2;
    const Graph g = graph_view(t, b);
    const float* le = lam_ext + (size_t)b * Ee;
    const int* edg = edges + (size_t)b * E * 2;
    const long* nv = node_vedge + (size_t)b * N;
    float* out = dlam_ext + (size_t)b * Ee;
    float sq = 0.f;
    int cnt = 0;

    for (int e = tid; e < g.Eb; e += nt) lam[e] = le[e];
    if (!p.large) {
        float* h = lds + p.hist;
        for (size_t i = tid; i < (size_t)(iters + 1) * E; i += nt)
            h[i] = hg[i];
    }
    const Csr csr = stage_csr(g.cip, g.rates, g.ccols, g.Eb,
                              smem_raw + stage_align(p.lds_bytes),
                              stage_budget, tid, nt);
    __syncthreads();
    const float* mu_last = hist + (size_t)iters * E;

    for (int e = tid; e < g.Eb; e += nt) {
        const int u = edg[e * 2], v = edg[e * 2 + 1];
        const float dd = cot.cell(b, N, u, v, e, sq, cnt)
            + cot.cell(b, N, v, u, e, sq, cnt);
        float dl_, dm_;
        unit_bwd(lam[e], mu_last[e], g.T, 101.0f, cap, dd, &dl_, &dm_);
        dlam[e] = dl_;
        dmu[e] = dm_;
    }
    __syncthreads();
    fixed_point_bwd(csr, lam, hist, dmu, s1, s2, dlam, g.Eb, E, iters, tid,
                    nt);

    for (int e = tid; e < E; e += nt) out[e] = e < g.Eb ? dlam[e] : 0.f;
    for (int n = tid; n < N; n += nt) {
        const long ve = nv[n];
        const float dd = cot.cell(b, N, n, n, (int)ve, sq, cnt);
        if (ve >= 0) {
            float dl_, dm_;
            unit_bwd(le[ve], g.bw[ve - E], g.T, 100.0f, cap, dd, &dl_, &dm_);
            out[ve] = dl_;
        }
    }
    for (int e = tid; e < Ee; e += nt) {
        if (e >= E + C) out[e] = 0.f;
    }
    cot.finish(b, sq, cnt, s1, s2);
}

}

std::vector<torch::Tensor> critic_hip(
    torch::Tensor route_links, torch::Tensor nhop, torch::Tensor vedge_dst,
    torch::Tensor mask, torch::Tensor rate, torch::Tensor ul,
    torch::Tensor dl, torch::Tensor conf_indptr, torch::Tensor conf_base,
    torch::Tensor conf_cols, torch::Tensor rates, torch::Tensor bw_comp,
    torch::Tensor E_arr, torch::Tensor T_arr, long Ee, long iters,
    double cap) {
    const int B = route_links.size(0), J = route_links.size(1);
    const int H = route_links.size(2);
    const int E = rates.size(1), C = bw_comp.size(1);
    auto loss = torch::empty({B}, rates.options());
    const CriticPlan p = critic_plan(E, (int)Ee, (int)iters);
    TORCH_CHECK(p.fits, "graph too large even for the global-scratch critic");
    torch::Tensor g_hist, g_dunit, g_dlam;
    torch::Tensor grad_edge;
    if (p.large) {
        g_hist = torch::empty({B, iters + 1, (long)E}, rates.options());
        g_dunit = torch::zeros({B, (long)Ee}, rates.options());
        g_dlam = torch::zeros({B, (long)Ee}, rates.options());
        grad_edge = torch::zeros({B, (long)Ee}, rates.options());
    } else {
        g_hist = torch::empty({1}, rates.options());
        g_dunit = g_hist;
        g_dlam = g_hist;
        grad_edge = torch::empty({B, (long)Ee}, rates.options());
    }
    auto stream = at::cuda::getCurrentCUDAStream();
    const int budget = stage_budget(p);
    hipLaunchKernelGGL(critic_kernel, dim3(B), dim3(p.threads),
                       launch_lds_bytes(p, budget), stream.stream(),
                       route_links.data_ptr<int>(), nhop.data_ptr<int>(),
                       vedge_dst.data_ptr<long>(), mask.data_ptr<bool>(),
                       rate.data_ptr<float>(), ul.data_ptr<float>(),
                       dl.data_ptr<float>(),
                       tables(conf_indptr, conf_base, conf_cols, rates,
                              bw_comp, T_arr, E_arr),
                       grad_edge.data_ptr<float>(), loss.data_ptr<float>(),
                       g_hist.data_ptr<float>(), g_dunit.data_ptr<float>(),
                       g_dlam.data_ptr<float>(), p, (float)cap, budget,
                       E, C, (int)Ee, J, H, (int)iters);
    return {grad_edge, loss};
}

std::vector<torch::Tensor> actor_head_fwd_hip(
    torch::Tensor lam_ext, torch::Tensor conf_indptr,
    torch::Tensor conf_base, torch::Tensor conf_cols, torch::Tensor rates,
    torch::Tensor bw_comp, torch::Tensor edges, torch::Tensor node_vedge,
    torch::Tensor T_arr, torch::Tensor E_arr, long N, long iters,
    double cap) {
    const int B = lam_ext.size(0), Ee = lam_ext.size(1);
    const int E = rates.size(1), C = bw_comp.size(1);
    auto dm = torch::empty({B, N, N}, lam_ext.options());
    auto mu_hist = torch::empty({B, iters + 1, (long)E}, lam_ext.options());
    const ActorFwdPlan p = actor_fwd_plan(E, (int)iters);
    TORCH_CHECK(p.fits, "graph too large for LDS actor head");
    auto stream = at::cuda::getCurrentCUDAStream();
    const int budget = stage_budget(p);
    hipLaunchKernelGGL(actor_head_fwd_kernel, dim3(B), dim3(p.threads),
                       launch_lds_bytes(p, budget), stream.stream(),
                       lam_ext.data_ptr<float>(),
                       tables(conf_indptr, conf_base, conf_cols, rates,
                              bw_comp, T_arr, E_arr),
                       edges.data_ptr<int>(), node_vedge.data_ptr<long>(),
                       dm.data_ptr<float>(), mu_hist.data_ptr<float>(),
                       p, (float)cap, budget, (int)N, E, C, Ee, (int)iters);
    return {dm, mu_hist};
}

namespace {

template <class Cot>
torch::Tensor actor_head_bwd_launch(
    const Cot& cot, int N, torch::Tensor lam_ext, torch::Tensor mu_hist,
    torch::Tensor conf_indptr, torch::Tensor conf_base,
    torch::Tensor conf_cols, torch::Tensor rates, torch::Tensor bw_comp,
    torch::Tensor edges, torch::Tensor node_vedge, torch::Tensor T_arr,
    torch::Tensor E_arr, long iters, double cap) {
    const int B = lam_ext.size(0), Ee = lam_ext.size(1);
    const int E = rates.size(1), C = bw_comp.size(1);
    auto dlam = torch::zeros_like(lam_ext);
    const ActorBwdPlan p = actor_bwd_plan(E, (int)iters);
    TORCH_CHECK(p.fits, "graph too large for LDS actor head bwd");
    auto stream = at::cuda::getCurrentCUDAStream();
    const int budget = stage_budget(p);
    hipLaunchKernelGGL(actor_head_bwd_kernel<Cot>, dim3(B), dim3(p.threads),
                       launch_lds_bytes(p, budget), stream.stream(), cot,
                       lam_ext.data_ptr<float>(), mu_hist.data_ptr<float>(),
                       tables(conf_indptr, conf_base, conf_cols, rates,
                              bw_comp, T_arr, E_arr),
                       edges.data_ptr<int>(), node_vedge.data_ptr<long>(),
                       dlam.data_ptr<float>(),
                       p, (float)cap, budget, N, E, C, Ee, (int)iters);
    return dlam;
}

}

torch::Tensor actor_head_bwd_hip(
    torch::Tensor grad_dist, torch::Tensor lam_ext, torch::Tensor mu_hist,
    torch::Tensor conf_indptr, torch::Tensor conf_base,
    torch::Tensor conf_cols, torch::Tensor rates, torch::Tensor bw_comp,
    torch::Tensor edges, torch::Tensor node_vedge, torch::Tensor T_arr,
    torch::Tensor E_arr, long iters, double cap) {
    return actor_head_bwd_launch(
        DenseCot{grad_dist.data_ptr<float>()}, (int)grad_dist.size(1),
        lam_ext, mu_hist, conf_indptr, conf_base, conf_cols, rates, bw_comp,
        edges, node_vedge, T_arr, E_arr, iters, cap);
}

std::vector<torch::Tensor> actor_head_bwd_fused_hip(
    torch::Tensor grad_edge, torch::Tensor dm, torch::Tensor unit_mtx,
    torch::Tensor written, torch::Tensor lam_ext, torch::Tensor mu_hist,
    torch::Tensor conf_indptr, torch::Tensor conf_base,
    torch::Tensor conf_cols, torch::Tensor rates, torch::Tensor bw_comp,
    torch::Tensor edges, torch::Tensor node_vedge, torch::Tensor T_arr,
    torch::Tensor E_arr, long iters, double cap) {
    const int B = lam_ext.size(0), Ee = lam_ext.size(1);
    const int N = dm.size(1);
    TORCH_CHECK(grad_edge.is_contiguous() && dm.is_contiguous()
                && unit_mtx.is_contiguous() && written.is_contiguous()
                && lam_ext.is_contiguous(), "contiguous inputs expected");
    TORCH_CHECK(grad_edge.size(0) == B && grad_edge.size(1) == Ee
                && dm.size(0) == B && dm.size(2) == N
                && unit_mtx.sizes() == dm.sizes()
                && written.sizes() == dm.sizes(), "shape mismatch");
    auto mse_sq = torch::empty({B}, lam_ext.options());
    auto mse_cnt = torch::empty({B}, lam_ext.options().dtype(torch::kInt));
    auto dlam = actor_head_bwd_launch(
        FusedCot{grad_edge.data_ptr<float>(), dm.data_ptr<float>(),
                 unit_mtx.data_ptr<float>(), written.data_ptr<bool>(),
                 mse_sq.data_ptr<float>(), mse_cnt.data_ptr<int>(), Ee},
        N, lam_ext, mu_hist, conf_indptr, conf_base, conf_cols, rates,
        bw_comp, edges, node_vedge, T_arr, E_arr, iters, cap);
    auto loss_mse = torch::empty({}, lam_ext.options());
    hipLaunchKernelGGL(mse_finish_kernel, dim3(1), dim3(256), 0,
                       at::cuda::getCurrentCUDAStream().stream(),
                       mse_sq.data_ptr<float>(), mse_cnt.data_ptr<int>(), B,
                       loss_mse.data_ptr<float>());
    return {dlam, loss_mse};
}

py::dict queue_lds_plan(long N, long E, long Ee, long iters) {
    using namespace pybind11::literals;
    auto row = [](const Launch& l) {
        return py::dict("lds_bytes"_a = l.lds_bytes, "large"_a = l.large,
                        "threads"_a = l.threads, "fits"_a = l.fits);
    };
    return py::dict(
        "critic"_a = row(critic_plan((int)E, (int)Ee, (int)iters)),
        "actor_head_fwd"_a = row(actor_fwd_plan((int)E, (int)iters)),
        "actor_head_bwd"_a = row(actor_bwd_plan((int)E, (int)iters)),
        "walk_eval"_a = row(walk_plan((int)N, (int)E)));
}

py::dict queue_csr_stage(long N, long E, long Ee, long iters) {
    using namespace pybind11::literals;
    auto row = [](const Launch& l) {
        return py::dict("budget_bytes"_a = stage_budget(l));
    };
    return py::dict(
        "critic"_a = row(critic_plan((int)E, (int)Ee, (int)iters)),
        "actor_head_fwd"_a = row(actor_fwd_plan((int)E, (int)iters)),
        "actor_head_bwd"_a = row(actor_bwd_plan((int)E, (int)iters)),
        "walk_eval"_a = row(walk_plan((int)N, (int)E)));
}

long queue_csr_bytes(long Eb, long nnz) {
    return Eb <= STAGE_MAX_E ? (long)stage_bytes(Eb, nnz) : -1;
}

void queue_csr_force_global(bool on) { stage_force_global = on; }

long queue_csr_set_budget(long bytes) {
    const long prev = stage_budget_setting;
    stage_budget_setting = bytes < 0 ? STAGE_BUDGET_DEFAULT : (int)bytes;
    return prev;
}
```

Measured before the change: 489,200 episodes/s.

## Fold small torch launches into HIP kernels across the episode step

Several separate torch operations are folded into existing HIP kernels. Zero-fills of dW/db, dlam and walk scratch move inside the kernels, the critic loss sum moves into the mse finish kernel, and overflow accumulation moves into walk_eval. The node_vedge gather now runs in the critic kernel, uds is passed strided without a contiguous copy, and the fused Adam kernel gains a ticket for a single-launch reduction. The aim is to cut kernel launches and host overhead per step, at the cost of more kernel complexity and some correctness risk around in-kernel zeroing.

Result: faster. 570,400 episodes/s, median of 6 (+16.6%).

```diff
diff --git a/multihop_offload_amd/engine.py b/multihop_offload_amd/engine.py
--- a/multihop_offload_amd/engine.py
+++ b/multihop_offload_amd/engine.py
@@ -491,13 +491,14 @@
         return dm, (lam, lam_c, mu_hist)
 
     def _actor_backward_native(self, saved, grad_edge, dm, unit_mtx,
-                               written):
+                               written, critic_loss=None):
         lam, lam_c, mu_hist = saved
-        dlam, loss_mse = ops.require_hip().actor_head_bwd_fused(
+        out = ops.require_hip().actor_head_bwd_fused(
             grad_edge.contiguous(), dm, unit_mtx, written, lam_c, mu_hist,
-            *self._actor_head_tables(), self.fp_iters, self.delay_clamp)
-        lam.backward(dlam)
-        return loss_mse
+            *self._actor_head_tables(), self.fp_iters, self.delay_clamp,
+            critic_loss)
+        lam.backward(out[0])
+        return out[1] if critic_loss is None else (out[1], out[2])
 
     def actor_forward(self, jobs: JobBatch):
         B, E, Ee, N = self.B, self.E, self.Ee, self.N
@@ -574,7 +575,7 @@
                 self._rng_state[1] += 1
                 rng_t = self._rng_state
             dst, islocal = ext.decide(
-                sp.contiguous(), self.sp_hop.contiguous(), uds.contiguous(),
+                sp.contiguous(), self.sp_hop.contiguous(), uds,
                 self.k_servers, jobs.sources, jobs.mask,
                 jobs.ul.contiguous(), jobs.dl.contiguous(),
                 expl_t, rng_t, 1 if prob else 0)
@@ -673,9 +674,8 @@
                 self.k_conf_cols, self.link_rates.contiguous(),
                 self.proc_bws.contiguous(), self.k_edges,
                 self.T_arr.contiguous(), self.k_E_arr, self.k_N_arr, H,
-                self.fp_iters)
+                self.fp_iters, self.overflow_total)
             self._last_overflow = overflow
-            self.overflow_total += overflow.sum().to(torch.int64)
             return rl, nhop, delay_emp, unit_mtx, written
         rl, nhop = self.route_walk(jobs, dst, sp)
         delay_emp, unit_mtx, written, *_ = self.evaluate(jobs, dst, rl, nhop)
@@ -772,22 +772,23 @@
 
     def critic_backward(self, jobs: JobBatch, dst: torch.Tensor,
                         route_links: torch.Tensor,
-                        nhop: Optional[torch.Tensor] = None):
+                        nhop: Optional[torch.Tensor] = None,
+                        per_graph: bool = False):
         B, E, Ee, J = self.B, self.E, self.Ee, self.Jmax
-        vedge_dst = self.node_vedge.gather(1, dst)
         if self.use_hip and self.hip_critic_ok:
             from .ops import dispatch
             ext = dispatch.require_hip()
             grad_edge, loss = ext.critic(
                 route_links.contiguous(), nhop.contiguous(),
-                vedge_dst.contiguous(), jobs.mask,
+                dst.contiguous(), jobs.mask,
                 jobs.rates.contiguous(), jobs.ul.contiguous(),
                 jobs.dl.contiguous(), self.k_conf_indptr, self.k_conf_base,
                 self.k_conf_cols, self.link_rates.contiguous(),
                 self.bw_comp.contiguous(), self.k_E_arr,
                 self.T_arr.contiguous(), Ee,
-                self.fp_iters, self.delay_clamp)
-            return grad_edge, loss.sum()
+                self.fp_iters, self.delay_clamp, self.node_vedge)
+            return grad_edge, (loss if per_graph else loss.sum())
+        vedge_dst = self.node_vedge.gather(1, dst)
         H = route_links.shape[2]
         valid = route_links >= 0
         safe = route_links.clamp(min=0)
@@ -890,10 +891,14 @@
         loss_fn = loss_mse = None
         self.last_per_sample_grads = None
         if train:
-            grad_edge, loss_fn = self.critic_backward(jobs, dst, route_links,
-                                                      nhop)
+            fuse_sum = native_bwd and self.use_hip and self.hip_critic_ok
+            grad_edge, loss_fn = self.critic_backward(
+                jobs, dst, route_links, nhop, per_graph=fuse_sum)
             self.per_sample_request = per_sample
-            if native_bwd:
+            if fuse_sum:
+                loss_mse, loss_fn = self._actor_backward_native(
+                    actor_saved, grad_edge, dm, unit_mtx, written, loss_fn)
+            elif native_bwd:
                 loss_mse = self._actor_backward_native(
                     actor_saved, grad_edge, dm, unit_mtx, written)
             else:
diff --git a/multihop_offload_amd/ops/dispatch.py b/multihop_offload_amd/ops/dispatch.py
--- a/multihop_offload_amd/ops/dispatch.py
+++ b/multihop_offload_amd/ops/dispatch.py
@@ -58,6 +58,10 @@
 
 def cheb_force_full_width(on: bool) -> None:
     _require_hip().cheb_force_full_width(bool(on))
+
+
+def adam_force_single_block(on: bool) -> None:
+    _require_hip().adam_force_single_block(bool(on))
 
 
 def cheb_lds_plan(Ee: int, K: int, max_nnz: int) -> dict:
diff --git a/multihop_offload_amd/ops/functions.py b/multihop_offload_amd/ops/functions.py
--- a/multihop_offload_amd/ops/functions.py
+++ b/multihop_offload_amd/ops/functions.py
@@ -161,6 +161,7 @@
         self.m = _t.zeros_like(self.flat_p)
         self.v = _t.zeros_like(self.flat_p)
         self.step_dev = _t.zeros(1, dtype=_t.int32, device=dev)
+        self._ticket = _t.zeros(1, dtype=_t.int32, device=dev)
         segs = []
         off = 0
         with _t.no_grad():
@@ -187,7 +188,8 @@
         ext = dispatch.require_hip()
         ext.fused_adam(self.flat_p, self.flat_g, self.m, self.v, self.seg,
                        self.step_dev, scale, self.lr, self.betas[0],
-                       self.betas[1], self.eps, self.constraints)
+                       self.betas[1], self.eps, self.constraints,
+                       self._ticket)
 
     def state_dict(self):
         return {"m": self.m.detach().clone(),
diff --git a/multihop_offload_amd/ops/hip/bindings.cpp b/multihop_offload_amd/ops/hip/bindings.cpp
--- a/multihop_offload_amd/ops/hip/bindings.cpp
+++ b/multihop_offload_amd/ops/hip/bindings.cpp
@@ -16,14 +16,14 @@
     torch::Tensor conf_base, torch::Tensor conf_cols, torch::Tensor rates,
     torch::Tensor bw, torch::Tensor edges, torch::Tensor T_arr,
     torch::Tensor E_arr, torch::Tensor n_arr, long H,
-    long fp_iters);
+    long fp_iters, c10::optional<torch::Tensor> overflow_total);
 std::vector<torch::Tensor> critic_hip(
     torch::Tensor route_links, torch::Tensor nhop, torch::Tensor vedge_dst,
     torch::Tensor mask, torch::Tensor rate, torch::Tensor ul,
     torch::Tensor dl, torch::Tensor conf_indptr, torch::Tensor conf_base,
     torch::Tensor conf_cols, torch::Tensor rates, torch::Tensor bw_comp,
     torch::Tensor E_arr, torch::Tensor T_arr, long Ee, long iters,
-    double cap);
+    double cap, c10::optional<torch::Tensor> node_vedge);
 std::vector<torch::Tensor> actor_head_fwd_hip(
     torch::Tensor lam_ext, torch::Tensor conf_indptr,
     torch::Tensor conf_base, torch::Tensor conf_cols, torch::Tensor rates,
@@ -42,7 +42,8 @@
     torch::Tensor conf_indptr, torch::Tensor conf_base,
     torch::Tensor conf_cols, torch::Tensor rates, torch::Tensor bw_comp,
     torch::Tensor edges, torch::Tensor node_vedge, torch::Tensor T_arr,
-    torch::Tensor E_arr, long iters, double cap);
+    torch::Tensor E_arr, long iters, double cap,
+    c10::optional<torch::Tensor> critic_loss);
 torch::Tensor floyd_warshall_dm_hip(torch::Tensor dm, torch::Tensor adj,
                                     c10::optional<torch::Tensor> n_arr);
 void fw_force_inplace(bool on);
@@ -155,16 +156,38 @@
 void fused_adam_hip(torch::Tensor p, torch::Tensor g, torch::Tensor m,
                     torch::Tensor v, torch::Tensor seg, torch::Tensor step,
                     double scale, double lr, double beta1, double beta2,
-                    double eps, bool constraints);
+                    double eps, bool constraints,
+                    c10::optional<torch::Tensor> ticket);
+void adam_force_single_block(bool on);
 
 PYBIND11_MODULE(TORCH_EXTENSION_NAME, m) {
     m.def("floyd_warshall", &floyd_warshall_hip);
     m.def("decide", &decide_hip);
-    m.def("walk_eval", &walk_eval_hip);
-    m.def("critic", &critic_hip);
+    m.def("walk_eval", &walk_eval_hip, py::arg("sp"), py::arg("src"),
+          py::arg("dst"), py::arg("mask"), py::arg("rate"), py::arg("ul"),
+          py::arg("dl"), py::arg("adj_indptr"), py::arg("adj_idx"),
+          py::arg("adj_link"), py::arg("conf_indptr"), py::arg("conf_base"),
+          py::arg("conf_cols"), py::arg("rates"), py::arg("bw"),
+          py::arg("edges"), py::arg("T_arr"), py::arg("E_arr"),
+          py::arg("n_arr"), py::arg("H"), py::arg("fp_iters"),
+          py::arg("overflow_total") = py::none());
+    m.def("critic", &critic_hip, py::arg("route_links"), py::arg("nhop"),
+          py::arg("vedge_dst"), py::arg("mask"), py::arg("rate"),
+          py::arg("ul"), py::arg("dl"), py::arg("conf_indptr"),
+          py::arg("conf_base"), py::arg("conf_cols"), py::arg("rates"),
+          py::arg("bw_comp"), py::arg("E_arr"), py::arg("T_arr"),
+          py::arg("Ee"), py::arg("iters"), py::arg("cap"),
+          py::arg("node_vedge") = py::none());
     m.def("actor_head_fwd", &actor_head_fwd_hip);
     m.def("actor_head_bwd", &actor_head_bwd_hip);
-    m.def("actor_head_bwd_fused", &actor_head_bwd_fused_hip);
+    m.def("actor_head_bwd_fused", &actor_head_bwd_fused_hip,
+          py::arg("grad_edge"), py::arg("dm"), py::arg("unit_mtx"),
+          py::arg("written"), py::arg("lam_ext"), py::arg("mu_hist"),
+          py::arg("conf_indptr"), py::arg("conf_base"), py::arg("conf_cols"),
+          py::arg("rates"), py::arg("bw_comp"), py::arg("edges"),
+          py::arg("node_vedge"), py::arg("T_arr"), py::arg("E_arr"),
+          py::arg("iters"), py::arg("cap"),
+          py::arg("critic_loss") = py::none());
     m.def("floyd_warshall_dm", &floyd_warshall_dm_hip);
     m.def("fw_force_inplace", &fw_force_inplace);
     m.def("fw_register_rows", &fw_register_rows);
@@ -196,7 +219,12 @@
     m.def("cheb_kn_bwd", &cheb_kn_bwd_hip);
     m.def("cheb_fits_lds", &cheb_fits_lds);
     m.def("cheb_lds_plan", &cheb_lds_plan_py);
-    m.def("fused_adam", &fused_adam_hip);
+    m.def("fused_adam", &fused_adam_hip, py::arg("p"), py::arg("g"),
+          py::arg("m"), py::arg("v"), py::arg("seg"), py::arg("step"),
+          py::arg("scale"), py::arg("lr"), py::arg("beta1"),
+          py::arg("beta2"), py::arg("eps"), py::arg("constraints"),
+          py::arg("ticket") = py::none());
+    m.def("adam_force_single_block", &adam_force_single_block);
     m.def("cheb_large_fwd", &cheb_large_fwd_hip);
     m.def("cheb_large_bwd", &cheb_large_bwd_hip);
 }
diff --git a/multihop_offload_amd/ops/hip/chebconv.hip b/multihop_offload_amd/ops/hip/chebconv.hip
--- a/multihop_offload_amd/ops/hip/chebconv.hip
+++ b/multihop_offload_amd/ops/hip/chebconv.hip
@@ -531,13 +531,20 @@
 
     const int b = blockIdx.x;
     const int tid = threadIdx.x, nt = blockDim.x;
+    float* dWb = dW + (size_t)b * L * K * F * F;
+    float* dbb = db + (size_t)b * L * F;
+    {
+        const float4 z = make_float4(0.f, 0.f, 0.f, 0.f);
+        float4* w4 = reinterpret_cast<float4*>(dWb);
+        for (int i = tid; i < L * K * F * F / 4; i += nt) w4[i] = z;
+        float4* b4 = reinterpret_cast<float4*>(dbb);
+        for (int i = tid; i < L * F / 4; i += nt) b4[i] = z;
+    }
     const int *ipt, *cls;
     graph_csr(ext_indptr, ext_base, ext_cols, b, Ee, stage_csr,
               reinterpret_cast<int*>(Wl + (size_t)K * F * F), tid, nt, ipt,
               cls);
     const float* actsb = acts + (size_t)b * (L + 1) * Ee * F;
-    float* dWb = dW + (size_t)b * L * K * F * F;
-    float* dbb = db + (size_t)b * L * F;
 
     if (EDGE) {
         const int l = L - 1;
@@ -928,8 +935,8 @@
                     "forward expected");
     const LdsPlan plan = cheb_lds_plan(Ee, K, BWD_NBUF, false, max_nnz);
     TORCH_CHECK(plan.fits, "graph too large for fused ChebConv bwd");
-    auto dW = torch::zeros({B, L, K, F, F}, dlam.options());
-    auto db = torch::zeros({B, L, F}, dlam.options());
+    auto dW = torch::empty({B, L, K, F, F}, dlam.options());
+    auto db = torch::empty({B, L, F}, dlam.options());
     auto stream = at::cuda::getCurrentCUDAStream();
     hipLaunchKernelGGL(edge ? cheb_bwd_kernel<true> : cheb_bwd_kernel<false>,
                        dim3(B), dim3(512), plan.lds_bytes, stream.stream(),
diff --git a/multihop_offload_amd/ops/hip/episode.hip b/multihop_offload_amd/ops/hip/episode.hip
--- a/multihop_offload_amd/ops/hip/episode.hip
+++ b/multihop_offload_amd/ops/hip/episode.hip
@@ -21,12 +21,12 @@
 }
 
 DEV_INLINE float server_cost(const float* sp_row, const float* hop_row,
-                             const float* uds, int sv, float ulj,
+                             const float* uds, long us, int sv, float ulj,
                              float dlj) {
     const float spv = sp_row[sv];
     const float hpv = hop_row[sv];
     return fmax1(spv * ulj, hpv) + fmax1(spv * dlj, hpv)
-           + fmax1(uds[sv] * ulj, 1.0f);
+           + fmax1(uds[sv * us] * ulj, 1.0f);
 }
 
 DEV_INLINE float softmax_w(float c, float cmax) {
@@ -37,6 +37,7 @@
     const float* __restrict__ sp,
     const float* __restrict__ hop,
     const float* __restrict__ uds,
+    long uds_sb, long uds_sn,
     const int* __restrict__ servers,
     const long* __restrict__ src,
     const bool* __restrict__ mask,
@@ -50,7 +51,7 @@
     const int b = blockIdx.x;
     const float* spb = sp + (size_t)b * N * N;
     const float* hpb = hop + (size_t)b * N * N;
-    const float* udsb = uds + (size_t)b * N;
+    const float* udsb = uds + (size_t)b * uds_sb;
     const int* srvb = servers + (size_t)b * S;
     const float eps = explore ? *explore : 0.0f;
     const unsigned long long key =
@@ -63,7 +64,7 @@
         const int s0 = (int)src[bj];
         if (!mask[bj]) { dst_out[bj] = s0; islocal_out[bj] = true; continue; }
         const float ulj = ul[bj], dlj = dl[bj];
-        const float local = udsb[s0] * ulj;
+        const float local = udsb[s0 * uds_sn] * ulj;
         const float* sp_row = spb + (size_t)s0 * N;
         const float* hop_row = hpb + (size_t)s0 * N;
         int best_s;
@@ -72,7 +73,7 @@
             for (int s = 0; s < S; ++s) {
                 const int sv = srvb[s];
                 if (sv < 0) continue;
-                float c = server_cost(sp_row, hop_row, udsb, sv, ulj, dlj);
+                float c = server_cost(sp_row, hop_row, udsb, uds_sn, sv, ulj, dlj);
                 if (isfinite(c)) { c = c < 1e30f ? c : 1e30f;
                                    cmax = c > cmax ? c : cmax; }
             }
@@ -81,7 +82,7 @@
                 const int sv = srvb[s];
                 if (sv < 0) continue;
                 psum += softmax_w(
-                    server_cost(sp_row, hop_row, udsb, sv, ulj, dlj), cmax);
+                    server_cost(sp_row, hop_row, udsb, uds_sn, sv, ulj, dlj), cmax);
             }
             psum += softmax_w(local, cmax);
             const float r = u01(mix64(key ^ (unsigned long long)bj)) * psum;
@@ -91,7 +92,7 @@
                 const int sv = srvb[s];
                 if (sv < 0) continue;
                 acc += softmax_w(
-                    server_cost(sp_row, hop_row, udsb, sv, ulj, dlj), cmax);
+                    server_cost(sp_row, hop_row, udsb, uds_sn, sv, ulj, dlj), cmax);
                 if (r < acc) { best_s = s; break; }
             }
         } else {
@@ -101,7 +102,7 @@
                 const int sv = srvb[s];
                 if (sv < 0) continue;
                 const float c =
-                    server_cost(sp_row, hop_row, udsb, sv, ulj, dlj);
+                    server_cost(sp_row, hop_row, udsb, uds_sn, sv, ulj, dlj);
                 if (c < best) { best = c; best_s = s; }
             }
             if (local < best) best_s = -1;
@@ -139,6 +140,7 @@
     bool* __restrict__ written,
     unsigned long long* __restrict__ upack,
     int* __restrict__ overflow,
+    unsigned long long* __restrict__ overflow_total,
     const int* __restrict__ n_arr,
     const qm::WalkPlan p, int stage_budget, int N, int E, int J, int H,
     int fp_iters) {
@@ -148,6 +150,7 @@
     float* mu = lds + p.mu;
     float* busy = lds + p.busy;
     float* sload = lds + p.sload;
+    __shared__ int ovf_s;
 
     const int b = blockIdx.x;
     const int tid = threadIdx.x;
@@ -157,7 +160,9 @@
     const int* aix = adj_idx + (size_t)b * 2 * E;
     const int* alk = adj_link + (size_t)b * 2 * E;
     const qm::Graph g = qm::graph_view(t, b);
-    unsigned long long* upk = upack + (size_t)b * N * N;
+    unsigned long long* upk = upack + (size_t)b * (E + N);
+    float* um = unit_mtx + (size_t)b * N * N;
+    bool* wm = written + (size_t)b * N * N;
     const int Eb = g.Eb;
     const int nb_ = n_arr[b];
     const qm::Csr csr = qm::stage_csr(
@@ -166,8 +171,18 @@
 
     for (int e = tid; e < Eb; e += nt) lam[e] = 0.0f;
     for (int n = tid; n < nb_; n += nt) sload[n] = 0.0f;
-    for (int i = tid; i < nb_ * nb_; i += nt)
-        upk[(i / nb_) * N + (i % nb_)] = 0ull;
+    for (int i = tid; i < E + N; i += nt) upk[i] = 0ull;
+    if (tid == 0) ovf_s = 0;
+    if (((N * N) & 15) == 0) {
+        float4* um4 = reinterpret_cast<float4*>(um);
+        uint4* wm4 = reinterpret_cast<uint4*>(wm);
+        for (int i = tid; i < N * N / 4; i += nt)
+            um4[i] = make_float4(0.f, 0.f, 0.f, 0.f);
+        for (int i = tid; i < N * N / 16; i += nt)
+            wm4[i] = make_uint4(0u, 0u, 0u, 0u);
+    } else {
+        for (int i = tid; i < N * N; i += nt) { um[i] = 0.f; wm[i] = false; }
+    }
     __syncthreads();
 
     for (int j = tid; j < J; j += nt) {
@@ -197,7 +212,7 @@
             node = bestn;
             ++h;
         }
-        if (node != d) atomicAdd(&overflow[b], 1);
+        if (node != d) atomicAdd(&ovf_s, 1);
         nhop[bj] = h;
         for (int h2 = h; h2 < H; ++h2)
             route_links[bj * H + h2] = -1;
@@ -220,30 +235,40 @@
             const int l = route_links[((size_t)b * J + j) * H + h];
             if (l < 0) break;
             const float unit = qm::emp_unit(lam[l], mu[l], g.T, tot);
-            const int u = edg[l * 2], v = edg[l * 2 + 1];
-            const unsigned long long pk = jtag | (unsigned long long)
-                __float_as_uint(unit);
-            atomicMax(&upk[(size_t)u * N + v], pk);
-            atomicMax(&upk[(size_t)v * N + u], pk);
+            atomicMax(&upk[l], jtag | (unsigned long long)
+                                   __float_as_uint(unit));
             acc += fmax1(ulj * unit, nh) + fmax1(dlj * unit, nh);
         }
         const int d = (int)dstv[bj];
         const float sunit = qm::emp_unit(sload[d], g.bw[d], g.T, ulj);
-        atomicMax(&upk[(size_t)d * N + d],
+        atomicMax(&upk[E + d],
                   jtag | (unsigned long long)__float_as_uint(sunit));
         acc += fmax1(ulj * sunit, 1.0f);
         delay_emp[bj] = acc;
     }
     __syncthreads();
-    float* um = unit_mtx + (size_t)b * N * N;
-    bool* wm = written + (size_t)b * N * N;
-    for (int i = tid; i < N * N; i += nt) {
-        const int r = i / N, c = i % N;
-        const unsigned long long pk =
-            (r < nb_ && c < nb_) ? upk[i] : 0ull;
-        um[i] = pk ? __uint_as_float((unsigned int)(pk & 0xffffffffull))
-                   : 0.f;
-        wm[i] = pk != 0ull;
+    for (int e = tid; e < Eb; e += nt) {
+        const unsigned long long pk = upk[e];
+        if (!pk) continue;
+        const float unit = __uint_as_float((unsigned int)(pk & 0xffffffffull));
+        const int u = edg[e * 2], v = edg[e * 2 + 1];
+        um[(size_t)u * N + v] = unit;
+        um[(size_t)v * N + u] = unit;
+        wm[(size_t)u * N + v] = true;
+        wm[(size_t)v * N + u] = true;
+    }
+    for (int n = tid; n < nb_; n += nt) {
+        const unsigned long long pk = upk[E + n];
+        if (!pk) continue;
+        um[(size_t)n * N + n] =
+            __uint_as_float((unsigned int)(pk & 0xffffffffull));
+        wm[(size_t)n * N + n] = true;
+    }
+    if (tid == 0) {
+        const int cnt = ovf_s;
+        overflow[b] = cnt;
+        if (cnt && overflow_total)
+            atomicAdd(overflow_total, (unsigned long long)cnt);
     }
 }
 
@@ -257,6 +282,9 @@
     long prob) {
     const int B = sp.size(0), N = sp.size(1);
     const int J = src.size(1), S = servers.size(1);
+    TORCH_CHECK(uds.dim() == 2 && uds.size(0) == B && uds.size(1) == N
+                && uds.scalar_type() == torch::kFloat32,
+                "decide: uds is (B,N) fp32");
     auto dst = torch::empty({B, J}, src.options());
     auto islocal = torch::empty({B, J}, mask.options());
     const float* ep = explore.has_value()
@@ -265,7 +293,8 @@
     auto stream = at::cuda::getCurrentCUDAStream();
     hipLaunchKernelGGL(decide_kernel, dim3(B), dim3(256), 0, stream.stream(),
                        sp.data_ptr<float>(), hop.data_ptr<float>(),
-                       uds.data_ptr<float>(),
+                       uds.data_ptr<float>(), (long)uds.stride(0),
+                       (long)uds.stride(1),
                        servers.data_ptr<int>(), src.data_ptr<long>(),
                        mask.data_ptr<bool>(), ul.data_ptr<float>(),
                        dl.data_ptr<float>(), ep, rp,
@@ -282,9 +311,18 @@
     torch::Tensor conf_base, torch::Tensor conf_cols, torch::Tensor rates,
     torch::Tensor bw, torch::Tensor edges, torch::Tensor T_arr,
     torch::Tensor E_arr, torch::Tensor n_arr, long H,
-    long fp_iters) {
+    long fp_iters, c10::optional<torch::Tensor> overflow_total) {
     const int B = sp.size(0), N = sp.size(1);
     const int J = src.size(1), E = rates.size(1);
+    unsigned long long* ovf_total = nullptr;
+    if (overflow_total.has_value()) {
+        TORCH_CHECK(overflow_total->scalar_type() == torch::kInt64
+                    && overflow_total->numel() == 1
+                    && overflow_total->is_cuda(),
+                    "walk_eval: overflow_total is one int64 on the device");
+        ovf_total = reinterpret_cast<unsigned long long*>(
+            overflow_total->data_ptr<long>());
+    }
     auto opts_i = adj_indptr.options();
     auto opts_f = sp.options();
     auto route_links = torch::empty({B, J, H}, opts_i.dtype(torch::kInt32));
@@ -292,8 +330,8 @@
     auto delay_emp = torch::empty({B, J}, opts_f);
     auto unit_mtx = torch::empty({B, N, N}, opts_f);
     auto written = torch::empty({B, N, N}, opts_f.dtype(torch::kBool));
-    auto upack = torch::empty({B, N, N}, opts_f.dtype(torch::kInt64));
-    auto overflow = torch::zeros({B}, opts_i.dtype(torch::kInt32));
+    auto upack = torch::empty({B, E + N}, opts_f.dtype(torch::kInt64));
+    auto overflow = torch::empty({B}, opts_i.dtype(torch::kInt32));
     const qm::WalkPlan p = qm::walk_plan(N, E);
     TORCH_CHECK(p.fits, "graph too large for LDS walk_eval");
     auto stream = at::cuda::getCurrentCUDAStream();
@@ -314,7 +352,8 @@
                        unit_mtx.data_ptr<float>(), written.data_ptr<bool>(),
                        reinterpret_cast<unsigned long long*>(
                            upack.data_ptr<long>()),
-                       overflow.data_ptr<int>(), n_arr.data_ptr<int>(), p,
+                       overflow.data_ptr<int>(), ovf_total,
+                       n_arr.data_ptr<int>(), p,
                        budget, N, E, J, (int)H, (int)fp_iters);
     return {route_links, nhop, delay_emp, unit_mtx, written, overflow};
 }
diff --git a/multihop_offload_amd/ops/hip/optimizer.hip b/multihop_offload_amd/ops/hip/optimizer.hip
--- a/multihop_offload_amd/ops/hip/optimizer.hip
+++ b/multihop_offload_amd/ops/hip/optimizer.hip
@@ -7,6 +7,8 @@
 
 constexpr int NT = 256;
 constexpr int SEG_GROUP = 16;
+constexpr int EPT = 8;
+constexpr int PPT = 4;
 
 __device__ __forceinline__ void tree_rows(float (*red)[NT], int rows,
                                           int tid, int nt) {
@@ -18,19 +20,29 @@
     }
 }
 
+__device__ __forceinline__ float adam_value(
+    float pj, float gj, float mj, float vj, float f, float lr, float beta1,
+    float beta2, float eps, float bc1, float bc2, float* mn_out,
+    float* vn_out) {
+    float gv = gj * f;
+    gv = isfinite(gv) ? gv : 0.f;
+    const float mn = beta1 * mj + (1.f - beta1) * gv;
+    const float vn = beta2 * vj + (1.f - beta2) * gv * gv;
+    *mn_out = mn;
+    *vn_out = vn;
+    return pj - lr * (mn * bc1) / (sqrtf(vn * bc2) + eps);
+}
+
 __device__ __forceinline__ float adam_element(
     float* __restrict__ p, const float* __restrict__ g,
     float* __restrict__ m, float* __restrict__ v, int j, float f, float lr,
     float beta1, float beta2, float eps, float bc1, float bc2) {
     if (f < 0.f) return p[j];
-    float gv = g[j] * f;
-    gv = isfinite(gv) ? gv : 0.f;
-    const float mn = beta1 * m[j] + (1.f - beta1) * gv;
-    const float vn = beta2 * v[j] + (1.f - beta2) * gv * gv;
+    float mn, vn;
+    const float pj = adam_value(p[j], g[j], m[j], v[j], f, lr, beta1, beta2,
+                                eps, bc1, bc2, &mn, &vn);
     m[j] = mn;
     v[j] = vn;
-    float pj = p[j];
-    pj -= lr * (mn * bc1) / (sqrtf(vn * bc2) + eps);
     p[j] = pj;
     return pj;
 }
@@ -124,14 +136,215 @@
     }
 }
 
-}
+__device__ __forceinline__ void tree_one(float* red, int tid) {
+    __syncthreads();
+    for (int w = NT >> 1; w > 0; w >>= 1) {
+        if (tid < w) red[tid] += red[tid + w];
+        __syncthreads();
+    }
+}
+
+template <int KC>
+__device__ __forceinline__ void adam_pairs(
+    float* __restrict__ p, const float* __restrict__ g,
+    float* __restrict__ m, float* __restrict__ v, int off, int pairs,
+    float f, float lr, float beta1, float beta2, float eps, float bc1,
+    float bc2, int tid) {
+    for (int base = 0; base < pairs; base += PPT * NT) {
+        float pv[PPT][KC], gv[PPT][KC], mv[PPT][KC], vv[PPT][KC];
+#pragma unroll
+        for (int u = 0; u < PPT; ++u) {
+            const int i = base + u * NT + tid;
+#pragma unroll
+            for (int k = 0; k < KC; ++k) {
+                const int j = off + k * pairs + i;
+                const bool in = i < pairs;
+                pv[u][k] = in ? p[j] : 0.f;
+                gv[u][k] = in && f >= 0.f ? g[j] : 0.f;
+                mv[u][k] = in && f >= 0.f ? m[j] : 0.f;
+                vv[u][k] = in && f >= 0.f ? v[j] : 0.f;
+            }
+        }
+#pragma unroll
+        for (int u = 0; u < PPT; ++u) {
+            const int i = base + u * NT + tid;
+            if (i >= pairs) continue;
+            float sq = 0.f;
+#pragma unroll
+            for (int k = 0; k < KC; ++k) {
+                if (f >= 0.f) {
+                    const int j = off + k * pairs + i;
+                    float mn, vn;
+                    pv[u][k] = adam_value(pv[u][k], gv[u][k], mv[u][k],
+                                          vv[u][k], f, lr, beta1, beta2, eps,
+                                          bc1, bc2, &mn, &vn);
+                    m[j] = mn;
+                    v[j] = vn;
+                }
+                sq = __fmaf_rn(pv[u][k], pv[u][k], sq);
+            }
+            const float nrm = sqrtf(sq);
+            const float c = 1.0f / nrm;
+            if (f >= 0.f || nrm > 1.0f) {
+#pragma unroll
+                for (int k = 0; k < KC; ++k)
+                    p[off + k * pairs + i] =
+                        nrm > 1.0f ? pv[u][k] * c : pv[u][k];
+            }
+        }
+    }
+}
+
+__global__ void __launch_bounds__(NT) fused_adam_blocks_kernel(
+    float* __restrict__ p, float* __restrict__ g,
+    float* __restrict__ m, float* __restrict__ v,
+    const int* __restrict__ seg, int n_seg,
+    float scale, float lr, float beta1, float beta2, float eps,
+    int* step_dev, int* ticket, int do_constraints) {
+    __shared__ float red[NT];
+    __shared__ float red2[NT];
+    __shared__ float bc_s[2];
+    __shared__ int t_s;
+    const int tid = threadIdx.x;
+    const int r = blockIdx.x;
+    const int off = seg[r * 5], size = seg[r * 5 + 1], K = seg[r * 5 + 2];
+    const int pairs = seg[r * 5 + 3] * seg[r * 5 + 4];
+    if (tid == 0) {
+        const int ti = __hip_atomic_load(step_dev, __ATOMIC_RELAXED,
+                                         __HIP_MEMORY_SCOPE_AGENT) + 1;
+        const float t = (float)ti;
+        t_s = ti;
+        bc_s[0] = 1.0f / (1.0f - powf(beta1, t));
+        bc_s[1] = 1.0f / (1.0f - powf(beta2, t));
+    }
+
+    float acc = 0.f;
+    for (int base = 0; base < size; base += EPT * NT) {
+        float gv[EPT];
+#pragma unroll
+        for (int u = 0; u < EPT; ++u) {
+            const int i = base + u * NT + tid;
+            gv[u] = i < size ? g[off + i] : 0.f;
+        }
+#pragma unroll
+        for (int u = 0; u < EPT; ++u) {
+            const int i = base + u * NT + tid;
+            if (i < size) {
+                const float x = gv[u] * scale;
+                g[off + i] = x;
+                acc = __fmaf_rn(x, x, acc);
+            }
+        }
+    }
+    red[tid] = acc;
+    tree_one(red, tid);
+    const float nrm = sqrtf(red[0]);
+    const float f = isfinite(nrm) ? (nrm > 1.0f ? 1.0f / nrm : 1.0f) : -1.0f;
+    const float bc1 = bc_s[0], bc2 = bc_s[1];
+
+    if (K > 0 && do_constraints) {
+        if (K == 1) {
+            adam_pairs<1>(p, g, m, v, off, pairs, f, lr, beta1, beta2, eps,
+                          bc1, bc2, tid);
+        } else if (K == 2) {
+            adam_pairs<2>(p, g, m, v, off, pairs, f, lr, beta1, beta2, eps,
+                          bc1, bc2, tid);
+        } else if (K == 3) {
+            adam_pairs<3>(p, g, m, v, off, pairs, f, lr, beta1, beta2, eps,
+                          bc1, bc2, tid);
+        } else {
+            for (int i = tid; i < pairs; i += NT) {
+                float sq = 0.f;
+                for (int k = 0; k < K; ++k) {
+                    const float w = adam_element(
+                        p, g, m, v, off + k * pairs + i, f, lr, beta1, beta2,
+                        eps, bc1, bc2);
+                    sq += w * w;
+                }
+                const float pn = sqrtf(sq);
+                if (pn > 1.0f) {
+                    const float c = 1.0f / pn;
+                    for (int k = 0; k < K; ++k) p[off + k * pairs + i] *= c;
+                }
+            }
+        }
+    } else {
+        float acc2 = 0.f;
+        for (int base = 0; base < size; base += EPT * NT) {
+            float pv[EPT], gv[EPT], mv[EPT], vv[EPT];
+#pragma unroll
+            for (int u = 0; u < EPT; ++u) {
+                const int i = base + u * NT + tid;
+                const bool in = i < size;
+                pv[u] = in ? p[off + i] : 0.f;
+                gv[u] = in && f >= 0.f ? g[off + i] : 0.f;
+                mv[u] = in && f >= 0.f ? m[off + i] : 0.f;
+                vv[u] = in && f >= 0.f ? v[off + i] : 0.f;
+            }
+#pragma unroll
+            for (int u = 0; u < EPT; ++u) {
+                const int i = base + u * NT + tid;
+                if (i >= size) continue;
+                if (f >= 0.f) {
+                    float mn, vn;
+                    pv[u] = adam_value(pv[u], gv[u], mv[u], vv[u], f, lr,
+                                       beta1, beta2, eps, bc1, bc2, &mn, &vn);
+                    m[off + i] = mn;
+                    v[off + i] = vn;
+                    p[off + i] = pv[u];
+                }
+                acc2 = __fmaf_rn(pv[u], pv[u], acc2);
+            }
+        }
+        if (do_constraints) {
+            red2[tid] = acc2;
+            tree_one(red2, tid);
+            const float bn = sqrtf(red2[0]);
+            if (bn > 1.0f) {
+                const float c = 1.0f / bn;
+                for (int i = tid; i < size; i += NT) p[off + i] *= c;
+            }
+        }
+    }
+
+    if (tid == 0) {
+        const int tk = __hip_atomic_fetch_add(ticket, 1, __ATOMIC_ACQ_REL,
+                                              __HIP_MEMORY_SCOPE_AGENT);
+        if (tk == n_seg - 1) {
+            __hip_atomic_store(step_dev, t_s, __ATOMIC_RELAXED,
+                               __HIP_MEMORY_SCOPE_AGENT);
+            __hip_atomic_store(ticket, 0, __ATOMIC_RELAXED,
+                               __HIP_MEMORY_SCOPE_AGENT);
+        }
+    }
+}
+
+bool adam_single_forced = false;
+
+}
+
+void adam_force_single_block(bool on) { adam_single_forced = on; }
 
 void fused_adam_hip(torch::Tensor p, torch::Tensor g, torch::Tensor m,
                     torch::Tensor v, torch::Tensor seg, torch::Tensor step,
                     double scale, double lr, double beta1, double beta2,
-                    double eps, bool constraints) {
+                    double eps, bool constraints,
+                    c10::optional<torch::Tensor> ticket) {
     const int n_seg = seg.size(0);
     auto stream = at::cuda::getCurrentCUDAStream();
+    if (ticket.has_value() && !adam_single_forced && n_seg > 0) {
+        TORCH_CHECK(ticket->scalar_type() == torch::kInt32
+                    && ticket->numel() == 1, "fused_adam: ticket is one int32");
+        hipLaunchKernelGGL(fused_adam_blocks_kernel, dim3(n_seg), dim3(NT),
+                           0, stream.stream(),
+                           p.data_ptr<float>(), g.data_ptr<float>(),
+                           m.data_ptr<float>(), v.data_ptr<float>(),
+                           seg.data_ptr<int>(), n_seg,
+                           (float)scale, (float)lr, (float)beta1,
+                           (float)beta2, (float)eps, step.data_ptr<int>(),
+                           ticket->data_ptr<int>(), constraints ? 1 : 0);
+        return;
+    }
     hipLaunchKernelGGL(fused_adam_kernel, dim3(1), dim3(NT), 0,
                        stream.stream(),
                        p.data_ptr<float>(), g.data_ptr<float>(),
diff --git a/multihop_offload_amd/ops/hip/queueing.hip b/multihop_offload_amd/ops/hip/queueing.hip
--- a/multihop_offload_amd/ops/hip/queueing.hip
+++ b/multihop_offload_amd/ops/hip/queueing.hip
@@ -13,6 +13,7 @@
     const int* __restrict__ route_links,
     const int* __restrict__ nhop,
     const long* __restrict__ vedge_dst,
+    const long* __restrict__ node_vedge,
     const bool* __restrict__ mask,
     const float* __restrict__ rate,
     const float* __restrict__ ul,
@@ -26,11 +27,16 @@
     const CriticPlan p,
     float cap,
     int stage_budget,
-    int E, int C, int Ee, int J, int H, int iters) {
+    int E, int C, int Ee, int J, int H, int iters, int N) {
     extern __shared__ __attribute__((aligned(16))) char smem_raw[];
     float* lds = reinterpret_cast<float*>(smem_raw);
     const int b = blockIdx.x;
     const int tid = threadIdx.x, nt = blockDim.x;
+    const long* nvb = node_vedge ? node_vedge + (size_t)b * N : nullptr;
+    auto dst_slot = [&](size_t bj) {
+        const long d = vedge_dst[bj];
+        return (int)(nvb ? nvb[d] : d);
+    };
     float* lam_e = lds + p.lam_e;
     float* unit = lds + p.unit;
     float* dunit = region(lds, p.dunit, g_dunit + (size_t)b * Ee);
@@ -63,7 +69,7 @@
             if (l < 0) break;
             atomicAdd(&lam_e[l], load);
         }
-        atomicAdd(&lam_e[(int)vedge_dst[bj]], load);
+        atomicAdd(&lam_e[dst_slot(bj)], load);
     }
     __syncthreads();
 
@@ -83,7 +89,7 @@
         const int nh = nhop[bj];
         for (int h = 0; h <= nh; ++h) {
             const int e = (h < nh) ? route_links[bj * H + h]
-                                   : (int)vedge_dst[bj];
+                                   : dst_slot(bj);
             if (e < 0) break;
             const float x = data * unit[e];
             lloc += x > 1.f ? x : 1.f;
@@ -121,7 +127,7 @@
         float run = 0.f;
         for (int h = 0; h <= nh; ++h) {
             const int e = (h < nh) ? route_links[bj * H + h]
-                                   : (int)vedge_dst[bj];
+                                   : dst_slot(bj);
             if (e < 0) break;
             const float x = data * unit[e];
             const float wx = x > 1.f ? 1.f : (x < 1.f ? 0.f : 0.5f);
@@ -237,28 +243,36 @@
 };
 
 __global__ void mse_finish_kernel(const float* __restrict__ mse_sq,
-                                  const int* __restrict__ mse_cnt, int B,
-                                  float* __restrict__ out) {
+                                  const int* __restrict__ mse_cnt,
+                                  const float* __restrict__ loss, int B,
+                                  float* __restrict__ out,
+                                  float* __restrict__ loss_out) {
     __shared__ float s_sq[256];
+    __shared__ float s_ls[256];
     __shared__ long long s_cnt[256];
-    float sq = 0.f;
+    float sq = 0.f, ls = 0.f;
     long long cnt = 0;
     for (int b = threadIdx.x; b < B; b += 256) {
         sq += mse_sq[b];
         cnt += mse_cnt[b];
+        if (loss) ls += loss[b];
     }
     s_sq[threadIdx.x] = sq;
+    s_ls[threadIdx.x] = ls;
     s_cnt[threadIdx.x] = cnt;
     __syncthreads();
     for (int w = 128; w > 0; w >>= 1) {
         if (threadIdx.x < w) {
             s_sq[threadIdx.x] += s_sq[threadIdx.x + w];
+            s_ls[threadIdx.x] += s_ls[threadIdx.x + w];
             s_cnt[threadIdx.x] += s_cnt[threadIdx.x + w];
         }
         __syncthreads();
     }
-    if (threadIdx.x == 0)
+    if (threadIdx.x == 0) {
         out[0] = s_sq[0] / (float)(s_cnt[0] > 1 ? s_cnt[0] : 1);
+        if (loss) loss_out[0] = s_ls[0];
+    }
 }
 
 template <class Cot>
@@ -291,6 +305,7 @@
     float sq = 0.f;
     int cnt = 0;
 
+    for (int e = E + tid; e < Ee; e += nt) out[e] = 0.f;
     for (int e = tid; e < g.Eb; e += nt) lam[e] = le[e];
     if (!p.large) {
         float* h = lds + p.hist;
@@ -326,9 +341,6 @@
             out[ve] = dl_;
         }
     }
-    for (int e = tid; e < Ee; e += nt) {
-        if (e >= E + C) out[e] = 0.f;
-    }
     cot.finish(b, sq, cnt, s1, s2);
 }
 
@@ -340,10 +352,21 @@
     torch::Tensor dl, torch::Tensor conf_indptr, torch::Tensor conf_base,
     torch::Tensor conf_cols, torch::Tensor rates, torch::Tensor bw_comp,
     torch::Tensor E_arr, torch::Tensor T_arr, long Ee, long iters,
-    double cap) {
+    double cap, c10::optional<torch::Tensor> node_vedge) {
     const int B = route_links.size(0), J = route_links.size(1);
     const int H = route_links.size(2);
     const int E = rates.size(1), C = bw_comp.size(1);
+    const long* nv = nullptr;
+    int N = 0;
+    if (node_vedge.has_value()) {
+        TORCH_CHECK(node_vedge->scalar_type() == torch::kInt64
+                    && node_vedge->dim() == 2 && node_vedge->size(0) == B
+                    && node_vedge->is_contiguous()
+                    && vedge_dst.is_contiguous(),
+                    "critic: node_vedge is a contiguous (B,N) int64");
+        nv = node_vedge->data_ptr<long>();
+        N = node_vedge->size(1);
+    }
     auto loss = torch::empty({B}, rates.options());
     const CriticPlan p = critic_plan(E, (int)Ee, (int)iters);
     TORCH_CHECK(p.fits, "graph too large even for the global-scratch critic");
@@ -365,7 +388,7 @@
     hipLaunchKernelGGL(critic_kernel, dim3(B), dim3(p.threads),
                        launch_lds_bytes(p, budget), stream.stream(),
                        route_links.data_ptr<int>(), nhop.data_ptr<int>(),
-                       vedge_dst.data_ptr<long>(), mask.data_ptr<bool>(),
+                       vedge_dst.data_ptr<long>(), nv, mask.data_ptr<bool>(),
                        rate.data_ptr<float>(), ul.data_ptr<float>(),
                        dl.data_ptr<float>(),
                        tables(conf_indptr, conf_base, conf_cols, rates,
@@ -373,7 +396,7 @@
                        grad_edge.data_ptr<float>(), loss.data_ptr<float>(),
                        g_hist.data_ptr<float>(), g_dunit.data_ptr<float>(),
                        g_dlam.data_ptr<float>(), p, (float)cap, budget,
-                       E, C, (int)Ee, J, H, (int)iters);
+                       E, C, (int)Ee, J, H, (int)iters, N);
     return {grad_edge, loss};
 }
 
@@ -413,7 +436,7 @@
     torch::Tensor E_arr, long iters, double cap) {
     const int B = lam_ext.size(0), Ee = lam_ext.size(1);
     const int E = rates.size(1), C = bw_comp.size(1);
-    auto dlam = torch::zeros_like(lam_ext);
+    auto dlam = torch::empty_like(lam_ext);
     const ActorBwdPlan p = actor_bwd_plan(E, (int)iters);
     TORCH_CHECK(p.fits, "graph too large for LDS actor head bwd");
     auto stream = at::cuda::getCurrentCUDAStream();
@@ -449,9 +472,15 @@
     torch::Tensor conf_indptr, torch::Tensor conf_base,
     torch::Tensor conf_cols, torch::Tensor rates, torch::Tensor bw_comp,
     torch::Tensor edges, torch::Tensor node_vedge, torch::Tensor T_arr,
-    torch::Tensor E_arr, long iters, double cap) {
+    torch::Tensor E_arr, long iters, double cap,
+    c10::optional<torch::Tensor> critic_loss) {
     const int B = lam_ext.size(0), Ee = lam_ext.size(1);
     const int N = dm.size(1);
+    if (critic_loss.has_value())
+        TORCH_CHECK(critic_loss->scalar_type() == torch::kFloat32
+                    && critic_loss->numel() == B
+                    && critic_loss->is_contiguous(),
+                    "critic_loss is the critic's (B,) fp32 loss");
     TORCH_CHECK(grad_edge.is_contiguous() && dm.is_contiguous()
                 && unit_mtx.is_contiguous() && written.is_contiguous()
                 && lam_ext.is_contiguous(), "contiguous inputs expected");
@@ -468,10 +497,15 @@
         N, lam_ext, mu_hist, conf_indptr, conf_base, conf_cols, rates,
         bw_comp, edges, node_vedge, T_arr, E_arr, iters, cap);
     auto loss_mse = torch::empty({}, lam_ext.options());
+    auto loss_fn = torch::empty({}, lam_ext.options());
     hipLaunchKernelGGL(mse_finish_kernel, dim3(1), dim3(256), 0,
                        at::cuda::getCurrentCUDAStream().stream(),
-                       mse_sq.data_ptr<float>(), mse_cnt.data_ptr<int>(), B,
-                       loss_mse.data_ptr<float>());
+                       mse_sq.data_ptr<float>(), mse_cnt.data_ptr<int>(),
+                       critic_loss.has_value()
+                           ? critic_loss->data_ptr<float>() : nullptr,
+                       B, loss_mse.data_ptr<float>(),
+                       loss_fn.data_ptr<float>());
+    if (critic_loss.has_value()) return {dlam, loss_mse, loss_fn};
     return {dlam, loss_mse};
 }
 
```
